# ecmwf-ifs/ecwam

Hardware: AMD Instinct MI355X
Metric: grid-point spectral steps/sec (whole node) at O320, 36dir x 36freq (higher is better)
Workload: dtype f32; 1 GPU; O320 all-ocean octahedral grid, 421080 sea points, 36 dir x 36 freq (NFRE_RED=36), full WAMINTGR step = PROPAGS2 advection + NEWWIND + IMPLSCH as one kernel (PROPAGS2 inside IMPLSCH's tile load), IDELT=IDELPRO=450 s, flag set A (IPHYS=1, ISNONLIN=0, LLGCBZ0=F, LLNORMAGAM=F); points_per_gpu=421080, halo_points=0, parallelism=sea-point block x1, ranks=1

## Files before the change

ecwam_amd/api.py:

```python
from __future__ import annotations

import ctypes as C

import numpy as np
import torch

from . import lib as _lib
from .tables import Tables

NFF, NINTF, NWPR = 16, 16, 5
OUTBS_SEP_FIELDS = ("mp1", "mp2", "wdw", "shww", "shts", "mdww", "mdts", "mpww", "mpts",
                    "p1sea", "p1swell", "p2sea", "p2swell", "sprdsea", "sprdswell")
OUTBS_PART_FIELDS = OUTBS_SEP_FIELDS + ("swh1", "mwd1", "mwp1", "swh2", "mwd2", "mwp2", "swh3", "mwd3", "mwp3")
OUTBS_EXT_FIELDS = ("c4", "bfi", "qp", "hmax", "tmax", "c3", "eta_m", "r", "xnslc", "cmax_f", "hmax_n", "cmax_st", "hmax_st")
OUTBS_ABS_FIELDS = ("swh", "mwd", "mwp", "em", "pp1d", "mp1", "mp2", "wdw")


class EcwamHipError(RuntimeError):
    pass


def _stream_ptr() -> int:
    return torch.cuda.current_stream().cuda_stream

# ... 146 lines not shown
            self._real(g["wlat"], (n, 2), "WLAT"), self._real(g["cosphm1_ext"], (nrow,), "COSPHM1_EXT"),
            self._real(depth_ext, (nrow,), "DEPTH_EXT"), self._real(u_ext, (nrow,), "U_EXT"), self._real(v_ext, (nrow,), "V_EXT"),
            self._real(refr, (n, 2 * self.NANG + 5), "REFR"), _stream_ptr()))

    def ctuw_refra(self, grid_dev: dict, cgroup_ext, omosnh2kd_ext, wavnum_ext, refr, cflfail, delpro: float, mstart=1, mend=None,
                   llcflcuroff=True, frange=0):
        mend = self.NR if mend is None else mend
        g = grid_dev
        n, nland, ngy = g["n"], g["nland"], g["ngy"]
        nrow = cgroup_ext.shape[0]
        if nland >= nrow:
            raise ValueError("CTUW: CGROUP_EXT must include the land row")
        ext = [self._real(a, (nrow, self.NFRE), nm) for a, nm in ((cgroup_ext, "CGROUP_EXT"), (omosnh2kd_ext, "OMOSNH2KD_EXT"),
                                                                 (wavnum_ext, "WAVNUM_EXT"))]
        self._chk(self.lib.ecwam_hip_ctuw_refra(self._h, n, nland, ngy, float(delpro), mstart, mend, *self._geom(g, n, ngy), *ext,
                                                self._real(g["cosphm1_ext"], (nrow,), "COSPHM1_EXT"),
                                                self._real(refr, (n, 2 * self.NANG + 5), "REFR"), int(llcflcuroff), int(frange),
                                                self._int(cflfail, (n,), "CFLFAIL"), _stream_ptr()))

    def propags2_refra(self, f1, f3, grid_dev: dict, cgroup_ext, omosnh2kd_ext, wavnum_ext, refr, delpro: float, kijs, kijl, nd3s=1,
                       nd3e=None, copy_rest=True, frange=0):
        nd3e = self.NR if nd3e is None else nd3e
        g = grid_dev
        n, nland, ngy = g["n"], g["nland"], g["ngy"]
        nrow = f1.shape[0]
        if not (0 <= kijs <= kijl <= n) or nland >= nrow or cgroup_ext.shape[0] != nrow:
            raise ValueError("PROPAGS2: KIJS/KIJL outside the neighbour tables, or F1 / CGROUP_EXT without the land row")
        ext = [self._real(a, (nrow, self.NFRE), nm) for a, nm in ((cgroup_ext, "CGROUP_EXT"), (omosnh2kd_ext, "OMOSNH2KD_EXT"),
                                                                 (wavnum_ext, "WAVNUM_EXT"))]
        self._chk(self.lib.ecwam_hip_propags2_refra(
            self._h, self._real(f1, (nrow, self.NANG, self.NFRE), "F1"), self._real(f3, (nrow, self.NANG, self.NFRE), "F3"), n, ngy,
            float(delpro), *self._geom(g, n, ngy), *ext, self._real(g["cosphm1_ext"], (nrow,), "COSPHM1_EXT"),
            self._real(refr, (n, 2 * self.NANG + 5), "REFR"), int(frange), kijs, kijl, nd3s, nd3e, int(copy_rest), _stream_ptr()))

    def implsch(self, kijs, kijl, fl1, wvprpt, ff, intf, mij, xllws, dbg=None, wam2nemo=None):
        nrow = fl1.shape[0]
        if not (0 <= kijs <= kijl <= min(nrow, wvprpt.shape[0], ff.shape[0], intf.shape[0], mij.shape[0], xllws.shape[0])):
            raise ValueError("IMPLSCH: KIJS/KIJL outside the operands")
        a = [self._real(fl1, (nrow, self.NANG, self.NFRE), "FL1"), self._real(wvprpt, (wvprpt.shape[0], NWPR, self.NFRE), "WVPRPT"),
             self._real(ff, (ff.shape[0], NFF), "FF"), self._real(intf, (intf.shape[0], NINTF), "INTF"),
             self._int(mij, (mij.shape[0],), "MIJ"), self._real(xllws, (xllws.shape[0], self.NANG, self.NFRE), "XLLWS")]
        pd = None if dbg is None else self._real(dbg, (nrow, 32), "DBG")
        pw = None
        if wam2nemo is not None:
            if not (wam2nemo.is_cuda and wam2nemo.dtype == torch.float64 and wam2nemo.is_contiguous() and wam2nemo.dim() == 2
                    and wam2nemo.shape[1] == 13 and wam2nemo.shape[0] >= kijl):
                raise ValueError("WAM2NEMO: expected contiguous float64 cuda tensor [npts >= KIJL][13]")
            pw = wam2nemo.data_ptr()
        self._chk(self.lib.ecwam_hip_implsch(self._h, kijs, kijl, *a, pw, pd, _stream_ptr()))

    def fused_supported(self, fast_waves: bool = False, obstructions: bool = False) -> bool:
        mask = int(self.lib.ecwam_hip_propags2_implsch_supported(self._h))
        need = 1 | (2 if fast_waves else 0) | (4 if obstructions else 0)
        return (mask & need) == need

    def propags2_implsch(self, f1, f3, grid_dev: dict, cgroup_ext, delpro: float, kijs, kijl, wvprpt, ff, intf, mij, xllws, nd3s=1, nd3e=None,
                         wam2nemo=None, flags: int = 0, ifrelfmax: int = 0, delpro_lf: float | None = None, gin=None):
        nd3e = self.NR if nd3e is None else nd3e
        g = grid_dev
        n, nland, ngy = g["n"], g["nland"], g["ngy"]
        nrow = f1.shape[0]
        if not (0 <= kijs <= kijl <= n) or nland >= nrow or cgroup_ext.shape[0] != nrow or f3.shape[0] < kijl:
            raise ValueError("PROPAGS2 + IMPLSCH: KIJS/KIJL outside the neighbour tables, or F1 / CGROUP_EXT without the land row")
        if not (kijl <= min(wvprpt.shape[0], ff.shape[0], intf.shape[0], mij.shape[0], xllws.shape[0])):
            raise ValueError("PROPAGS2 + IMPLSCH: KIJL outside the operands")
        pw = None
        if wam2nemo is not None:
            if not (wam2nemo.is_cuda and wam2nemo.dtype == torch.float64 and wam2nemo.is_contiguous() and wam2nemo.dim() == 2
                    and wam2nemo.shape[1] == 13 and wam2nemo.shape[0] >= kijl):
                raise ValueError("WAM2NEMO: expected contiguous float64 cuda tensor [npts >= KIJL][13]")
            pw = wam2nemo.data_ptr()
        args = [self._real(f1, (nrow, self.NANG, self.NFRE), "F1"), self._real(f3, (f3.shape[0], self.NANG, self.NFRE), "F3"), n, ngy, float(delpro),
                self._int(g["kxlt"], (n,), "KXLT"), self._real(g["zdello"], (ngy,), "ZDELLO"), float(g["xdella"]),
                self._real(g["cosph"], (ngy,), "COSPH"), self._real(g["sinph"], (ngy,), "SINPH"),
                self._int(g["klon"], (n, 2), "KLON"), self._int(g["klat"], (n, 2, 2), "KLAT"), self._int(g["kcor"], (n, 4, 2), "KCOR"),
                self._real(g["wlat"], (n, 2), "WLAT"), self._real(g["wcor"], (n, 4), "WCOR"),
                self._real(cgroup_ext, (nrow, self.NFRE), "CGROUP_EXT"), self._real(g["cosphm1_ext"], (nrow,), "COSPHM1_EXT"), kijs, kijl, nd3s, nd3e,
                self._real(wvprpt, (wvprpt.shape[0], NWPR, self.NFRE), "WVPRPT"), self._real(ff, (ff.shape[0], NFF), "FF"),
                self._real(intf, (intf.shape[0], NINTF), "INTF"), self._int(mij, (mij.shape[0],), "MIJ"),
                self._real(xllws, (xllws.shape[0], self.NANG, self.NFRE), "XLLWS"), pw,
                float(delpro if delpro_lf is None else delpro_lf), int(ifrelfmax),
                None if gin is None else self._real(gin, (gin.shape[0], self.NANG, gin.shape[2]), "GIN"), 0 if gin is None else int(gin.shape[2]),
                int(flags), _stream_ptr()]
        self._chk(self.lib.ecwam_hip_propags2_implsch(self._h, *args))

    def implsch_reserve(self, npts: int) -> None:
        self._chk(self.lib.ecwam_hip_implsch_reserve(self._h, int(npts)))

    def implsch_generation_used(self) -> int:
        return int(self.lib.ecwam_hip_implsch_generation_used(self._h))

    def device_tables(self) -> int:
        return int(self.lib.ecwam_hip_device_tables(self._h) or 0)

    def outbs(self, kijs, kijl, fl1, out, zmiss: float = -999.0):
        nrow = fl1.shape[0]
        if not (0 <= kijs <= kijl <= min(nrow, out.shape[0])):
            raise ValueError("OUTBS: KIJS/KIJL outside the operands")
        self._chk(self.lib.ecwam_hip_outbs(self._h, kijs, kijl, self._real(fl1, (nrow, self.NANG, self.NFRE), "FL1"), float(zmiss),
                                           self._real(out, (out.shape[0], 5), "OUT"), _stream_ptr()))

    def outbs_sepwisw(self, kijs, kijl, fl1, xllws, wvprpt, ff, out, zmiss: float = -999.0, small_domain: bool = False):
        nrow = fl1.shape[0]
        if not (0 <= kijs <= kijl <= min(nrow, xllws.shape[0], wvprpt.shape[0], ff.shape[0], out.shape[0])):
            raise ValueError("OUTBS_SEPWISW: KIJS/KIJL outside the operands")
        a = [self._real(fl1, (nrow, self.NANG, self.NFRE), "FL1"), self._real(xllws, (xllws.shape[0], self.NANG, self.NFRE), "XLLWS"),
             self._real(wvprpt, (wvprpt.shape[0], NWPR, self.NFRE), "WVPRPT"), self._real(ff, (ff.shape[0], NFF), "FF")]
        self._chk(self.lib.ecwam_hip_outbs_sepwisw(self._h, kijs, kijl, *a, 1 if small_domain else 0, float(zmiss),
                                                   self._real(out, (out.shape[0], len(OUTBS_SEP_FIELDS)), "OUT"), _stream_ptr()))

    def outbs_partition(self, kijs, kijl, fl1, xllws, mij, wvprpt, ff, out, zmiss: float = -999.0, flags: int = 0):
        nrow = fl1.shape[0]
        if not (0 <= kijs <= kijl <= min(nrow, xllws.shape[0], mij.shape[0], wvprpt.shape[0], ff.shape[0], out.shape[0])):
            raise ValueError("OUTBS_PARTITION: KIJS/KIJL outside the operands")
        a = [self._real(fl1, (nrow, self.NANG, self.NFRE), "FL1"), self._real(xllws, (xllws.shape[0], self.NANG, self.NFRE), "XLLWS"),
             self._int(mij, (mij.shape[0],), "MIJ"), self._real(wvprpt, (wvprpt.shape[0], NWPR, self.NFRE), "WVPRPT"),
             self._real(ff, (ff.shape[0], NFF), "FF")]
        self._chk(self.lib.ecwam_hip_outbs_partition(self._h, kijs, kijl, *a, int(flags), float(zmiss),
                                                     self._real(out, (out.shape[0], len(OUTBS_PART_FIELDS)), "OUT"), _stream_ptr()))

    def outbs_extremes(self, kijs, kijl, fl1, wvprpt, ff, out, kurtosis_only: bool = False):
        nrow = fl1.shape[0]
        if not (0 <= kijs <= kijl <= min(nrow, wvprpt.shape[0], ff.shape[0], out.shape[0])):
            raise ValueError("OUTBS_EXTREMES: KIJS/KIJL outside the operands")
        a = [self._real(fl1, (nrow, self.NANG, self.NFRE), "FL1"), self._real(wvprpt, (wvprpt.shape[0], NWPR, self.NFRE), "WVPRPT"),
             self._real(ff, (ff.shape[0], NFF), "FF")]
        self._chk(self.lib.ecwam_hip_outbs_extremes(self._h, kijs, kijl, *a, 1 if kurtosis_only else 0,
                                                    self._real(out, (out.shape[0], len(OUTBS_EXT_FIELDS)), "OUT"), _stream_ptr()))

    def outbs_absolute(self, kijs, kijl, fl1, wvprpt, ucur, vcur, ff, out, fl2nd=None, zmiss: float = -999.0, flags: int = 0):
        nrow = fl1.shape[0]
        rows = [nrow, out.shape[0]] + [a.shape[0] for a in (wvprpt, ucur, vcur, ff, fl2nd) if a is not None]
        if not (0 <= kijs <= kijl <= min(rows)):
            raise ValueError("OUTBS_ABSOLUTE: KIJS/KIJL outside the operands")
        opt = lambda a, shape, name: None if a is None else self._real(a, shape, name)
        a = [self._real(fl1, (nrow, self.NANG, self.NFRE), "FL1"),
             opt(wvprpt, (0 if wvprpt is None else wvprpt.shape[0], NWPR, self.NFRE), "WVPRPT"),
             opt(ucur, (0 if ucur is None else ucur.shape[0],), "UCUR"), opt(vcur, (0 if vcur is None else vcur.shape[0],), "VCUR"),
             opt(ff, (0 if ff is None else ff.shape[0], NFF), "FF")]
        self._chk(self.lib.ecwam_hip_outbs_absolute(self._h, kijs, kijl, *a, int(flags), float(zmiss),
                                                    self._real(out, (out.shape[0], len(OUTBS_ABS_FIELDS)), "OUT"),
                                                    opt(fl2nd, (0 if fl2nd is None else fl2nd.shape[0], self.NANG, self.NFRE), "FL2ND"), _stream_ptr()))

    @property
    def has_second_order(self) -> bool:
        return getattr(self, "_second_order", False)

    def set_second_order(self, so, coefficients=None) -> None:
        self._second_order = False
        if so is None:
            self._chk(self.lib.ecwam_hip_set_second_order(self._h, 0, 1.0, 1.1, 0, None, None, None, None, None, None, None))
            return
        dt = self.t.dtype
        if so.dtype != dt or so.NANGH * 2 != self.NANG or so.NFREH * 2 != self.NFRE:
            raise ValueError("second-order tables of another grid or precision")
        tabs = [getattr(so, c) for c in so.COEFFICIENTS] if coefficients is None else list(coefficients)
        shape = (so.NDEPTH, so.NANGH, so.NFREH, so.NFREH)
        host = [np.ascontiguousarray(np.asarray(a, dt).reshape(shape).transpose(3, 2, 1, 0)) for a in tabs]
        imp = np.ascontiguousarray(so.IM_P.T.astype(np.int32))
        imm = np.ascontiguousarray(so.IM_M.T.astype(np.int32))
        self._chk(self.lib.ecwam_hip_set_second_order(self._h, so.NDEPTH, float(so.DEPTHA), float(so.DEPTHD), so.NMAX, imp.ctypes.data, imm.ctypes.data,
                                                      *[a.ctypes.data for a in host]))
        self._second_order = True

    def outbs_second_order(self, kijs, kijl, fl1, wvprpt, depth, ucur, vcur, ff, out, fl2nd=None, sig: float = 1.0, zmiss: float = -999.0):
        nrow = fl1.shape[0]
        rows = [nrow, out.shape[0], wvprpt.shape[0], depth.shape[0]] + [a.shape[0] for a in (ucur, vcur, ff, fl2nd) if a is not None]
# ... 146 lines not shown
```

ecwam_amd/csrc/capi.hip:

```cpp
#include <cmath>
#include <cstdio>
#include <cstdlib>
#include <cstring>
#include <string>
#include <vector>

#include <dlfcn.h>
#include <rccl/rccl.h>

#include "dev.h"
#include "implsch_adv_args.h"

static thread_local std::string g_err;
static int fail(const std::string& m) {
  g_err = m;
  return 1;
}
#define HIPCHK(x)                                                                        \
  do {                                                                                   \
    hipError_t e_ = (x);                                                                 \
    if (e_ != hipSuccess) return fail(std::string(#x) + ": " + hipGetErrorString(e_));   \
  } while (0)

struct ecwam_hip_ctx {
  int real_bytes;
  int device;
  int NANG, NFRE, NFRE_RED;
  void* dtab = nullptr;
  double* norm_scratch = nullptr;
  void* itab = nullptr;
  int v4_ok = 0, v4_r1 = 0, v4_r2 = 0, v4_nh = 0, v4_shelter = 0;
  int implsch_last = 0;
  void* fin = nullptr;
  size_t fin_bytes = 0;
  void* wi = nullptr;
  size_t wi_bytes = 0;
  int rank = 0, nranks = 1;
  std::vector<int> peer, send_cnt, send_off, recv_dst0, recv_cnt;
  int n_send = 0, n_recv = 0;
  int* d_send_idx = nullptr;
  struct HaloSlot {
    int rowlen = 0;
    void* buf = nullptr;
    size_t bytes = 0;
    hipEvent_t ev_packed = nullptr, ev_done = nullptr;
    bool used = false;
    bool pending = false;
    unsigned long long age = 0;
  };
  static constexpr int NSLOT = 4;
  HaloSlot slot[NSLOT];
  unsigned long long slot_clock = 0;
  ncclComm_t comm = nullptr;
  hipStream_t comm_stream = nullptr;
  ecwam_hip_params p;
  void* fast_g = nullptr;
  int fast_gk = 0;
  std::string implsch_why;
  void* adv_pt = nullptr;
  size_t adv_pt_bytes = 0;
  void* adv_dir = nullptr;
  void* so_tab = nullptr;
  void* so_coef = nullptr;
  void* so_work = nullptr;
  size_t so_work_bytes = 0;
  int so_nmax = 0;
  std::vector<unsigned char> fr_host;
  const void* obs = nullptr;
  int n_obs = 0;
};

template <typename T> void launch_propags2(const void*, const void*, void*, const int*, const int*, const int*, const void*, int, int, int, int, int, int, hipStream_t);
template <typename T> void launch_ctuw(const void*, int, int, int, double, int, int, const int*, const void*, double, const void*, const void*, const int*, const int*, const int*, void*, void*, const void*, const void*, void*, int*, int, const void*, hipStream_t);
template <typename T> void launch_ctuwini_only(int, int, const int*, const int*, void*, void*, hipStream_t);
template <typename T> void launch_propdot(const void*, int, int, int, const int*, const void*, double, const void*, const int*, const int*, const void*, const void*, const void*, const void*, const void*, void*, hipStream_t);
template <typename T> void launch_curmask(int, int, int, const int*, void*, hipStream_t);
template <typename T> void launch_propags2_gen(const void*, int, const void*, void*, int, double, const int*, const void*, double, const void*, const void*, const int*, const int*, const int*, const void*, const void*, const void*, const void*, const void*, const void*, const void*, int*, int, int, int, int, int, int, int, const void*, hipStream_t);
template <typename T> void launch_propags2_otf(const void*, const void*, void*, int, int, double, const int*, const void*, double, const void*, const void*, const int*, const int*, const int*, const void*, const void*, const void*, const void*, const int*, int, int, int, int, int, int, const void*, int, double, int, void*, int, const void*, int, int, hipStream_t);
template <typename T> void launch_copy_freq_range(const void*, void*, int, int, int, int, int, int, hipStream_t);
template <typename T> int launch_outbs(const void*, int, int, const void*, double, void*, int, int, hipStream_t);
template <typename T> int launch_outbs_sepwisw(const void*, int, int, const void*, const void*, const void*, const void*, int, double, void*, int, int,
                                               hipStream_t);
template <typename T> int launch_outbs_partition(const void*, int, int, const void*, const void*, const int*, const void*, const void*, double, void*, int,
                                                  int, hipStream_t);
template <typename T> int launch_outbs_extremes(const void*, int, int, const void*, const void*, const void*, int, void*, int, int, hipStream_t);
template <typename T> int launch_outbs_absolute(const void*, const void*, int, int, int, const void*, const void*, const void*, const void*, const void*,
                                                 double, void*, void*, int, int, hipStream_t);
template <typename T> int launch_outbs_second_order(const void*, const void*, const void*, const void*, void*, int, int, int, int, const void*, const void*,
                                                     const void*, const void*, const void*, const void*, double, double, void*, void*, int, int, hipStream_t);
const char* so_tab_build(const ecwam_hip_params*, const void*, int, int, double, double, int, const int*, const int*, std::vector<unsigned char>&);
void so_coef_layout(int, int, int, int, const void* const[5], std::vector<unsigned char>&);
size_t so_work_bytes(int, int, int, int, int);
size_t intpol_tab_build(const ecwam_hip_params*, const ecwam_hip_tables*, int, std::vector<unsigned char>&);
template <typename T> void launch_norm(const void*, int, int, double, double*, int, hipStream_t);
template <typename T> void launch_newwind(const void*, int, void*, const void*, int, hipStream_t);
template <typename T> void launch_nosource(const void*, int, int, int, void*, void*, int*, hipStream_t);
template <typename T> void launch_c2p(const void*, void*, int, int, int, int, int, hipStream_t);
template <typename T> void launch_p2c(const void*, void*, int, int, int, int, int, hipStream_t);
template <typename T> void launch_pack(const void*, const int*, int, int, void*, hipStream_t);
template <typename T> void launch_proenv_pack(int, int, const void*, const void*, const void*, const void*, const void*, void*, hipStream_t);
template <typename T> void launch_proenv_unpack(int, int, const void*, const void*, void*, void*, void*, void*, void*, void*, hipStream_t);
template <typename T> int launch_implsch4(const void*, int, int, void*, const void*, void*, void*, int*, void*, void*, double*, void*, int, void*, int, int, int, int, int, int, hipStream_t);
template <typename T> int launch_implsch4x(const void*, int, int, void*, const void*, void*, void*, int*, void*, void*, double*, void*, int, void*, int, int, int, int, int, int, hipStream_t);
template <typename T> int launch_implsch4r(const void*, int, int, void*, const void*, void*, void*, int*, void*, void*, double*, void*, int, void*, int, int, int, int, int, int, hipStream_t);
template <typename T> void launch_ctu_prep(const void*, int, int, int, double, double, const int*, const void*, double, const void*, const void*, const void*, const void*, const void*, void*, void*, int*, hipStream_t);
template <typename T> int launch_implsch4_adv(const void*, int, int, void*, const void*, void*, void*, int*, void*, void*, double*, const Implsch4AdvArgs*, int, int, int, int, int, int, hipStream_t);
int implsch4_adv_forms(int, int);
int implsch4_fin_row();

template <typename T>
static void v4_probe(const DevTab<T>& h, ecwam_hip_ctx* c) {
  c->v4_ok = 0;
  const int NANG = h.NANG;
  if (!h.DIA_PULL || !h.V4_ROWS || (NANG & 1) || h.NFRE != 36) return;
  const int r1 = (NANG - h.K1W[0][0]) % NANG, r2 = h.K2W[0][0];
  if (h.D11[0] != -1 || h.D21[0] != 1 || h.D11[1] != 1 || h.D21[1] != -1) return;
  if (h.K1W[1][0] != r1 % NANG || h.K2W[1][0] != (NANG - r2) % NANG) return;
  T wmax = T(0);
  for (int t = 0; t < h.NTAP; t++) wmax = wmax > h.SATWEIGHTS[t][NANG / 2] ? wmax : h.SATWEIGHTS[t][NANG / 2];
  const T eps = sizeof(T) == 4 ? T(1.2e-7) : T(2.3e-16);
  for (int t = 0; t < h.NTAP; t++)
    for (int k = 0; k < NANG; k++) {
      const T d = h.SATWEIGHTS[t][k] - h.SATWEIGHTS[t][NANG / 2];
      if ((d < 0 ? -d : d) > T(16) * eps * wmax) return;
      const T e = h.SATWEIGHTS[t][NANG / 2] - h.SATWEIGHTS[h.NTAP - 1 - t][NANG / 2];
      if ((e < 0 ? -e : e) > T(16) * eps * wmax) return;
      if (h.INDICESSAT[t][k] != ((k - h.NSDSNTH + t) % NANG + NANG) % NANG) return;
    }
  c->v4_r1 = r1; c->v4_r2 = r2; c->v4_nh = h.NSDSNTH; c->v4_shelter = (h.TAUWSHELTER != T(0)); c->v4_ok = 1;
}

template <typename T>
static void cpv(T* dst, const void* src, int n) {
  if (src) for (int i = 0; i < n; i++) dst[i] = ((const T*)src)[i];
}

template <typename T>
static int build_tab(const ecwam_hip_params* p, const ecwam_hip_tables* t, DevTab<T>* d) {
  memset(d, 0, sizeof(*d));
  const int NANG = p->nang, NFRE = p->nfre, ML = p->mlsthg;
  d->NANG = NANG; d->NFRE = NFRE; d->NFRE_RED = p->nfre_red; d->NFRE_ODD = p->nfre_odd; d->IDELT = p->idelt;
  d->LLGCBZ0 = p->llgcbz0; d->LLNORMAGAM = p->llnormagam; d->LLCAPCHNK = p->llcapchnk; d->LBIWBK = p->lbiwbk;
  d->LICERUN = p->licerun; d->LMASKICE = p->lmaskice; d->LWAMRSETCI = p->lwamrsetci; d->LWVFLX_SNL = p->lwvflx_snl;
  d->LWFLUX = p->lwflux; d->LCFLX = (p->lwflux || p->lwfluxout || p->lwnemocou); d->LWNEMOCOU = p->lwnemocou; d->LWCOU = p->lwcou;
  d->LWCOUAST = p->lwcouast; d->LWNEMOCOUWRS = p->lwnemocouwrs;
  d->LWNEMOTAUOC = p->lwnemotauoc; d->LWNEMOCOUSEND = p->lwnemocousend; d->LWNEMOCOUSTK = p->lwnemocoustk;
  d->ICODE = p->icode; d->ISNONLIN = p->isnonlin; d->IPHYS = p->iphys; d->IDAMPING = p->idamping;
  d->LCISCAL = p->lciscal; d->LCIWA2 = p->lciwa2; d->LCIWA3 = p->lciwa3;
  d->LCIWA1 = p->lciwa1; d->LWNEMOCOUIBR = p->lwnemocouibr; d->LWNEMOCOUSTRN = p->lwnemocoustrn; d->NICT = p->nict; d->NICH = p->nich;
  for (int i = 0; i < 36 * 16; i++) d->CIDEAC[i] = T(0);
  if (p->lciwa1 && t->cideac) cpv(d->CIDEAC, t->cideac, p->nict * p->nich);
  d->DBG_SKIP = 0;
#ifdef ECWAM_HIP_DIAGNOSTICS
  { const char* e_ = getenv("ECWAM_HIP_DEBUG_SKIP"); d->DBG_SKIP = e_ ? atoi(e_) : 0; }
#endif
  d->NSDSNTH = p->nsdsnth; d->NTAP = 2 * p->nsdsnth + 1; d->MFRSTLW = p->mfrstlw; d->MLSTHG = ML; d->KFRH = p->kfrh; d->NWAV_GC = p->nwav_gc;
#define S_(dst, src) d->dst = (T)p->src
  S_(ZIBRW_THRSH, zibrw_thrsh); S_(TICMIN, ticmin); S_(DTIC, dtic); S_(DHIC, dhic); S_(HICMIN, hicmin);
  S_(XIMP, ximp); S_(G, g); S_(GM1, gm1); S_(PI, pi); S_(ZPI, zpi); S_(ZPI4GM1, zpi4gm1); S_(ZPI4GM2, zpi4gm2); S_(EPSMIN, epsmin);
  S_(ROWATER, rowater); S_(ROWATERM1, rowaterm1); S_(EPSUS, epsus); S_(EPSU10, epsu10); S_(ACD, acd); S_(BCD, bcd);
  S_(ACDLIN, acdlin); S_(BCDLIN, bcdlin); S_(CDMAX, cdmax); S_(TAUOCMIN, tauocmin); S_(TAUOCMAX, tauocmax);
  S_(PHIEPSMIN, phiepsmin); S_(PHIEPSMAX, phiepsmax); S_(WSEMEAN_MIN, wsemean_min); S_(CIRC, circ); S_(R, r_earth);
  S_(FRATIO, fratio); S_(WETAIL, wetail); S_(FRTAIL, frtail); S_(WP1TAIL, wp1tail); S_(FRIC, fric); S_(DELTH, delth);
  S_(FLOGSPRDM1, flogsprdm1); S_(XKAPPA, xkappa); S_(XNLEV, xnlev); S_(RNU, rnu); S_(RNUM, rnum);
  S_(BETAMAXOXKAPPA2, betamaxoxkappa2); S_(BMAXOKAP, bmaxokap); S_(GAMNCONST, gamnconst); S_(ZALP, zalp); S_(ALPHA, alpha);
  S_(ALPHAMIN, alphamin); S_(ALPHAMAX, alphamax); S_(CHNKMIN_U, chnkmin_u); S_(TAUWSHELTER, tauwshelter); S_(DTHRN_A, dthrn_a);
  S_(DTHRN_U, dthrn_u); S_(TAILFACTOR, tailfactor); S_(TAILFACTOR_PM, tailfactor_pm); S_(ANG_GC_A, ang_gc_a);
  S_(ANG_GC_B, ang_gc_b); S_(ANG_GC_C, ang_gc_c); S_(RN1_RN, rn1_rn); S_(ALPHAPMAX, alphapmax); S_(CDIS, cdis); S_(DELTA_SDIS, delta_sdis); S_(CDISVIS, cdisvis); S_(CDICWA, cdicwa); S_(ZALPFACB, zalpfacb); S_(ZALPFACX, zalpfacx); S_(SWELLF, swellf); S_(SWELLF2, swellf2);
  S_(SWELLF3, swellf3); S_(SWELLF4, swellf4); S_(SWELLF5, swellf5); S_(SWELLF6, swellf6); S_(SWELLF7, swellf7);
  S_(SWELLF7M1, swellf7m1); S_(Z0RAT, z0rat); S_(Z0TUBMAX, z0tubmax); S_(ABMIN, abmin); S_(ABMAX, abmax); S_(SDSBR, sdsbr);
  S_(SSDSC2, ssdsc2); S_(SSDSC3, ssdsc3); S_(SSDSC4, ssdsc4); S_(SSDSC5, ssdsc5); S_(SSDSC6, ssdsc6); S_(MICHE, miche);
  S_(EGRCRV, egrcrv); S_(AFCRV, afcrv); S_(BFCRV, bfcrv); S_(X0TAUHF, x0tauhf); S_(EPS1, eps1); S_(FLMIN, flmin);
  S_(CITHRSH, cithrsh); S_(CIBLOCK, ciblock); S_(CITHRSH_TAIL, cithrsh_tail); S_(ZALPWRS, zalpwrs); S_(BATHYMAX, bathymax);
  S_(WSPMIN, wspmin); S_(WSPMIN_RESET_TAUW, wspmin_reset_tauw); S_(DAL1, dal1); S_(DAL2, dal2);
  S_(XLOGKRATIOM1_GC, xlogkratiom1_gc); S_(SQRTGOSURFT, sqrtgosurft);
#undef S_
  cpv(d->FR, t->fr, NFRE); cpv(d->DFIM, t->dfim, NFRE); cpv(d->DFIMOFR, t->dfimofr, NFRE); cpv(d->DFIMFR, t->dfimfr, NFRE);
  cpv(d->DFIM_SIM, t->dfim_sim, NFRE); cpv(d->RHOWG_DFIM, t->rhowg_dfim, NFRE); cpv(d->ZPIFR, t->zpifr, NFRE);
  cpv(d->FR5, t->fr5, NFRE); cpv(d->COFRM4, t->cofrm4, NFRE); cpv(d->FLMAX, t->flmax, NFRE);
  cpv(d->TH, t->th, NANG); cpv(d->COSTH, t->costh, NANG); cpv(d->SINTH, t->sinth, NANG);
  cpv(d->WTAUHF, t->wtauhf, JTOT);
  cpv(d->SWELLFT + 1, t->swellft, ECWAM_HIP_IAB);
  for (int i = 0; i < ML; i++) { d->IKP[i] = t->ikp[i]; d->IKP1[i] = t->ikp1[i]; d->IKM[i] = t->ikm[i]; d->IKM1[i] = t->ikm1[i]; }
  cpv(d->AF11, t->af11, ML);
  for (int k = 0; k < NANG; k++)
    for (int kh = 0; kh < 2; kh++) {
      d->K1W[kh][k] = t->k1w[k * 2 + kh] - 1; d->K2W[kh][k] = t->k2w[k * 2 + kh] - 1;
      d->K11W[kh][k] = t->k11w[k * 2 + kh] - 1; d->K21W[kh][k] = t->k21w[k * 2 + kh] - 1;
// ... 237 lines not shown
  HIPCHK(hipGetLastError());
  HIPCHK(hipMemcpy(h, d, 2 * sizeof(int), hipMemcpyDeviceToHost));
  (void)hipFree(d);
  if (h[0] || h[1]) return fail("ecwam_hip_selftest: a wavefront primitive returned a wrong value");
  return 0;
}

int ecwam_hip_create(const ecwam_hip_params* p, const ecwam_hip_tables* t, int real_bytes, int device, ecwam_hip_ctx** out) {
  if (!p || !t || !out) return fail("ecwam_hip_create: null argument");
  if (real_bytes != 4 && real_bytes != 8) return fail("ecwam_hip_create: real_bytes must be 4 or 8");
  if (p->nang < 4 || p->nang > MAXA || p->nfre < 8 || p->nfre > MAXF || p->nfre_red < 1 || p->nfre_red > p->nfre)
    return fail("ecwam_hip_create: NANG/NFRE/NFRE_RED out of the supported range");
  if (p->mlsthg > MAXMC || 2 * p->nsdsnth + 1 > MAXTAP || p->nwav_gc + 1 > MAXGC) return fail("ecwam_hip_create: table size exceeds library limits");
  if ((p->iphys != 0 && p->iphys != 1) || (p->isnonlin < 0 || p->isnonlin > 2) || p->irefra < 0 || p->irefra > 3 || p->icode < 1 || p->icode > 3)
    return fail("ecwam_hip_create: only IPHYS=0/1, ISNONLIN=0/1/2, IREFRA=0..3, ICODE=1..3 are on the hot path (SURVEY.md 8a)");
  if (p->lciwa1 && (!t->cideac || p->nict < 2 || p->nich < 2 || p->nict * p->nich > 36 * 16))
    return fail("ecwam_hip_create: LCIWA1 (SDICE1) needs the CIDEAC table (tables.cideac, NICT*NICH <= 576)");
  {
    const void* need[] = {t->fr, t->dfim, t->dfimofr, t->dfimfr, t->dfim_sim, t->rhowg_dfim, t->zpifr, t->fr5, t->cofrm4, t->flmax, t->th, t->costh,
                          t->sinth, t->wtauhf, t->swellft, t->ikp, t->ikp1, t->ikm, t->ikm1, t->af11, t->k1w, t->k2w, t->k11w, t->k21w, t->inlcoef,
                          t->rnlcoef, t->indicessat, t->satweights, t->kpm, t->jxo, t->jyo, t->kcr};
    for (const void* q : need) if (!q) return fail("ecwam_hip_create: a required table pointer is NULL");
    if (p->nwav_gc > 0 && (!t->xk_gc || !t->xkm_gc || !t->omega_gc || !t->omxkm3_gc || !t->cm_gc || !t->c2osqrtvg_gc || !t->xkmsqrtvgoc2_gc ||
                           !t->om3gmkm_gc || !t->delkcc_gc_ns || !t->delkcc_omxkm3_gc)) return fail("ecwam_hip_create: a gravity-capillary table pointer is NULL");
  }
  HIPCHK(hipSetDevice(device));
  ecwam_hip_ctx* c = new ecwam_hip_ctx();
  c->real_bytes = real_bytes; c->device = device; c->NANG = p->nang; c->NFRE = p->nfre; c->NFRE_RED = p->nfre_red; c->p = *p;
  c->fr_host.assign((const unsigned char*)t->fr, (const unsigned char*)t->fr + (size_t)p->nfre * real_bytes);
#define HIPCHK_CTX(x)                                                                              \
  do {                                                                                             \
    hipError_t e_ = (x);                                                                           \
    if (e_ != hipSuccess) { if (c->dtab) (void)hipFree(c->dtab); if (c->itab) (void)hipFree(c->itab); delete c; return fail(std::string(#x) + ": " + hipGetErrorString(e_)); } \
  } while (0)
  if (real_bytes == 4) {
    std::vector<DevTab<float>> h(1);
    build_tab<float>(p, t, h.data());
    if (!h[0].DIA_PULL) { delete c; return fail("ecwam_hip_create: the interaction tables do not have the rotation structure of INISNONLIN (K1W = K -+ r1, K2W = K +- r2, INLCOEF = MC, MC+2, MC+3, MC-4, MC-3; KFRH = 8, MFRSTLW = -3): not supported"); }
    v4_probe<float>(h[0], c);
    HIPCHK_CTX(hipMalloc(&c->dtab, sizeof(DevTab<float>)));
    HIPCHK_CTX(hipMemcpy(c->dtab, h.data(), sizeof(DevTab<float>), hipMemcpyHostToDevice));
  } else {
    std::vector<DevTab<double>> h(1);
    build_tab<double>(p, t, h.data());
    if (!h[0].DIA_PULL) { delete c; return fail("ecwam_hip_create: the interaction tables do not have the rotation structure of INISNONLIN (K1W = K -+ r1, K2W = K +- r2, INLCOEF = MC, MC+2, MC+3, MC-4, MC-3; KFRH = 8, MFRSTLW = -3): not supported"); }
    v4_probe<double>(h[0], c);
    HIPCHK_CTX(hipMalloc(&c->dtab, sizeof(DevTab<double>)));
    HIPCHK_CTX(hipMemcpy(c->dtab, h.data(), sizeof(DevTab<double>), hipMemcpyHostToDevice));
  }
  if (p->irefra >= 2) {
    std::vector<unsigned char> h;
    const size_t nb = intpol_tab_build(p, t, real_bytes, h);
    if (nb) {
      HIPCHK_CTX(hipMalloc(&c->itab, nb));
      HIPCHK_CTX(hipMemcpy(c->itab, h.data(), nb, hipMemcpyHostToDevice));
    }
  }
#undef HIPCHK_CTX
  {
    const char* why = nullptr;
    const bool inst = (c->NANG == 48 && c->v4_r1 == 1 && c->v4_r2 == 4 && c->v4_nh == 11) || (c->NANG == 36 && c->v4_r1 == 1 && c->v4_r2 == 3 && c->v4_nh == 8) ||
                      (c->NANG == 24 && c->v4_r1 == 0 && c->v4_r2 == 2 && c->v4_nh == 5) || (c->NANG == 12 && c->v4_r1 == 0 && c->v4_r2 == 1 && c->v4_nh == 3);
    if (p->nfre != 36) why = "NFRE must be 36 (the frequency grid of every configuration of the reference)";
    else if (!c->v4_ok) why = "the saturation weights / indices do not have the structure of INIT_SDISS_ARDH (COS**2 taps, symmetric, the same for every direction) or the DIA mirror images differ";
    else if (!inst) why = "NANG must be 48, 36, 24 or 12 with the interaction rotations and the saturation half-width of INISNONLIN / INIT_SDISS_ARDH on that grid";
    else if (p->iphys == 1 && p->llnormagam && c->v4_shelter) why = "LLNORMAGAM needs TAUWSHELTER = 0 (setwavphys.F90:150-190: the normalised growth rate replaces the sheltering)";
    else if (p->iphys == 1 && !p->llnormagam && !c->v4_shelter) why = "IPHYS = 1 without LLNORMAGAM needs TAUWSHELTER /= 0 (setwavphys.F90:150-190)";
    if (why) c->implsch_why = std::string("configuration not covered by the IMPLSCH kernel: ") + why;
  }
  *out = c;
  return 0;
}

int ecwam_hip_destroy(ecwam_hip_ctx* c) {
  if (!c) return 0;
  if (c->dtab) (void)hipFree(c->dtab);
  if (c->norm_scratch) (void)hipFree(c->norm_scratch);
  if (c->itab) (void)hipFree(c->itab);
  if (c->so_tab) (void)hipFree(c->so_tab);
  if (c->so_coef) (void)hipFree(c->so_coef);
  if (c->so_work) (void)hipFree(c->so_work);
  if (c->fin) (void)hipFree(c->fin);
  if (c->wi) (void)hipFree(c->wi);
  if (c->adv_pt) (void)hipFree(c->adv_pt);
  if (c->adv_dir) (void)hipFree(c->adv_dir);
  halo_release(c);
  delete c;
  return 0;
}

#define DISPATCH(call_f, call_d) \
  do {                           \
    if (c->real_bytes == 4) {    \
      call_f;                    \
    } else {                     \
      call_d;                    \
    }                            \
  } while (0)

int ecwam_hip_set_obstructions(ecwam_hip_ctx* c, const void* obs, int n) {
  if (!c) return fail("null context");
  if (n < 0 || (obs && n == 0)) return fail("ecwam_hip_set_obstructions: bad size");
  c->obs = obs; c->n_obs = obs ? n : 0;
  return 0;
}

int ecwam_hip_propags2(ecwam_hip_ctx* c, const void* f1, void* f3, const int* klon, const int* klat, const int* kcor, const void* w,
                       int kijs, int kijl, int nd3s, int nd3e, int copy_rest, void* stream) {
  if (!c) return fail("null context");
  if (kijl < kijs || nd3s < 1 || nd3e > c->NFRE_RED || nd3e < nd3s - 1) return fail("ecwam_hip_propags2: bad range");
  if (kijl > kijs && (!f1 || !f3 || !klon || !klat || !kcor || !w)) return fail("ecwam_hip_propags2: null pointer");
  if (f1 == f3) return fail("ecwam_hip_propags2: F1 and F3 must not alias");
  hipStream_t s = (hipStream_t)stream;
  const int N = (c->NANG << 16) | (c->NFRE << 8) | c->NFRE_RED;
  DISPATCH(launch_propags2<float>(c->dtab, f1, f3, klon, klat, kcor, w, kijs, kijl, nd3s - 1, nd3e, copy_rest, N, s),
           launch_propags2<double>(c->dtab, f1, f3, klon, klat, kcor, w, kijs, kijl, nd3s - 1, nd3e, copy_rest, N, s));
  HIPCHK(hipGetLastError());
  return 0;
}

int ecwam_hip_ctuw(ecwam_hip_ctx* c, int n, int nland, int ngy, double delpro, int mstart, int mend, const int* kxlt, const void* zdello,
                   double xdella, const void* cosph, const void* sinph, const int* klon, const int* klat, const int* kcor, void* wlat,
                   void* wcor, const void* cgroup_ext, const void* cosphm1_ext, void* w, int* cflfail, void* stream) {
  if (!c) return fail("null context");
  if (n < 0 || mstart < 1 || mend > c->NFRE_RED || mend < mstart) return fail("ecwam_hip_ctuw: bad range");
  if (n > 0 && (!kxlt || !zdello || !cosph || !sinph || !klon || !klat || !kcor || !wlat || !wcor || !cgroup_ext || !cosphm1_ext || !cflfail))
    return fail("ecwam_hip_ctuw: null pointer");
  if (c->obs && n > c->n_obs) return fail("ecwam_hip_ctuw: more points than the obstruction table holds");
  hipStream_t s = (hipStream_t)stream;
  DISPATCH(launch_ctuw<float>(c->dtab, n, nland, ngy, delpro, mstart - 1, mend, kxlt, zdello, xdella, cosph, sinph, klon, klat, kcor, wlat, wcor, cgroup_ext, cosphm1_ext, w, cflfail, c->NANG, c->obs, s),
           launch_ctuw<double>(c->dtab, n, nland, ngy, delpro, mstart - 1, mend, kxlt, zdello, xdella, cosph, sinph, klon, klat, kcor, wlat, wcor, cgroup_ext, cosphm1_ext, w, cflfail, c->NANG, c->obs, s));
  HIPCHK(hipGetLastError());
  return 0;
}

int ecwam_hip_propags2_otf_split(ecwam_hip_ctx* c, const void* f1, void* f3, int n, int ngy, double delpro, double delpro_lf, int ifrelfmax,
                                 int in_nfre, void* gout, int gout_nfre, const int* kxlt, const void* zdello, double xdella, const void* cosph, const void* sinph, const int* klon,
                                 const int* klat, const int* kcor, const void* wlat, const void* wcor, const void* cgroup_ext,
                                 const void* cosphm1_ext, const int* order, int kijs, int kijl, int nd3s, int nd3e, int copy_rest,
                                 void* stream) {
  return ecwam_hip_propags2_otf_fast(c, f1, f3, n, ngy, delpro, delpro_lf, ifrelfmax, in_nfre, nullptr, 0, 0, gout, gout_nfre, kxlt, zdello, xdella, cosph,
                                     sinph, klon, klat, kcor, wlat, wcor, cgroup_ext, cosphm1_ext, order, kijs, kijl, nd3s, nd3e, copy_rest, stream);
}

int ecwam_hip_propags2_otf_fast(ecwam_hip_ctx* c, const void* f1, void* f3, int n, int ngy, double delpro, double delpro_lf, int ifrelfmax,
                                int in_nfre, const void* gin, int gin_nfre, int out_nfre, void* gout, int gout_nfre, const int* kxlt,
                                const void* zdello, double xdella, const void* cosph, const void* sinph, const int* klon, const int* klat,
                                const int* kcor, const void* wlat, const void* wcor, const void* cgroup_ext, const void* cosphm1_ext,
                                const int* order, int kijs, int kijl, int nd3s, int nd3e, int copy_rest, void* stream) {
  if (!c) return fail("null context");
  if (out_nfre == 0) out_nfre = c->NFRE;
  if (out_nfre != c->NFRE && (out_nfre < nd3e || out_nfre > c->NFRE || gout))
    return fail("ecwam_hip_propags2_otf_fast: a compact output buffer must hold every advected frequency and excludes a second compact copy");
  if (gin && (in_nfre != 0 && in_nfre != c->NFRE)) return fail("ecwam_hip_propags2_otf_fast: the compact fast-wave input goes with full input rows");
  if (gin && (gin_nfre < 1 || gin_nfre > c->NFRE || gin == f3 || gin == gout)) return fail("ecwam_hip_propags2_otf_fast: bad compact input buffer");
  {
    const int vec = 16 / c->real_bytes;
    if ((gin && (gin_nfre % vec != 0 || ((uintptr_t)gin % 16) != 0)) || (out_nfre != c->NFRE && (out_nfre % vec != 0 || ((uintptr_t)f3 % 16) != 0)) ||
        (in_nfre != 0 && in_nfre != c->NFRE && (in_nfre % vec != 0 || ((uintptr_t)f1 % 16) != 0)))
      return fail("ecwam_hip_propags2_otf_fast: compact rows must be 16-byte aligned and hold a multiple of 16 bytes per direction");
  }
  if (kijl < kijs || kijs < 0 || (!order && kijl > n) || nd3s < 1 || nd3e > c->NFRE_RED || nd3e < nd3s - 1 || ifrelfmax < 0 || ifrelfmax > c->NFRE_RED)
    return fail("ecwam_hip_propags2_otf: bad range");
  if ((copy_rest & 4) && !order) return fail("ecwam_hip_propags2_otf: 2-D tiles need a processing order");
  if (in_nfre == 0) in_nfre = c->NFRE;
  if (gout && (gout_nfre < 1 || gout_nfre > c->NFRE || gout_nfre % (16 / c->real_bytes) != 0 || gout == f1 || ((uintptr_t)gout % 16) != 0))
    return fail("ecwam_hip_propags2_otf: the compact output buffer must be 16-byte aligned, distinct from F1, and hold a multiple of 16 bytes per direction");
  if (in_nfre != c->NFRE && (in_nfre < nd3e || in_nfre > c->NFRE || ((copy_rest & 1) && out_nfre != in_nfre)))
    return fail("ecwam_hip_propags2_otf: a compact input buffer must hold every advected frequency; copy_rest only into a compact output of the same width");
  if (kijl > kijs && (!f1 || !f3 || !kxlt || !zdello || !cosph || !sinph || !klon || !klat || !kcor || !wlat || !wcor || !cgroup_ext || !cosphm1_ext))
    return fail("ecwam_hip_propags2_otf: null pointer");
  if (f1 == f3) return fail("ecwam_hip_propags2_otf: F1 and F3 must not alias");
  if (c->obs && (order ? n : kijl) > c->n_obs) return fail("ecwam_hip_propags2_otf: more points than the obstruction table holds");
  hipStream_t s = (hipStream_t)stream;
  const int N = (c->NANG << 16) | (c->NFRE << 8) | c->NFRE_RED;
  copy_rest = (copy_rest & 1) | (copy_rest & 4);
#ifdef ECWAM_HIP_DIAGNOSTICS
  { const char* e_ = getenv("ECWAM_HIP_OTF_WALK"); if (e_ && atoi(e_) == 0) copy_rest |= 2; }
#endif
  DISPATCH(launch_propags2_otf<float>(c->dtab, f1, f3, n, ngy, delpro, kxlt, zdello, xdella, cosph, sinph, klon, klat, kcor, wlat, wcor, cgroup_ext, cosphm1_ext, order, kijs, kijl, nd3s - 1, nd3e, copy_rest, N, c->obs, ifrelfmax, delpro_lf, in_nfre, gout, gout_nfre, gin, gin_nfre, out_nfre, s),
           launch_propags2_otf<double>(c->dtab, f1, f3, n, ngy, delpro, kxlt, zdello, xdella, cosph, sinph, klon, klat, kcor, wlat, wcor, cgroup_ext, cosphm1_ext, order, kijs, kijl, nd3s - 1, nd3e, copy_rest, N, c->obs, ifrelfmax, delpro_lf, in_nfre, gout, gout_nfre, gin, gin_nfre, out_nfre, s));
  HIPCHK(hipGetLastError());
  return 0;
}

int ecwam_hip_propags2_otf(ecwam_hip_ctx* c, const void* f1, void* f3, int n, int ngy, double delpro, const int* kxlt, const void* zdello,
                           double xdella, const void* cosph, const void* sinph, const int* klon, const int* klat, const int* kcor,
                           const void* wlat, const void* wcor, const void* cgroup_ext, const void* cosphm1_ext, const int* order,
                           int kijs, int kijl, int nd3s, int nd3e, int copy_rest, void* stream) {
  return ecwam_hip_propags2_otf_split(c, f1, f3, n, ngy, delpro, delpro, 0, 0, nullptr, 0, kxlt, zdello, xdella, cosph, sinph, klon, klat, kcor, wlat, wcor,
                                      cgroup_ext, cosphm1_ext, order, kijs, kijl, nd3s, nd3e, copy_rest, stream);
}

int ecwam_hip_copy_freq_range(ecwam_hip_ctx* c, const void* src, void* dst, int n, int m_first, int m_last, int dst_nfre, void* stream) {
  if (!c) return fail("null context");
  if (dst_nfre == 0) dst_nfre = c->NFRE;
  if (n < 0 || m_first < 1 || m_last > c->NFRE || m_last < m_first - 1 || m_last > dst_nfre) return fail("ecwam_hip_copy_freq_range: bad range");
  if (n > 0 && (!src || !dst)) return fail("ecwam_hip_copy_freq_range: null pointer");
  hipStream_t s = (hipStream_t)stream;
  DISPATCH(launch_copy_freq_range<float>(src, dst, n, c->NANG, c->NFRE, m_first - 1, m_last, dst_nfre, s),
           launch_copy_freq_range<double>(src, dst, n, c->NANG, c->NFRE, m_first - 1, m_last, dst_nfre, s));
  HIPCHK(hipGetLastError());
  return 0;
}

int ecwam_hip_propdot(ecwam_hip_ctx* c, int n, int nland, const int* kxlt, const void* zdello, double xdella, const void* cosph,
                      const int* klon, const int* klat, const void* wlat, const void* cosphm1_ext, const void* depth_ext,
                      const void* u_ext, const void* v_ext, void* refr, void* stream) {
  if (!c) return fail("null context");
  if (n < 0) return fail("ecwam_hip_propdot: bad range");
  if (n > 0 && (!kxlt || !zdello || !cosph || !klon || !klat || !wlat || !cosphm1_ext || !depth_ext || !u_ext || !v_ext || !refr))
// ... 6 lines not shown
}

static int propags2_gen_launch(ecwam_hip_ctx* c, const char* who, const void* f1, void* f3, int ngy, double delpro,
                               const int* kxlt, const void* zdello, double xdella, const void* cosph, const void* sinph,
                               const int* klon, const int* klat, const int* kcor, const void* wlat, const void* wcor,
                               const void* cgroup_ext, const void* omosnh2kd_ext, const void* wavnum_ext, const void* cosphm1_ext,
                               const void* refr, int* cflfail, int slot, int kijs, int kijl, int m0, int m1, int copy_rest,
                               hipStream_t s) {
  if (kijl > kijs && (!kxlt || !zdello || !cosph || !sinph || !klon || !klat || !kcor || !wlat || !wcor || !cgroup_ext || !omosnh2kd_ext ||
                      !wavnum_ext || !cosphm1_ext || !refr))
    return fail((std::string(who) + ": null pointer").c_str());
  const int N = (c->NANG << 16) | (c->NFRE << 8) | c->NFRE_RED;
  DISPATCH(launch_propags2_gen<float>(c->dtab, c->p.irefra, f1, f3, ngy, delpro, kxlt, zdello, xdella, cosph, sinph, klon, klat, kcor, wlat, wcor, cgroup_ext, omosnh2kd_ext, wavnum_ext, cosphm1_ext, refr, cflfail, slot, kijs, kijl, m0, m1, copy_rest, N, c->obs, s),
           launch_propags2_gen<double>(c->dtab, c->p.irefra, f1, f3, ngy, delpro, kxlt, zdello, xdella, cosph, sinph, klon, klat, kcor, wlat, wcor, cgroup_ext, omosnh2kd_ext, wavnum_ext, cosphm1_ext, refr, cflfail, slot, kijs, kijl, m0, m1, copy_rest, N, c->obs, s));
  HIPCHK(hipGetLastError());
  return 0;
}

int ecwam_hip_ctuw_refra(ecwam_hip_ctx* c, int n, int nland, int ngy, double delpro, int mstart, int mend, const int* kxlt,
                         const void* zdello, double xdella, const void* cosph, const void* sinph, const int* klon, const int* klat,
                         const int* kcor, void* wlat, void* wcor, const void* cgroup_ext, const void* omosnh2kd_ext,
                         const void* wavnum_ext, const void* cosphm1_ext, void* refr, int llcflcuroff, int range, int* cflfail,
                         void* stream) {
  if (!c) return fail("null context");
  if (n < 0 || mstart < 1 || mend > c->NFRE_RED || mend < mstart || range < 0 || range > 1) return fail("ecwam_hip_ctuw_refra: bad range");
  if (n > 0 && (!wlat || !wcor || !cflfail || !klat || !kcor || !refr)) return fail("ecwam_hip_ctuw_refra: null pointer");
  if (n == 0) return 0;
  hipStream_t s = (hipStream_t)stream;
  DISPATCH(launch_ctuwini_only<float>(n, nland, klat, kcor, wlat, wcor, s), launch_ctuwini_only<double>(n, nland, klat, kcor, wlat, wcor, s));
  const bool cur = c->p.irefra == 2 || c->p.irefra == 3;
  std::vector<int> prev;
  if (range == 1) {
    prev.resize((size_t)n);
    HIPCHK(hipMemcpyAsync(prev.data(), cflfail, sizeof(int) * (size_t)n, hipMemcpyDeviceToHost, s));
    HIPCHK(hipStreamSynchronize(s));
  }
  HIPCHK(hipMemsetAsync(cflfail, 0, sizeof(int) * (size_t)n, s));
  DISPATCH(launch_curmask<float>(n, c->NANG, range, nullptr, refr, s), launch_curmask<double>(n, c->NANG, range, nullptr, refr, s));
  int rc = propags2_gen_launch(c, "ecwam_hip_ctuw_refra", nullptr, nullptr, ngy, delpro, kxlt, zdello, xdella, cosph, sinph, klon, klat, kcor,
                               wlat, wcor, cgroup_ext, omosnh2kd_ext, wavnum_ext, cosphm1_ext, refr, cflfail, range, 0, n, mstart - 1, mend, 0, s);
  if (rc) return rc;
  if (cur && llcflcuroff) {
    std::vector<int> h((size_t)n);
    HIPCHK(hipMemcpyAsync(h.data(), cflfail, sizeof(int) * (size_t)n, hipMemcpyDeviceToHost, s));
    HIPCHK(hipStreamSynchronize(s));
    bool any = false;
    for (int i = 0; i < n && !any; i++) any = h[i] != 0;
    if (any) {
      DISPATCH(launch_curmask<float>(n, c->NANG, range, cflfail, refr, s), launch_curmask<double>(n, c->NANG, range, cflfail, refr, s));
      HIPCHK(hipMemsetAsync(cflfail, 0, sizeof(int) * (size_t)n, s));
      rc = propags2_gen_launch(c, "ecwam_hip_ctuw_refra", nullptr, nullptr, ngy, delpro, kxlt, zdello, xdella, cosph, sinph, klon, klat,
                               kcor, wlat, wcor, cgroup_ext, omosnh2kd_ext, wavnum_ext, cosphm1_ext, refr, cflfail, range, 0, n, mstart - 1, mend, 0, s);
      if (rc) return rc;
    }
  }
  if (range == 1) {
    std::vector<int> h((size_t)n);
    HIPCHK(hipMemcpyAsync(h.data(), cflfail, sizeof(int) * (size_t)n, hipMemcpyDeviceToHost, s));
    HIPCHK(hipStreamSynchronize(s));
    for (int i = 0; i < n; i++) h[i] |= prev[i];
    HIPCHK(hipMemcpyAsync(cflfail, h.data(), sizeof(int) * (size_t)n, hipMemcpyHostToDevice, s));
    HIPCHK(hipStreamSynchronize(s));
  }
  return 0;
}

int ecwam_hip_propags2_refra(ecwam_hip_ctx* c, const void* f1, void* f3, int n, int ngy, double delpro, const int* kxlt,
                             const void* zdello, double xdella, const void* cosph, const void* sinph, const int* klon,
                             const int* klat, const int* kcor, const void* wlat, const void* wcor, const void* cgroup_ext,
                             const void* omosnh2kd_ext, const void* wavnum_ext, const void* cosphm1_ext, const void* refr, int range,
                             int kijs, int kijl, int nd3s, int nd3e, int copy_rest, void* stream) {
  if (!c) return fail("null context");
  if (kijl < kijs || kijs < 0 || kijl > n || nd3s < 1 || nd3e > c->NFRE_RED || nd3e < nd3s - 1 || range < 0 || range > 1)
    return fail("ecwam_hip_propags2_refra: bad range");
  if (kijl > kijs && (!f1 || !f3)) return fail("ecwam_hip_propags2_refra: null pointer");
  if (f1 == f3) return fail("ecwam_hip_propags2_refra: F1 and F3 must not alias");
  if (c->obs && kijl > c->n_obs) return fail("ecwam_hip_propags2_refra: more points than the obstruction table holds");
  return propags2_gen_launch(c, "ecwam_hip_propags2_refra", f1, f3, ngy, delpro, kxlt, zdello, xdella, cosph, sinph, klon, klat, kcor, wlat,
                             wcor, cgroup_ext, omosnh2kd_ext, wavnum_ext, cosphm1_ext, refr, nullptr, range, kijs, kijl, nd3s - 1, nd3e,
                             copy_rest ? 1 : 0, (hipStream_t)stream);
}

static bool fused_ok(const ecwam_hip_ctx* c);
static int adv_reserve(ecwam_hip_ctx* c, int npts) {
  if (!fused_ok(c) || !implsch4_adv_forms(c->NANG, c->real_bytes)) return 0;
  const size_t need = (size_t)(npts > 0 ? npts : 0) * 12 * c->real_bytes;
  if (need > c->adv_pt_bytes) {
    if (c->adv_pt) HIPCHK(hipFree(c->adv_pt));
    c->adv_pt = nullptr; c->adv_pt_bytes = 0;
    HIPCHK(hipMalloc(&c->adv_pt, need));
    c->adv_pt_bytes = need;
  }
  if (!c->adv_dir) HIPCHK(hipMalloc(&c->adv_dir, (size_t)(6 * c->NANG + 4) * c->real_bytes + (size_t)4 * c->NANG * sizeof(int)));
  return 0;
}
static bool runs_rare_builds(const ecwam_hip_ctx* c) {
  const int ext = (c->p.llnormagam || c->p.llgcbz0) ? 1 : 0;
  const bool rare4 = c->p.lciwa2 || c->p.lwnemocouwrs || c->p.lwnemocoustrn || c->p.isnonlin > 1 || c->p.icode != 3 || !c->p.lwvflx_snl;
  const int alt = (c->p.iphys == 0 ? 1 : 0) | (c->p.isnonlin == 1 ? 2 : 0);
  return !(!rare4 && (alt == 0 || (!ext && alt != 3)));
}
static int implsch_reserve_on(ecwam_hip_ctx* c, int npts, hipStream_t s, bool sync);
int ecwam_hip_implsch(ecwam_hip_ctx* c, int kijs, int kijl, void* fl1, const void* wvprpt, void* ff, void* intf, int* mij, void* xllws,
                      double* wam2nemo, void* dbg, void* stream) {
  if (!c) return fail("null context");
  if (kijl < kijs || kijs < 0) return fail("ecwam_hip_implsch: bad range");
  HIPCHK(hipSetDevice(c->device));
  if (kijl > kijs && (!fl1 || !wvprpt || !ff || !intf || !mij || !xllws)) return fail("ecwam_hip_implsch: null pointer");
  if (kijl > kijs && c->p.lwnemocou && !wam2nemo) return fail("ecwam_hip_implsch: LWNEMOCOU needs the WAVE2OCEAN buffer");
  if (!c->p.lwnemocou) wam2nemo = nullptr;
  hipStream_t s = (hipStream_t)stream;
  int rc = -1;
  if (!c->implsch_why.empty()) return fail("ecwam_hip_implsch: " + c->implsch_why);
  if (dbg) return fail("ecwam_hip_implsch: the per-point debug rows were an output of the retired one-point-per-wavefront kernel: pass NULL");
  const int ext = (c->p.llnormagam || c->p.llgcbz0) ? 1 : 0;
  const bool rare4 = c->p.lciwa2 || c->p.lwnemocouwrs || c->p.lwnemocoustrn || c->p.isnonlin > 1 || c->p.icode != 3 || !c->p.lwvflx_snl;
  const int alt = (c->p.iphys == 0 ? 1 : 0) | (c->p.isnonlin == 1 ? 2 : 0);
  const bool common_ok = !rare4 && (alt == 0 || (!ext && alt != 3));
  {
    if (int rc2 = implsch_reserve_on(c, kijl, s, false)) return rc2;
    if (!common_ok)
      DISPATCH(rc = launch_implsch4r<float>(c->dtab, kijs, kijl, fl1, wvprpt, ff, intf, mij, xllws, c->fin, wam2nemo, c->fast_g, c->fast_gk, c->wi, c->NANG, c->NFRE, c->v4_r1, c->v4_r2, c->v4_nh, c->p.iphys == 0 ? 1 : 0, s),
               rc = launch_implsch4r<double>(c->dtab, kijs, kijl, fl1, wvprpt, ff, intf, mij, xllws, c->fin, wam2nemo, c->fast_g, c->fast_gk, c->wi, c->NANG, c->NFRE, c->v4_r1, c->v4_r2, c->v4_nh, c->p.iphys == 0 ? 1 : 0, s));
    else if (alt)
      DISPATCH(rc = launch_implsch4x<float>(c->dtab, kijs, kijl, fl1, wvprpt, ff, intf, mij, xllws, c->fin, wam2nemo, c->fast_g, c->fast_gk, c->wi, c->NANG, c->NFRE, c->v4_r1, c->v4_r2, c->v4_nh, alt, s),
               rc = launch_implsch4x<double>(c->dtab, kijs, kijl, fl1, wvprpt, ff, intf, mij, xllws, c->fin, wam2nemo, c->fast_g, c->fast_gk, c->wi, c->NANG, c->NFRE, c->v4_r1, c->v4_r2, c->v4_nh, alt, s));
    else
      DISPATCH(rc = launch_implsch4<float>(c->dtab, kijs, kijl, fl1, wvprpt, ff, intf, mij, xllws, c->fin, wam2nemo, c->fast_g, c->fast_gk, c->wi, c->NANG, c->NFRE, c->v4_r1, c->v4_r2, c->v4_nh, ext, s),
               rc = launch_implsch4<double>(c->dtab, kijs, kijl, fl1, wvprpt, ff, intf, mij, xllws, c->fin, wam2nemo, c->fast_g, c->fast_gk, c->wi, c->NANG, c->NFRE, c->v4_r1, c->v4_r2, c->v4_nh, ext, s));
    if (rc == 0) { HIPCHK(hipGetLastError()); c->implsch_last = 4; return 0; }
  }
  return fail("ecwam_hip_implsch: no build of k_implsch4 covers the configuration (ecwam_hip_create should have refused it)");
}

static bool fused_ok(const ecwam_hip_ctx* c) {
  if (!c->implsch_why.empty()) return false;
  const bool rare4 = c->p.lciwa2 || c->p.lwnemocouwrs || c->p.lwnemocoustrn || c->p.isnonlin > 1 || c->p.icode != 3 || !c->p.lwvflx_snl;
  return !rare4 && c->p.iphys == 1 && c->p.isnonlin == 0 && c->NFRE == 36;
}
int ecwam_hip_propags2_implsch_supported(ecwam_hip_ctx* c) { return c && fused_ok(c) ? implsch4_adv_forms(c->NANG, c->real_bytes) : 0; }

int ecwam_hip_propags2_implsch(ecwam_hip_ctx* c, const void* f1, void* f3, int n, int ngy, double delpro, const int* kxlt, const void* zdello,
                               double xdella, const void* cosph, const void* sinph, const int* klon, const int* klat, const int* kcor,
                               const void* wlat, const void* wcor, const void* cgroup_ext, const void* cosphm1_ext, int kijs, int kijl, int nd3s,
                               int nd3e, const void* wvprpt, void* ff, void* intf, int* mij, void* xllws, double* wam2nemo, double delpro_lf,
                               int ifrelfmax, const void* gin, int gin_nfre, int flags, void* stream) {
  if (!c) return fail("null context");
  if (flags) return fail("ecwam_hip_propags2_implsch: unknown flags");
  if (!fused_ok(c) || !implsch4_adv_forms(c->NANG, c->real_bytes)) return fail("ecwam_hip_propags2_implsch: no one-kernel build covers the configuration (ecwam_hip_propags2_implsch_supported): call ecwam_hip_propags2_otf and ecwam_hip_implsch");
  if (kijl < kijs || kijs < 0 || kijl > n || nd3s < 1 || nd3e > c->NFRE_RED || nd3e < nd3s - 1) return fail("ecwam_hip_propags2_implsch: bad range");
  if (kijl > kijs && (!f1 || !f3 || !kxlt || !zdello || !cosph || !sinph || !klon || !klat || !kcor || !wlat || !wcor || !cgroup_ext || !cosphm1_ext ||
                      !wvprpt || !ff || !intf || !mij || !xllws))
    return fail("ecwam_hip_propags2_implsch: null pointer");
  if (f1 == f3) return fail("ecwam_hip_propags2_implsch: F1 and F3 must not alias (the neighbours of a point are read while other points are stored)");
  if (((uintptr_t)f1 % 16) != 0 || ((uintptr_t)f3 % 16) != 0) return fail("ecwam_hip_propags2_implsch: the spectra must be 16-byte aligned");
  if (ifrelfmax < 0 || ifrelfmax > c->NFRE_RED || (ifrelfmax > 0) != (gin != nullptr))
    return fail("ecwam_hip_propags2_implsch: fast waves (ifrelfmax > 0) come with their compact input rows (gin), and only then");
  if (gin && (nd3s != 1 || gin_nfre < ifrelfmax || gin_nfre > c->NFRE || gin_nfre % (16 / c->real_bytes) != 0 || ((uintptr_t)gin % 16) != 0 || gin == c->fast_g ||
              !(delpro_lf > 0.0)))
    return fail("ecwam_hip_propags2_implsch: the compact fast-wave rows must be 16-byte aligned, hold the fast waves in a multiple of 16 bytes per direction, and differ from the rows of ecwam_hip_set_fastwave_copy");
  if (c->p.lwnemocou && kijl > kijs && !wam2nemo) return fail("ecwam_hip_propags2_implsch: LWNEMOCOU needs the WAVE2OCEAN buffer");
  if (c->obs && kijl > c->n_obs) return fail("ecwam_hip_propags2_implsch: more points than the obstruction table holds");
  if (!c->p.lwnemocou) wam2nemo = nullptr;
  HIPCHK(hipSetDevice(c->device));
  hipStream_t s = (hipStream_t)stream;
  if (kijl == kijs) return 0;
  if (int rc2 = implsch_reserve_on(c, kijl, s, false)) return rc2;
  const size_t dir_reals = (size_t)(6 * c->NANG + 4);
  int* dirI = reinterpret_cast<int*>(reinterpret_cast<char*>(c->adv_dir) + dir_reals * c->real_bytes);
  const double dlf = gin ? delpro_lf : 0.0;
  DISPATCH(launch_ctu_prep<float>(c->dtab, kijs, kijl, ngy, delpro, dlf, kxlt, zdello, xdella, cosph, sinph, wlat, wcor, cosphm1_ext, c->adv_pt, c->adv_dir, dirI, s),
           launch_ctu_prep<double>(c->dtab, kijs, kijl, ngy, delpro, dlf, kxlt, zdello, xdella, cosph, sinph, wlat, wcor, cosphm1_ext, c->adv_pt, c->adv_dir, dirI, s));
  Implsch4AdvArgs a;
  a.f_in = f1; a.klon = klon; a.klat = klat; a.kcor = kcor; a.cg = cgroup_ext; a.pt = c->adv_pt; a.dirT = c->adv_dir; a.dirI = dirI;
  a.xdella = xdella; a.delpro = delpro; a.m0 = nd3s - 1; a.m1 = nd3e;
  a.gin = gin; a.delpro_lf = dlf; a.gin_k = gin ? gin_nfre : 0; a.mlf = gin ? ifrelfmax : 0;
  a.obs = c->obs;
  a.gfast = c->fast_g; a.gfast_k = c->fast_g ? c->fast_gk : 0;
  const int ext = (c->p.llnormagam || c->p.llgcbz0) ? 1 : 0;
  int rc = -1;
  DISPATCH(rc = launch_implsch4_adv<float>(c->dtab, kijs, kijl, f3, wvprpt, ff, intf, mij, xllws, c->fin, wam2nemo, &a, c->NANG, c->NFRE, c->v4_r1, c->v4_r2, c->v4_nh, ext, s),
           rc = launch_implsch4_adv<double>(c->dtab, kijs, kijl, f3, wvprpt, ff, intf, mij, xllws, c->fin, wam2nemo, &a, c->NANG, c->NFRE, c->v4_r1, c->v4_r2, c->v4_nh, ext, s));
  if (rc != 0) return fail("ecwam_hip_propags2_implsch: no one-kernel build covers the configuration (the strict build of the weights has neither the fast-wave nor the obstruction form)");
  HIPCHK(hipGetLastError());
  c->implsch_last = 4;
  return 0;
}

int ecwam_hip_set_fastwave_copy(ecwam_hip_ctx* c, void* g, int g_nfre) {
  if (!c) return fail("null context");
  if (g && (g_nfre < 1 || g_nfre > c->NFRE || g_nfre % (16 / c->real_bytes) != 0 || ((uintptr_t)g % 16) != 0))
    return fail("ecwam_hip_set_fastwave_copy: the compact rows must be 16-byte aligned and hold a multiple of 16 bytes per direction");
  c->fast_g = g; c->fast_gk = g ? g_nfre : 0;
  return 0;
}

static int implsch_reserve_on(ecwam_hip_ctx* c, int npts, hipStream_t s, bool sync) {
  HIPCHK(hipSetDevice(c->device));
  const size_t need = (size_t)(npts > 0 ? npts : 0) * implsch4_fin_row() * c->real_bytes;
  if (need > c->fin_bytes) {
    if (c->fin) HIPCHK(hipFree(c->fin));
    c->fin = nullptr; c->fin_bytes = 0;
    HIPCHK(hipMalloc(&c->fin, need));
    HIPCHK(hipMemsetAsync(c->fin, 0, need, s));
    HIPCHK(hipStreamSynchronize(s));
    (void)sync;
    c->fin_bytes = need;
  }
  const bool split = c->real_bytes == 8 && runs_rare_builds(c);
  const size_t need_wi = split ? (size_t)(npts > 0 ? npts : 0) * c->NANG * c->NFRE * c->real_bytes : 0;
  if (need_wi > c->wi_bytes) {
    if (c->wi) HIPCHK(hipFree(c->wi));
    c->wi = nullptr; c->wi_bytes = 0;
    HIPCHK(hipMalloc(&c->wi, need_wi));
    c->wi_bytes = need_wi;
  }
  return adv_reserve(c, npts);
}

int ecwam_hip_implsch_reserve(ecwam_hip_ctx* c, int npts) {
  if (!c) return fail("ecwam_hip_implsch_reserve: null context");
  return implsch_reserve_on(c, npts, nullptr, true);
}

int ecwam_hip_implsch_generation_used(ecwam_hip_ctx* c) { return c ? c->implsch_last : 0; }

const void* ecwam_hip_device_tables(ecwam_hip_ctx* c) { return c ? c->dtab : nullptr; }

int ecwam_hip_outbs(ecwam_hip_ctx* c, int kijs, int kijl, const void* fl1, double zmiss, void* out, void* stream) {
  if (!c) return fail("null context");
  if (kijl < kijs || kijs < 0) return fail("ecwam_hip_outbs: bad range");
  if (kijl > kijs && (!fl1 || !out)) return fail("ecwam_hip_outbs: null pointer");
  hipStream_t s = (hipStream_t)stream;
  int rc;
  DISPATCH(rc = launch_outbs<float>(c->dtab, kijs, kijl, fl1, zmiss, out, c->NANG, c->NFRE, s),
           rc = launch_outbs<double>(c->dtab, kijs, kijl, fl1, zmiss, out, c->NANG, c->NFRE, s));
  if (rc) return fail("ecwam_hip_outbs: unsupported spectral size");
  HIPCHK(hipGetLastError());
  return 0;
}

int ecwam_hip_outbs_sepwisw(ecwam_hip_ctx* c, int kijs, int kijl, const void* fl1, const void* xllws, const void* wvprpt, const void* ff, int flags,
                            double zmiss, void* out, void* stream) {
  if (!c) return fail("null context");
  if (kijl < kijs || kijs < 0) return fail("ecwam_hip_outbs_sepwisw: bad range");
  if (kijl > kijs && (!fl1 || !xllws || !wvprpt || !ff || !out)) return fail("ecwam_hip_outbs_sepwisw: null pointer");
  if (flags & ~1) return fail("ecwam_hip_outbs_sepwisw: unknown flags");
  hipStream_t s = (hipStream_t)stream;
  int rc;
  DISPATCH(rc = launch_outbs_sepwisw<float>(c->dtab, kijs, kijl, fl1, xllws, wvprpt, ff, flags, zmiss, out, c->NANG, c->NFRE, s),
           rc = launch_outbs_sepwisw<double>(c->dtab, kijs, kijl, fl1, xllws, wvprpt, ff, flags, zmiss, out, c->NANG, c->NFRE, s));
  if (rc) return fail("ecwam_hip_outbs_sepwisw: unsupported spectral size");
  HIPCHK(hipGetLastError());
  return 0;
}

int ecwam_hip_outbs_partition(ecwam_hip_ctx* c, int kijs, int kijl, const void* fl1, const void* xllws, const int* mij, const void* wvprpt,
                              const void* ff, int flags, double zmiss, void* out, void* stream) {
  if (!c) return fail("null context");
  if (kijl < kijs || kijs < 0) return fail("ecwam_hip_outbs_partition: bad range");
  if (kijl > kijs && (!fl1 || !xllws || !mij || !wvprpt || !ff || !out)) return fail("ecwam_hip_outbs_partition: null pointer");
  if (flags & 1)
    return fail("ecwam_hip_outbs_partition: CLDOMAIN = 's' (flags bit 0) is not supported: SEP3TR would read an FSEA that SEPWISW has not computed");
  if (flags) return fail("ecwam_hip_outbs_partition: unknown flags");
  hipStream_t s = (hipStream_t)stream;
  int rc;
  DISPATCH(rc = launch_outbs_partition<float>(c->dtab, kijs, kijl, fl1, xllws, mij, wvprpt, ff, zmiss, out, c->NANG, c->NFRE, s),
           rc = launch_outbs_partition<double>(c->dtab, kijs, kijl, fl1, xllws, mij, wvprpt, ff, zmiss, out, c->NANG, c->NFRE, s));
  if (rc) return fail("ecwam_hip_outbs_partition: unsupported spectral size");
  HIPCHK(hipGetLastError());
  return 0;
}

int ecwam_hip_outbs_extremes(ecwam_hip_ctx* c, int kijs, int kijl, const void* fl1, const void* wvprpt, const void* ff, int flags, void* out,
                             void* stream) {
  if (!c) return fail("null context");
  if (kijl < kijs || kijs < 0) return fail("ecwam_hip_outbs_extremes: bad range");
  if (kijl > kijs && (!fl1 || !wvprpt || !ff || !out)) return fail("ecwam_hip_outbs_extremes: null pointer");
  if (flags & ~1) return fail("ecwam_hip_outbs_extremes: unknown flags");
  hipStream_t s = (hipStream_t)stream;
  int rc;
  DISPATCH(rc = launch_outbs_extremes<float>(c->dtab, kijs, kijl, fl1, wvprpt, ff, flags, out, c->NANG, c->NFRE, s),
           rc = launch_outbs_extremes<double>(c->dtab, kijs, kijl, fl1, wvprpt, ff, flags, out, c->NANG, c->NFRE, s));
  if (rc) return fail("ecwam_hip_outbs_extremes: unsupported spectral size");
  HIPCHK(hipGetLastError());
  return 0;
}

int ecwam_hip_outbs_absolute(ecwam_hip_ctx* c, int kijs, int kijl, const void* fl1, const void* wvprpt, const void* ucur, const void* vcur,
                             const void* ff, int flags, double zmiss, void* out, void* fl2nd, void* stream) {
  if (!c) return fail("null context");
  if (kijl < kijs || kijs < 0) return fail("ecwam_hip_outbs_absolute: bad range");
  if (flags) return fail("ecwam_hip_outbs_absolute: unknown flags");
  const bool intpol = c->p.irefra >= 2, ice = c->p.licerun && !c->p.lmaskice;
  if (kijl > kijs && (!fl1 || !out)) return fail("ecwam_hip_outbs_absolute: null pointer");
  if (kijl > kijs && intpol && (!wvprpt || !ucur || !vcur)) return fail("ecwam_hip_outbs_absolute: IREFRA = 2 / 3 needs wvprpt, ucur and vcur");
  if (kijl > kijs && ice && !ff) return fail("ecwam_hip_outbs_absolute: LICERUN without LMASKICE needs ff (CICOVER, WSWAVE)");
  if (fl2nd && fl2nd == fl1) return fail("ecwam_hip_outbs_absolute: FL1 and FL2ND must not alias");
  if (intpol && !c->itab) return fail("ecwam_hip_outbs_absolute: NFRE_MAX of INTPOL exceeds the library's table");
  hipStream_t s = (hipStream_t)stream;
  const int mode = (intpol ? 1 : 0) | (ice ? 2 : 0);
  int rc;
  DISPATCH(rc = launch_outbs_absolute<float>(c->dtab, c->itab, kijs, kijl, mode, fl1, wvprpt, ucur, vcur, ff, zmiss, out, fl2nd, c->NANG, c->NFRE, s),
           rc = launch_outbs_absolute<double>(c->dtab, c->itab, kijs, kijl, mode, fl1, wvprpt, ucur, vcur, ff, zmiss, out, fl2nd, c->NANG, c->NFRE, s));
  if (rc) return fail("ecwam_hip_outbs_absolute: unsupported spectral size");
// ... 116 lines not shown
  if (!c) return fail("null context");
  if (nproma < 1 || nchnk < 0 || npts > nproma * nchnk || n2 < 1 || n3 < 1) return fail("ecwam_hip_chunks_to_points: bad shape");
  hipStream_t s = (hipStream_t)stream;
  DISPATCH(launch_c2p<float>(chunked, points, nproma, nchnk, npts, n2, n3, s), launch_c2p<double>(chunked, points, nproma, nchnk, npts, n2, n3, s));
  HIPCHK(hipGetLastError());
  return 0;
}

int ecwam_hip_points_to_chunks(ecwam_hip_ctx* c, const void* points, void* chunked, int nproma, int nchnk, int npts, int n2, int n3, void* stream) {
  if (!c) return fail("null context");
  if (nproma < 1 || nchnk < 0 || npts > nproma * nchnk || npts <= nproma * (nchnk - 1) || n2 < 1 || n3 < 1) return fail("ecwam_hip_points_to_chunks: bad shape");
  hipStream_t s = (hipStream_t)stream;
  DISPATCH(launch_p2c<float>(points, chunked, nproma, nchnk, npts, n2, n3, s), launch_p2c<double>(points, chunked, nproma, nchnk, npts, n2, n3, s));
  HIPCHK(hipGetLastError());
  return 0;
}

static int member_args(const char* who, int nproma, int nchnk, int npts, int nm, long long row_stride, long long row_off, int elem_bytes,
                       const void* a, const void* b) {
  if (nproma < 1 || nchnk < 0 || npts < 0 || npts > nproma * nchnk || (npts > 0 && npts <= nproma * (nchnk - 1)) || nm < 1 || row_off < 0 ||
      row_off + nm > row_stride || (elem_bytes != 4 && elem_bytes != 8))
    return fail(std::string(who) + ": bad shape");
  if (npts > 0 && (!a || !b)) return fail(std::string(who) + ": null pointer");
  return 0;
}

int ecwam_hip_member_scatter(ecwam_hip_ctx* c, const void* chunked, void* rows, int nproma, int nchnk, int npts, int nm, long long row_stride,
                             long long row_off, int elem_bytes, void* stream) {
  if (!c) return fail("null context");
  if (member_args("ecwam_hip_member_scatter", nproma, nchnk, npts, nm, row_stride, row_off, elem_bytes, chunked, rows)) return 1;
  if (npts == 0) return 0;
  hipStream_t s = (hipStream_t)stream;
  const long long total = (long long)npts * nm;
  const int nb = (int)((total + 255) / 256 > 65535 ? 65535 : (total + 255) / 256);
  if (elem_bytes == 4)
    hipLaunchKernelGGL(k_member_scatter<unsigned int>, dim3(nb), dim3(256), 0, s, (const unsigned int*)chunked, (unsigned int*)rows, nproma, npts, nm, row_stride, row_off);
  else
    hipLaunchKernelGGL(k_member_scatter<unsigned long long>, dim3(nb), dim3(256), 0, s, (const unsigned long long*)chunked, (unsigned long long*)rows, nproma, npts, nm, row_stride, row_off);
  HIPCHK(hipGetLastError());
  return 0;
}

int ecwam_hip_member_gather(ecwam_hip_ctx* c, const void* rows, void* chunked, int nproma, int nchnk, int npts, int nm, long long row_stride,
                            long long row_off, int elem_bytes, void* stream) {
  if (!c) return fail("null context");
  if (member_args("ecwam_hip_member_gather", nproma, nchnk, npts, nm, row_stride, row_off, elem_bytes, rows, chunked)) return 1;
  if (npts == 0) return 0;
  hipStream_t s = (hipStream_t)stream;
  const long long total = (long long)nchnk * nproma * nm;
  const int nb = (int)((total + 255) / 256 > 65535 ? 65535 : (total + 255) / 256);
  if (elem_bytes == 4)
    hipLaunchKernelGGL(k_member_gather<unsigned int>, dim3(nb), dim3(256), 0, s, (const unsigned int*)rows, (unsigned int*)chunked, nproma, nchnk, npts, nm, row_stride, row_off);
  else
    hipLaunchKernelGGL(k_member_gather<unsigned long long>, dim3(nb), dim3(256), 0, s, (const unsigned long long*)rows, (unsigned long long*)chunked, nproma, nchnk, npts, nm, row_stride, row_off);
  HIPCHK(hipGetLastError());
  return 0;
}

int ecwam_hip_pack_rows(ecwam_hip_ctx* c, const void* fl, const int* idx, int n, void* buf, void* stream) {
  if (!c) return fail("null context");
  if (n > 0 && (!fl || !idx || !buf)) return fail("ecwam_hip_pack_rows: null pointer");
  hipStream_t s = (hipStream_t)stream;
  const int rowlen = c->NANG * c->NFRE;
  DISPATCH(launch_pack<float>(fl, idx, n, rowlen, buf, s), launch_pack<double>(fl, idx, n, rowlen, buf, s));
  HIPCHK(hipGetLastError());
  return 0;
}

int ecwam_hip_unpack_rows(ecwam_hip_ctx* c, const void* buf, int n, void* fl, int dst0, void* stream) {
  if (!c) return fail("null context");
  if (n > 0 && (!fl || !buf)) return fail("ecwam_hip_unpack_rows: null pointer");
  if (n <= 0) return 0;
  const size_t row = (size_t)c->NANG * c->NFRE * c->real_bytes;
  HIPCHK(hipMemcpyAsync((char*)fl + (size_t)dst0 * row, buf, (size_t)n * row, hipMemcpyDeviceToDevice, (hipStream_t)stream));
  return 0;
}

int ecwam_hip_halo_setup(ecwam_hip_ctx* c, int rank, int nranks, int npeers, const int* peer, const int* send_count, const int* send_idx,
                         const int* recv_dst0, const int* recv_count) {
  if (!c) return fail("null context");
  if (nranks < 1 || rank < 0 || rank >= nranks || npeers < 0 || (npeers > 0 && (!peer || !send_count || !recv_dst0 || !recv_count)))
    return fail("ecwam_hip_halo_setup: bad arguments");
  HIPCHK(hipSetDevice(c->device));
  if (c->d_send_idx) { (void)hipFree(c->d_send_idx); c->d_send_idx = nullptr; }
  c->rank = rank; c->nranks = nranks;
  c->peer.assign(peer, peer + npeers); c->send_cnt.assign(send_count, send_count + npeers);
  c->recv_dst0.assign(recv_dst0, recv_dst0 + npeers); c->recv_cnt.assign(recv_count, recv_count + npeers);
  c->send_off.resize(npeers);
  c->n_send = 0; c->n_recv = 0;
  for (int i = 0; i < npeers; i++) {
    if (peer[i] < 0 || peer[i] >= nranks || send_count[i] < 0 || recv_count[i] < 0 || recv_dst0[i] < 0)
      return fail("ecwam_hip_halo_setup: bad peer entry");
    c->send_off[i] = c->n_send; c->n_send += send_count[i]; c->n_recv += recv_count[i];
  }
  if (c->n_send > 0) {
    if (!send_idx) return fail("ecwam_hip_halo_setup: send_idx missing");
    HIPCHK(hipMalloc(&c->d_send_idx, (size_t)c->n_send * sizeof(int)));
    HIPCHK(hipMemcpy(c->d_send_idx, send_idx, (size_t)c->n_send * sizeof(int), hipMemcpyHostToDevice));
  }
  if (!c->comm_stream) HIPCHK(hipStreamCreateWithFlags(&c->comm_stream, hipStreamNonBlocking));
  return 0;
}

int ecwam_hip_proenvhalo_pack(ecwam_hip_ctx* c, int n, const void* wvprpt, const void* omosnh2kd, const void* depth, const void* ucur, const void* vcur,
                              void* buffer_ext, void* stream) {
  if (!c) return fail("null context");
  if (n < 0 || (n > 0 && (!wvprpt || !omosnh2kd || !depth || !ucur || !vcur || !buffer_ext))) return fail("ecwam_hip_proenvhalo_pack: bad arguments");
  DISPATCH(launch_proenv_pack<float>(n, c->NFRE, wvprpt, omosnh2kd, depth, ucur, vcur, buffer_ext, (hipStream_t)stream),
           launch_proenv_pack<double>(n, c->NFRE, wvprpt, omosnh2kd, depth, ucur, vcur, buffer_ext, (hipStream_t)stream));
  HIPCHK(hipGetLastError());
  return 0;
}

int ecwam_hip_proenvhalo_unpack(ecwam_hip_ctx* c, int nrows, const void* buffer_ext, const void* land, void* wavnum_ext, void* cgroup_ext,
                                void* omosnh2kd_ext, void* depth_ext, void* u_ext, void* v_ext, void* stream) {
  if (!c) return fail("null context");
  if (nrows < 0 || !buffer_ext || !land || !wavnum_ext || !cgroup_ext || !omosnh2kd_ext || !depth_ext || !u_ext || !v_ext)
    return fail("ecwam_hip_proenvhalo_unpack: bad arguments");
  DISPATCH(launch_proenv_unpack<float>(nrows, c->NFRE, buffer_ext, land, wavnum_ext, cgroup_ext, omosnh2kd_ext, depth_ext, u_ext, v_ext, (hipStream_t)stream),
           launch_proenv_unpack<double>(nrows, c->NFRE, buffer_ext, land, wavnum_ext, cgroup_ext, omosnh2kd_ext, depth_ext, u_ext, v_ext, (hipStream_t)stream));
  HIPCHK(hipGetLastError());
  return 0;
}

int ecwam_hip_halo_counts(ecwam_hip_ctx* c, int* n_send, int* n_recv) {
  if (!c || !n_send || !n_recv) return fail("ecwam_hip_halo_counts: null argument");
  *n_send = c->n_send; *n_recv = c->n_recv;
  return 0;
}

int ecwam_hip_comm_unique_id(void* id128) {
  if (!id128) return fail("ecwam_hip_comm_unique_id: null argument");
  if (rccl_load()) return 1;
  static_assert(sizeof(ncclUniqueId) == 128, "ncclUniqueId");
  NCCLCHK(g_rccl.GetUniqueId((ncclUniqueId*)id128));
  return 0;
}

int ecwam_hip_comm_init(ecwam_hip_ctx* c, const void* id128) {
  if (!c || !id128) return fail("ecwam_hip_comm_init: null argument");
  if (c->nranks < 2 && c->peer.empty()) return 0;
  if (rccl_load()) return 1;
  HIPCHK(hipSetDevice(c->device));
  if (c->comm) {
    if (c->comm_stream) HIPCHK(hipStreamSynchronize(c->comm_stream));
    (void)g_rccl.CommDestroy(c->comm);
    c->comm = nullptr;
    for (auto& q : c->slot) q.used = q.pending = false;
  }
  ncclUniqueId id;
  memcpy(&id, id128, sizeof(id));
  NCCLCHK(g_rccl.CommInitRank(&c->comm, c->nranks, id, c->rank));
  return 0;
}

int ecwam_hip_comm_count(ecwam_hip_ctx* c, int* nranks) {
  if (!c || !nranks) return fail("ecwam_hip_comm_count: null argument");
  *nranks = 0;
  if (!c->comm) return 0;
  NCCLCHK(g_rccl.CommCount(c->comm, nranks));
  return 0;
}

static ecwam_hip_ctx::HaloSlot* halo_slot(ecwam_hip_ctx* c, int rowlen) {
  ecwam_hip_ctx::HaloSlot* q = nullptr;
  for (auto& x : c->slot) if (x.rowlen == rowlen) { q = &x; break; }
  if (!q) for (auto& x : c->slot) if (x.rowlen == 0) { q = &x; break; }
  if (!q) { q = &c->slot[0]; for (auto& x : c->slot) if (x.age < q->age) q = &x; }
  q->rowlen = rowlen; q->age = ++c->slot_clock;
  return q;
}

static int halo_pack(ecwam_hip_ctx* c, ecwam_hip_ctx::HaloSlot* q, const void* fl, int rowlen, hipStream_t s) {
  const size_t need = (size_t)c->n_send * rowlen * c->real_bytes;
  if (!q->ev_packed) {
    HIPCHK(hipEventCreateWithFlags(&q->ev_packed, hipEventDisableTiming));
    HIPCHK(hipEventCreateWithFlags(&q->ev_done, hipEventDisableTiming));
  }
  if (q->used) HIPCHK(hipStreamWaitEvent(s, q->ev_done, 0));
  if (need > q->bytes) {
    if (q->buf) HIPCHK(hipFree(q->buf));
    q->buf = nullptr; q->bytes = 0;
    HIPCHK(hipMalloc(&q->buf, need));
    q->bytes = need;
  }
  if (c->n_send > 0) {
    DISPATCH(launch_pack<float>(fl, c->d_send_idx, c->n_send, rowlen, q->buf, s),
             launch_pack<double>(fl, c->d_send_idx, c->n_send, rowlen, q->buf, s));
    HIPCHK(hipGetLastError());
  }
  return 0;
}

int ecwam_hip_halo_start(ecwam_hip_ctx* c, void* fl, int rowlen, void* stream) {
  if (!c) return fail("null context");
  if (c->peer.empty()) return 0;
  if (!fl || rowlen < 1) return fail("ecwam_hip_halo_start: bad arguments");
  if (!c->comm) return fail("ecwam_hip_halo_start: no communicator (ecwam_hip_comm_init)");
  hipStream_t s = (hipStream_t)stream;
  HIPCHK(hipSetDevice(c->device));
  ecwam_hip_ctx::HaloSlot* q = halo_slot(c, rowlen);
// ... 114 lines not shown
```

ecwam_amd/csrc/implsch4a.hip:

```cpp
#include "implsch_v4_launch.h"
#include "implsch_adv_args.h"

template <typename T>
int launch_implsch4_adv(const void* tab, int kijs, int kijl, void* fl_out, const void* wvprpt, void* ff, void* intf, int* mij, void* xllws, void* fin,
                        double* w2n, const Implsch4AdvArgs* a, int NANG, int NFRE, int r1, int r2, int nh, int ext, hipStream_t s) {
  if (kijl - kijs <= 0) return 0;
  if (NFRE != V4_NFRE) return -1;
  V4Adv<T> adv;
  adv.f_in = (const T*)a->f_in; adv.klon = a->klon; adv.klat = a->klat; adv.kcor = a->kcor; adv.cg = (const T*)a->cg; adv.pt = (const T*)a->pt;
  adv.dirT = (const T*)a->dirT; adv.dirI = a->dirI; adv.xdella = (T)a->xdella; adv.delpro = (T)a->delpro; adv.m0 = a->m0; adv.m1 = a->m1;
  adv.gin = (const T*)a->gin; adv.delpro_lf = (T)a->delpro_lf; adv.gin_k = a->gin_k; adv.mlf = a->mlf; adv.obs = (const T*)a->obs;
#define V4_ARGS tab, kijs, kijl, fl_out, wvprpt, ff, intf, mij, xllws, fin, w2n, a->gfast, a->gfast_k, adv, s
#define V4_ADV_CASE(NA, PPV, R1V, R2V, NHV, LFOK)                                                                                         \
  if (NANG == NA && r1 == R1V && r2 == R2V && nh == NHV) {                                                                              \
    const int form = (a->gin ? 2 : 0) | (a->obs ? 4 : 0);                                                                               \
    if (!a->gin && a->mlf != 0) return -1;                                                                                              \
    if (form == 0) return ext ? launch4_adv<T, NA, PPV, R1V, R2V, NHV, true, 1>(V4_ARGS) : launch4_adv<T, NA, PPV, R1V, R2V, NHV, false, 1>(V4_ARGS); \
    if constexpr (!ECWAM_HIP_CTU_STRICT) {       \
      if (form == 4) return ext ? launch4_adv<T, NA, PPV, R1V, R2V, NHV, true, 5>(V4_ARGS) : launch4_adv<T, NA, PPV, R1V, R2V, NHV, false, 5>(V4_ARGS); \
      if constexpr (LFOK) {                                                                                                             \
        if (form == 2) return ext ? launch4_adv<T, NA, PPV, R1V, R2V, NHV, true, 3>(V4_ARGS) : launch4_adv<T, NA, PPV, R1V, R2V, NHV, false, 3>(V4_ARGS); \
        if (form == 6) return ext ? launch4_adv<T, NA, PPV, R1V, R2V, NHV, true, 7>(V4_ARGS) : launch4_adv<T, NA, PPV, R1V, R2V, NHV, false, 7>(V4_ARGS); \
      }                                                                                                                                 \
    }                                                                                                                                   \
    return -1;                                                                                                                          \
  }
  constexpr bool SP = sizeof(T) == 4;
  V4_ADV_CASE(36, 3, 1, 3, 8, true)
  if constexpr (SP) {
    V4_ADV_CASE(24, 5, 0, 2, 5, true)
    V4_ADV_CASE(12, 10, 0, 1, 3, true)
    V4_ADV_CASE(48, 2, 1, 4, 11, false)
  }
#undef V4_ADV_CASE
#undef V4_ARGS
  return -1;
}
template int launch_implsch4_adv<float>(const void*, int, int, void*, const void*, void*, void*, int*, void*, void*, double*, const Implsch4AdvArgs*, int, int, int, int, int, int, hipStream_t);
template int launch_implsch4_adv<double>(const void*, int, int, void*, const void*, void*, void*, int*, void*, void*, double*, const Implsch4AdvArgs*, int, int, int, int, int, int, hipStream_t);
int implsch4_adv_forms(int NANG, int real_bytes) {
  if (NANG != 48 && NANG != 36 && NANG != 24 && NANG != 12) return 0;
  if (real_bytes == 8 && NANG != 36) return 0;
  return 1 | (ECWAM_HIP_CTU_STRICT ? 0 : 4) | ((ECWAM_HIP_CTU_STRICT || NANG == 48) ? 0 : 2);
}
```

ecwam_amd/csrc/implsch_adv_args.h:

```cpp
#pragma once
struct Implsch4AdvArgs {
  const void* f_in;
  const int *klon, *klat, *kcor;
  const void* cg;
  const void* pt;
  const void* dirT;
  const int* dirI;
  double xdella, delpro;
  const void* gin;
  double delpro_lf;
  int gin_k, mlf;
  const void* obs;
  void* gfast;
  int gfast_k;
  int m0, m1;
};
```

ecwam_amd/csrc/implsch_v4.h:

```cpp
#pragma once
#include "ctu.h"

#define V4_NFRE 36
#ifdef ECWAM_HIP_DIAGNOSTICS
#define V4_PHASE_EXIT(k) do { if (tb.DBG_SKIP == (k)) return; } while (0)
#else
#define V4_PHASE_EXIT(k) do { } while (0)
#endif
#if defined(V4_CHECK) && V4_CHECK
#include <cassert>
#define V4_CHK(c) assert(c)
#else
#define V4_CHK(c) do { } while (0)
#endif
#define V4_NSTG 4
#define V4_NS(nang) ((V4_NFRE + (nang) / 2 - 1) / ((nang) / 2))
#define V4_PLN(pp, nang) ((pp) * ((nang) > V4_NFRE ? (nang) : V4_NFRE))
#define V4_NFAC 6

#define V4SYNC() WSYNC()
#define V4_WPE_MIN(T) (sizeof(T) == 4 ? 2 : 1)

template <typename T>
using V2 = T __attribute__((ext_vector_type(2)));
// ... 158 lines not shown
    v = v4_allsum1<G, T>(v, r);
  }
  spw[m] = v;
}

template <typename T, int NSH, int r>
__device__ __forceinline__ V2<T> v4_at(const T* row, const int (&sh)[2 * NSH + 1]) {
  if constexpr ((r & 1) == 0) {
    return *reinterpret_cast<const V2<T>*>(row + sh[r / 2 + NSH]);
  } else {
    return V2<T>{row[sh[(r - 1) / 2 + NSH] + 1], row[sh[(r + 1) / 2 + NSH]]};
  }
}

template <bool ON, typename T>
__device__ __forceinline__ T v4_vreg(T x) {
  if constexpr (ON && sizeof(T) == 4) {
    T r;
    asm("v_mov_b32 %0, %1" : "=v"(r) : "s"(x));
    return r;
  } else return x;
}
template <typename T>
__device__ __forceinline__ void v4_pin6(const T (&r)[6]) { asm volatile("" :: "s"(r[0]), "s"(r[1]), "s"(r[2]), "s"(r[3]), "s"(r[4]), "s"(r[5])); }
template <typename T>
__device__ __forceinline__ void v4_pin10(T (&r)[20], int o) {
  asm volatile("" :: "s"(r[o]), "s"(r[o + 1]), "s"(r[o + 2]), "s"(r[o + 3]), "s"(r[o + 4]), "s"(r[o + 5]), "s"(r[o + 6]), "s"(r[o + 7]), "s"(r[o + 8]), "s"(r[o + 9]));
}
template <typename T, int NSH, int ra, int rb>
__device__ __forceinline__ V2<T> v4_win(const T* row, const int (&sh)[2 * NSH + 1], V2<T> own, T ca, T cb) {
  static_assert(ra - rb == 1 || rb - ra == 1, "adjacent rotations");
  constexpr int lo = ra < rb ? ra : rb;
  constexpr int e = (lo >= 0) ? (lo / 2) * 2 : -(((-lo) + 1) / 2) * 2;
  static_assert(e / 2 + NSH >= 0 && e / 2 + 1 + NSH <= 2 * NSH, "shift table");
  const V2<T> a = (e == 0) ? own : *reinterpret_cast<const V2<T>*>(row + sh[e / 2 + NSH]);
  const V2<T> b = (e + 2 == 0) ? own : *reinterpret_cast<const V2<T>*>(row + sh[e / 2 + 1 + NSH]);
  const T el[4] = {a.x, a.y, b.x, b.y};
  return V2<T>{ca * el[ra - e] + cb * el[rb - e], ca * el[ra - e + 1] + cb * el[rb - e + 1]};
}

template <typename T, int NSH, int r>
__device__ __forceinline__ V2<T> v4_pair(const V2<T> (&A)[2 * NSH + 1]) {
  static_assert(r >= -2 * NSH && r <= 2 * NSH, "window");
  if constexpr ((r & 1) == 0) return A[NSH + r / 2];
  else return __builtin_shufflevector(A[NSH + (r - 1) / 2], A[NSH + (r + 1) / 2], 1, 2);
}
template <typename T, int NSH, int NH, int d>
__device__ __forceinline__ void v4_sat_taps(const V2<T> (&A)[2 * NSH + 1], const T (&wt)[NH + 1], V2<T>& acc) {
  if constexpr (d <= NH) {
    acc += wt[NH - d] * (v4_pair<T, NSH, -d>(A) + v4_pair<T, NSH, d>(A));
    v4_sat_taps<T, NSH, NH, d + 1>(A, wt, acc);
  }
}

template <typename T, int PP, bool RARE>
__device__ __forceinline__ void v4_stresso(const DevTab<T>& tb, T* sSC, int lane, bool LLPHIWA) {
  if constexpr (PP <= 3) {
    stresso_stage<T, PP, RARE>(tb, sSC, lane, LLPHIWA);
  } else {
    stresso_stage<T, 3, RARE>(tb, sSC, lane, LLPHIWA);
    WSYNC();
    v4_stresso<T, PP - 3, RARE>(tb, sSC + 3 * NSC, lane, LLPHIWA);
  }
}

template <typename T, int NANG_, int PP_>
struct V4Ctx {
  int lane, p, j;
  T* tile;
  int own;
  T* fac4;
  T* sq;
  T* zcn;
  T* c;
  V4Rot<T> rot;
  V2<T> sinth, costh;
  T rDFIM, rDFIMOFR, rDFIMFR, rZPIFR, rRHOWG, rCOFRM4, rFLMAX;
};
enum { Q4_BSC = 0, Q4_SBO, Q4_CINV, Q4_WAVNUM };

template <typename T>
struct V4Adv {
  const T* f_in;
  const int* klon;
  const int* klat;
  const int* kcor;
  const T* cg;
  const T* pt;
  const T* dirT;
  const int* dirI;
  T xdella, delpro;
  const T* gin;
  T delpro_lf;
  int gin_k, mlf;
  const T* obs;
  int m0, m1;
};
template <typename T, int NANG, int PP, int MODE, int NSCR>
__device__ __forceinline__ void v4_advect_tile(const V4Adv<T>& A, int ij0, int n, int lane, T* __restrict__ sT, T* __restrict__ sScr) {
  constexpr int NFRE = V4_NFRE, N = NANG * NFRE, RS = PP * NANG, VEC = 16 / (int)sizeof(T), NC = NFRE / VEC, NVL = N / VEC;
  constexpr int NFULL = NVL / 64, NREM = NVL - 64 * NFULL, NTS = (PP * NREM + 63) / 64, NCH = NFULL * PP + NTS, NRND = NFULL + NTS, D = 3;
  constexpr int PTW = 20;
  typedef T VT __attribute__((ext_vector_type(VEC)));
  typedef int I4 __attribute__((ext_vector_type(4)));
  T* sB = sScr;
  T* sPt = sB + PP * 5 * NFRE;
  T* sK = sPt + PP * PTW;
  constexpr bool LF = (MODE & 3) == 3;
  constexpr bool OBS = (MODE & 4) != 0;
  constexpr int NB = OBS ? 11 : 8;
  static_assert(MODE & 1, "modes: 1 plain, 3 fast waves, + 4 obstructions");
  constexpr int NKW = NANG * 4 + 4 + (LF ? NANG * 2 : 0);
  int* sI = reinterpret_cast<int*>(sK + NKW);
  int* sD = sI + PP * 16;
  static_assert((PP * 5 * NFRE + PP * PTW + NKW) * sizeof(T) + (PP * 16 + NANG * 4) * sizeof(int) <= NSCR * sizeof(T), "LDS scratch of the advecting load");
  for (int i = lane; i < PP * PTW; i += 64) {
    const int q = i / PTW, e = i - q * PTW;
    const T* g = A.pt + (size_t)(ij0 + (q < n ? q : n - 1)) * 12;
    T v = T(0);
    if (e < 12) v = g[e];
    else if (e < 18) v = T(1) - g[e - 6];
    else if (e == 18) v = g[0] * g[2];
    else v = A.xdella * g[2];
    if (e == 1) v = m_abs(v);
    sPt[i] = v;
  }
  for (int i = lane; i < PP * 16; i += 64) {
    const int q = i >> 4, e = i & 15;
    const int ijq = ij0 + (q < n ? q : n - 1);
    int v = ijq;
    if (e >= 1 && e <= 2) v = A.klon[(size_t)ijq * 2 + (e - 1)];
    if (e >= 3 && e <= 6) v = A.klat[(size_t)ijq * 4 + (e - 3)];
    if (e >= 7 && e <= 14) v = A.kcor[(size_t)ijq * 8 + (e - 7)];
    sI[i] = v;
  }
  for (int i = lane; i < NKW; i += 64) {
    const T v = A.dirT[i];
    const int e = i & 3;
    sK[i] = i >= NANG * 4 + 4 ? T(2) * v : (i >= NANG * 4 ? v : (e < 2 ? T(2) * v : m_abs(v)));
  }
  for (int i = lane; i < NANG * 4; i += 64) sD[i] = A.dirI[i];
  WSYNC();
  VT buf[D][NB];
  struct Rnd {
    int q;
    int k, m;
    int jx0, jy0, kc;
    unsigned off0, off6, off7;
    const char* src;
    const char* srcl;
    unsigned rnb;
  };
  Rnd R[NRND];
  auto round_of = [&](int c) { return c < NFULL * PP ? c / PP : NFULL + (c - NFULL * PP); };
  auto make_round = [&](int r) {
    Rnd o;
    int w;
    o.q = 0;
    if (r < NFULL) {
      w = lane + 64 * r;
    } else {
      int t = lane + 64 * (r - NFULL);
      t = t < PP * NREM ? t : PP * NREM - 1;
      o.q = t / (NREM > 0 ? NREM : 1);
      w = 64 * NFULL + (t - o.q * NREM);
    }
    o.k = w / NC;
    o.m = (w - o.k * NC) * VEC;
    const I4 dk = *reinterpret_cast<const I4*>(sD + 4 * o.k);
    o.jx0 = dk.x & 1; o.jy0 = (dk.x >> 1) & 1; o.kc = (dk.x >> 2) & 3;
    const bool fromg = LF && o.m < A.gin_k;
    const int rk = fromg ? A.gin_k : NFRE;
    o.src = reinterpret_cast<const char*>(fromg ? A.gin : A.f_in);
    o.rnb = (unsigned)(NANG * rk * (int)sizeof(T));
    o.off0 = (unsigned)((o.k * rk + o.m) * (int)sizeof(T));
    o.off6 = (unsigned)((dk.y * rk + o.m) * (int)sizeof(T));
    o.off7 = (unsigned)((dk.z * rk + o.m) * (int)sizeof(T));
    o.srcl = o.src + o.off0;
    return o;
  };
  auto ld = [](const char* p) { return *reinterpret_cast<const VT*>(p); };
  auto issue = [&](int c, VT (&b)[NB]) {
    const bool full = c < NFULL * PP;
    const int r = round_of(c);
    if (!full || c % PP == 0) R[r] = make_round(r);
    const Rnd& o = R[r];
    const int q = full ? c % PP : o.q;
    const int* iq = sI + q * 16;
    const int row0 = full ? ij0 + (q < n ? q : n - 1) : iq[0];
    const char* own = o.src + (size_t)(unsigned)row0 * o.rnb;
    b[0] = ld(own + o.off0);
    b[1] = ld(o.srcl + (size_t)(unsigned)iq[1 + o.jx0] * o.rnb);
    b[2] = ld(o.srcl + (size_t)(unsigned)iq[3 + 2 * o.jy0] * o.rnb);
    b[3] = ld(o.srcl + (size_t)(unsigned)iq[4 + 2 * o.jy0] * o.rnb);
    b[4] = ld(o.srcl + (size_t)(unsigned)iq[7 + 2 * o.kc] * o.rnb);
    b[5] = ld(o.srcl + (size_t)(unsigned)iq[8 + 2 * o.kc] * o.rnb);
    b[6] = ld(own + o.off6);
    b[7] = ld(own + o.off7);
    if constexpr (OBS) {
      const T* ob = A.obs + (size_t)row0 * 8 * NFRE + o.m;
      b[8] = *reinterpret_cast<const VT*>(ob + (2 + o.jx0) * NFRE);
      b[9] = *reinterpret_cast<const VT*>(ob + o.jy0 * NFRE);
      b[10] = *reinterpret_cast<const VT*>(ob + (4 + o.kc) * NFRE);
    }
  };
  const bool carry = A.m0 > 0 || A.m1 < NFRE;
  const T cmtodeg = sK[NANG * 4];
  auto finish = [&](int c, const VT (&b)[NB]) {
    const Rnd& o = R[round_of(c)];
    const int q = c < NFULL * PP ? c % PP : o.q, k = o.k, m = o.m;
    T r[VEC];
    const int jx0 = o.jx0, jy0 = o.jy0, kc = o.kc;
    const T* pq = sPt + q * PTW;
    const T zd = pq[0], acpm1 = pq[1], ga = pq[2], tanph = pq[3], wl = pq[6 + jy0], omwl = pq[12 + jy0], wc = pq[8 + kc], omwc = pq[14 + kc];
    const VT kk = *reinterpret_cast<const VT*>(sK + 4 * k);
    const T kk2 = sizeof(T) == 4 ? kk[2 % VEC] : sK[4 * k + 2], kk3 = sizeof(T) == 4 ? kk[3 % VEC] : sK[4 * k + 3];
#if ECWAM_HIP_CTU_STRICT
    T a2, b2, p2, m2;
    {
#pragma clang fp contract(off)
      const T tsp2 = tanph * kk[0], tsm2 = tanph * kk[1];
      a2 = m_max(tsp2, T(0)); p2 = m_max(-tsp2, T(0)); b2 = m_max(-tsm2, T(0)); m2 = m_max(tsm2, T(0));
    }
#else
    T ab2, p2, m2;
    ctu_fast_dir<T>(tanph, kk[0], kk[1], ab2, p2, m2);
    T ab2_lf = ab2, p2_lf = p2, m2_lf = m2;
    if constexpr (LF) ctu_fast_dir<T>(tanph, sK[NANG * 4 + 4 + 2 * k], sK[NANG * 4 + 4 + 2 * k + 1], ab2_lf, p2_lf, m2_lf);
#endif
    const T* bb = sB + q * 5 * NFRE + m;
    const VT bha = *reinterpret_cast<const VT*>(bb + jx0 * NFRE), bhb = *reinterpret_cast<const VT*>(bb + (1 - jx0) * NFRE),
             bya = *reinterpret_cast<const VT*>(bb + (2 + jy0) * NFRE), byb = *reinterpret_cast<const VT*>(bb + (3 - jy0) * NFRE),
             bc0 = *reinterpret_cast<const VT*>(bb + 4 * NFRE);
#if ECWAM_HIP_CTU_STRICT
    static_assert(!LF && !OBS, "the strict build of the weights has the plain form only");
#pragma unroll
    for (int i = 0; i < VEC; i += 2) {
#define P2(a) V2<T>{a[i], a[i + 1]}
      const V2<T> rr = ctu_w8_stencil_abs<T>(P2(bha), P2(bhb), P2(bya), P2(byb), P2(bc0), kk2, kk3, acpm1, zd, A.xdella, ga, A.delpro, cmtodeg, wl, omwl,
                                             wc, omwc, a2, b2, p2, m2, P2(b[0]), P2(b[1]), P2(b[2]), P2(b[3]), P2(b[4]), P2(b[5]), P2(b[6]), P2(b[7]));
#undef P2
      r[i] = rr.x; r[i + 1] = rr.y;
    }
#else
    const T zdg = pq[18], xdg = pq[19];
#pragma unroll
    for (int i = 0; i < VEC; i += 2) {
#define P2(a) V2<T>{a[i], a[i + 1]}
      const bool lf0 = LF && (m + i) < A.mlf, lf1 = LF && (m + i + 1) < A.mlf;
      CtuFastW8<T> w = ctu_fast_w8<T>(P2(bha), P2(bhb), P2(bya), P2(byb), P2(bc0), kk2, kk3, zd, A.xdella, ga, zdg, xdg, wl, omwl, wc, omwc,
                                      V2<T>{lf0 ? ab2_lf : ab2, lf1 ? ab2_lf : ab2}, V2<T>{lf0 ? p2_lf : p2, lf1 ? p2_lf : p2},
                                      V2<T>{lf0 ? m2_lf : m2, lf1 ? m2_lf : m2});
      if constexpr (OBS) {
        w.wlon = w.wlon * P2(b[8]); w.wlat1 = w.wlat1 * P2(b[9]); w.wlat2 = w.wlat2 * P2(b[9]); w.wcor1 = w.wcor1 * P2(b[10]); w.wcor2 = w.wcor2 * P2(b[10]);
      }
      const V2<T> rr = ctu_fast_apply<T>(w, P2(b[0]), P2(b[1]), P2(b[2]), P2(b[3]), P2(b[4]), P2(b[5]), P2(b[6]), P2(b[7]));
#undef P2
      r[i] = rr.x; r[i + 1] = rr.y;
    }
#endif
    if (carry) {
#pragma unroll
      for (int i = 0; i < VEC; i++)
        if (m + i < A.m0 || m + i >= A.m1) r[i] = b[0][i];
    }
    T* d = sT + m * RS + q * NANG + k;
#pragma unroll
    for (int i = 0; i < VEC; i++) d[i * RS] = r[i];
  };
#pragma unroll
  for (int c = 0; c < D - 1 && c < NCH; c++) issue(c, buf[c % D]);
  __builtin_amdgcn_sched_barrier(0);
  for (int i = lane; i < PP * NFRE; i += 64) {
    const int q = i / NFRE, m = i - q * NFRE;
    const int* iq = sI + q * 16;
    const T* pq = sPt + q * PTW;
    T cgl[2], cgy0[2], cgy1[2];
#pragma unroll
    for (int ic = 0; ic < 2; ic++) {
      cgl[ic] = A.cg[(size_t)iq[1 + ic] * NFRE + m];
      cgy0[ic] = A.cg[(size_t)iq[3 + 2 * ic] * NFRE + m];
      cgy1[ic] = A.cg[(size_t)iq[4 + 2 * ic] * NFRE + m];
    }
    const T wl[2] = {pq[6], pq[7]}, dp[2] = {pq[4], pq[5]};
    const CtuBase<T> b = ctu_base(A.cg[(size_t)iq[0] * NFRE + m], cgl, cgy0, cgy1, wl, dp);
    T* o = sB + q * 5 * NFRE + m;
#if ECWAM_HIP_CTU_STRICT
    o[0] = m_abs(b.h[0]); o[NFRE] = m_abs(b.h[1]); o[2 * NFRE] = m_abs(b.hy[0]); o[3 * NFRE] = m_abs(b.hy[1]); o[4 * NFRE] = b.cg0;
#else
    ctu_fast_planes<T>(b, pq[1], ((LF && m < A.mlf) ? A.delpro_lf : A.delpro) * sK[NANG * 4], o, o + NFRE, o + 2 * NFRE, o + 3 * NFRE);
    o[4 * NFRE] = b.cg0;
#endif
  }
  WSYNC();
#pragma unroll
  for (int c = 0; c < NCH; c++) {
    if (c + D - 1 < NCH) issue(c + D - 1, buf[(c + D - 1) % D]);
    __builtin_amdgcn_sched_barrier(0);
    finish(c, buf[c % D]);
    __builtin_amdgcn_sched_barrier(0);
  }
  WSYNC();
}

template <typename T>
__device__ T stress_gc_row(const DevTab<T>& tb, int l16, bool run, T ANG_GC, T USTAR, T Z0, T Z0MIN, T HALP, T RNFAC) {
  const T XLAMA = T(0.25), XLAMB = T(4.0);
  const int NS = ns_gc_d(tb, USTAR);
  const T t = USTAR * (Z0MIN / Z0);
  const T TAUWCG_MIN = t * t;
  const T XLAMBDA = T(1) + XLAMA * m_tanh(XLAMB * m_pow4(USTAR));
  const T LOGXL = m_log(XLAMBDA);
  const T hc = HALP * tb.C2OSQRTVG_GC[NS];
  const T ZABHRC = ANG_GC * tb.BETAMAXOXKAPPA2 * hc;
  const T CONST = tb.LLNORMAGAM ? RNFAC * tb.BMAXOKAP * hc / m_max(USTAR, tb.EPSUS) : T(0);
  T acc = T(0);
  for (int I = NS + l16;; I += 16) {
    const bool act = run && I <= tb.NWAV_GC;
    if (__builtin_amdgcn_ballot_w64(act) == 0ull) break;
    if (act) {
      const T X = USTAR * tb.CM_GC[I];
      const T XLOG = m_log(tb.XK_GC[I] * Z0) + tb.XKAPPA / (X + tb.ZALP);
      const T ZLOG = m_min(XLOG - LOGXL, T(0));
      const T ZLOG2X = ZLOG * ZLOG * X;
      const T GAM_W = ZLOG2X * ZLOG2X * m_exp(XLOG) * tb.OM3GMKM_GC[I];
      const T ZN = CONST * tb.XKMSQRTVGOC2_GC[I] * GAM_W;
      const T GAMNORMA = (T(1) + tb.RN1_RN * ZN) / (T(1) + ZN);
      const T wt = (I == NS) ? tb.DELKCC_GC_NS[NS] * tb.OMXKM3_GC[NS] : tb.DELKCC_OMXKM3_GC[I];
      acc = acc + (GAM_W * wt) * GAMNORMA;
    }
  }
  const T TAUWCG = v4_rowsum<T>(V2<T>{acc, T(0)}).x;
  return m_max(ZABHRC * TAUWCG, TAUWCG_MIN);
}
template <typename T>
__device__ void taut_z0_b_rows(const DevTab<T>& tb, int l16, int IUSFG, T HALP, T UTOP, T COSDIFF, T TAUW, T RNFAC, T& USTAR, T& Z0, T& Z0B,
                               T& CHRNCK) {
  const int NITER = 18;
  const T PMAX = T(0.99), Z0MIN = T(0.000001);
  const T US2TOTAUW = T(1) + tb.EPS1;
  const T RNUKAPPAM1 = (T(0.04) * tb.RNU) / tb.XKAPPA;
  const T PCE_GC = T(0.001) * IUSFG + (1 - IUSFG) * T(0.005);
  const T TAUWACT = m_max(TAUW * COSDIFF, tb.EPSMIN);
  const bool LLCOSDIFF = (COSDIFF > T(0.9));
  T ALPHAOG = T(0);
  if (tb.LLCAPCHNK) ALPHAOG = chnkmin(tb, UTOP) * tb.GM1;
  const T USMAX = m_max(-T(0.21339) + T(0.093698) * UTOP - T(0.0020944) * UTOP * UTOP + T(5.5091E-5) * UTOP * UTOP * UTOP, T(0.03));
  const T TAUWEFF = m_min(TAUWACT * US2TOTAUW, USMAX * USMAX);
  T X, CDFG;
  if (IUSFG == 0) {
    const T ALPHAGM1 = tb.ALPHA * tb.GM1;
    if (UTOP < T(1)) CDFG = T(0.002);
    else if (LLCOSDIFF) {
      const T um = m_max(USTAR, tb.EPSUS);
      X = m_min(TAUWACT / (um * um), PMAX);
      T ZCHAR = m_min(ALPHAGM1 * USTAR * USTAR / m_sqrt(T(1) - X), T(0.05) * m_exp(-T(0.05) * (UTOP - T(35.))));
      ZCHAR = m_min(ZCHAR, tb.ALPHAMAX);
      CDFG = tb.ACDLIN + tb.BCDLIN * m_sqrt(ZCHAR) * UTOP;
    } else CDFG = cdm_d(UTOP);
    USTAR = UTOP * m_sqrt(CDFG);
  }
  const T W1 = T(0.85) - T(0.05) * (m_tanh(T(10) * (UTOP - T(5))) + T(1));
  const T XKUTOP = tb.XKAPPA * UTOP;
  T USTOLD = USTAR;
  T TAUOLD = USTOLD * USTOLD;
  T TAUUNR = T(0);
  bool run = true;
  for (int ITER = 1; ITER <= NITER; ITER++) {
    if (__builtin_amdgcn_ballot_w64(run) == 0ull) break;
    const T Z0n = m_max(tb.XNLEV / (m_exp(m_min(XKUTOP / USTOLD, T(50))) - T(1)), Z0MIN);
    const T TAUV = RNUKAPPAM1 * USTOLD / Z0n;
    const T ANG_GC = tb.ANG_GC_A + tb.ANG_GC_B * m_tanh(tb.ANG_GC_C * TAUOLD);
    const T TAUUNRn = stress_gc_row(tb, l16, run, ANG_GC, USTAR, Z0n, Z0MIN, HALP, RNFAC);
    const T TAUNEW = TAUWEFF + TAUV + TAUUNRn;
    const T USTNEW = m_sqrt(TAUNEW);
    const T USTARn = W1 * USTOLD + (T(1) - W1) * USTNEW;
    if (run) {
// ... 1702 lines not shown
```

ecwam_amd/csrc/propag.hip:

```cpp
#include "dev.h"

#include "ctu.h"

template <typename T>
__global__ void __launch_bounds__(256) k_propags2(const DevTab<T>* __restrict__ tab, const T* __restrict__ f1, T* __restrict__ f3,
                                                  const int* __restrict__ klon, const int* __restrict__ klat,
                                                  const int* __restrict__ kcor, const T* __restrict__ w, int kijs, int kijl,
                                                  int m0, int m1, int copy_rest) {
  const int NANG = tab->NANG, NFRE = tab->NFRE, NR = tab->NFRE_RED;
  const int N = NANG * NFRE;
  const long long total = (long long)(kijl - kijs) * N;
  for (long long g = (long long)blockIdx.x * blockDim.x + threadIdx.x; g < total; g += (long long)gridDim.x * blockDim.x) {
    const int ij = kijs + (int)(g / N);
    const int e = (int)(g - (long long)(ij - kijs) * N);
    const int k = e / NFRE, m = e - k * NFRE;
    const size_t own = (size_t)ij * N;
    if (m < m0 || m >= m1) {
      if (copy_rest) f3[own + e] = f1[own + e];
      continue;
    }
    const int jx = tab->JXO[k][0], jy = tab->JYO[k][0], kc = tab->KCR[k][0];
    const int km = tab->KPM[k][0], kp = tab->KPM[k][2];
    const int ilon = klon[ij * 2 + jx];
    const int ilat1 = klat[(ij * 2 + jy) * 2 + 0], ilat2 = klat[(ij * 2 + jy) * 2 + 1];
// ... 1141 lines not shown
      (const T*)sinph, klon, klat, kcor, (const T*)wlat, (const T*)wcor, (const T*)cg, (const T*)cosphm1, order, kijs, kijl, m0, \
      m1, copy_rest, ntiles, (const T*)obs, mlf, (T)delpro_lf, in_k, (T*)gout, gout_k, (const T*)gin, gin_k, out_k
  int vw = W;
#ifdef ECWAM_HIP_DIAGNOSTICS
  { const char* e_ = getenv("ECWAM_HIP_OTF_VW"); if (e_) vw = atoi(e_); }
#endif
  if (gout && (gout_k % W != 0 || (uintptr_t)gout % 16 != 0)) gout = nullptr;
  if (out_k <= 0) out_k = NFRE;
  const bool vec = vw >= W && aligned && NFRE % W == 0 && in_k % W == 0 && out_k % W == 0 && (!gin || (gin_k % W == 0 && (uintptr_t)gin % 16 == 0));
  if (obs) {
    if (vec) { allow_lds(k_propags2_otf<T, W, true>, shmem); hipLaunchKernelGGL((k_propags2_otf<T, W, true>), dim3(grid), dim3(256), shmem, s, OTF_ARGS); }
    else { allow_lds(k_propags2_otf<T, 1, true>, shmem); hipLaunchKernelGGL((k_propags2_otf<T, 1, true>), dim3(grid), dim3(256), shmem, s, OTF_ARGS); }
  } else if (vec)
    { allow_lds(k_propags2_otf<T, W, false>, shmem); hipLaunchKernelGGL((k_propags2_otf<T, W, false>), dim3(grid), dim3(256), shmem, s, OTF_ARGS); }
  else if (vw >= 2 && aligned && NFRE % 2 == 0 && in_k % 2 == 0 && out_k % 2 == 0 && (!gin || gin_k % 2 == 0))
    { allow_lds(k_propags2_otf<T, 2, false>, shmem); hipLaunchKernelGGL((k_propags2_otf<T, 2, false>), dim3(grid), dim3(256), shmem, s, OTF_ARGS); }
  else
    { allow_lds(k_propags2_otf<T, 1, false>, shmem); hipLaunchKernelGGL((k_propags2_otf<T, 1, false>), dim3(grid), dim3(256), shmem, s, OTF_ARGS); }
#undef OTF_ARGS
}
template <typename T>
void launch_ctuwini_only(int n, int nland, const int* klat, const int* kcor, void* wlat, void* wcor, hipStream_t s) {
  if (n <= 0) return;
  hipLaunchKernelGGL(k_ctuwini<T>, dim3((n + 255) / 256), dim3(256), 0, s, n, nland, klat, kcor, (T*)wlat, (T*)wcor);
}
template <typename T>
void launch_propdot(const void* tab, int n, int nland, int irefra, const int* kxlt, const void* zdello, double xdella, const void* cosph,
                    const int* klon, const int* klat, const void* wlat, const void* cosphm1, const void* depth, const void* ue,
                    const void* ve, void* refr, hipStream_t s) {
  if (n <= 0) return;
  hipLaunchKernelGGL(k_propdot<T>, dim3((n + 127) / 128), dim3(128), 0, s, (const DevTab<T>*)tab, n, nland, irefra, kxlt,
                     (const T*)zdello, (T)xdella, (const T*)cosph, klon, klat, (const T*)wlat, (const T*)cosphm1, (const T*)depth,
                     (const T*)ue, (const T*)ve, (T*)refr);
}
template <typename T>
void launch_curmask(int n, int NANG, int slot, const int* cflfail, void* refr, hipStream_t s) {
  if (n <= 0) return;
  hipLaunchKernelGGL(k_curmask<T>, dim3((n + 255) / 256), dim3(256), 0, s, n, NANG, slot, cflfail, (T*)refr);
}
template <typename T>
void launch_propags2_gen(const void* tab, int irefra, const void* f1, void* f3, int ngy, double delpro, const int* kxlt,
                         const void* zdello, double xdella, const void* cosph, const void* sinph, const int* klon, const int* klat,
                         const int* kcor, const void* wlat, const void* wcor, const void* cg, const void* om, const void* wn,
                         const void* cosphm1, const void* refr, int* cflfail, int slot, int kijs, int kijl, int m0, int m1,
                         int copy_rest, int dims, const void* obs, hipStream_t s) {
  const int NANG = dims >> 16, NFRE = (dims >> 8) & 0xFF, NR = dims & 0xFF;
  const int n = kijl - kijs;
  if (n <= 0) return;
  const int ntiles = (n + GEN_TP - 1) / GEN_TP;
  const size_t shmem = GEN_TP * (sizeof(CtuPoint<T>) + 16 * sizeof(int)) +
                       ((size_t)GEN_TP * (obs && f1 ? 19 : 11) * NFRE + (size_t)GEN_TP * (REFR_W(NANG) + 12) + 4 * NANG + 2 * NFRE) * sizeof(T) + 12 * NANG * sizeof(int) + 16;
  const int grid = ntiles < 256 * 16 ? ntiles : 256 * 16;
  constexpr int W = VecOf<T>::W;
  const bool aligned = ((uintptr_t)f1 % 16 == 0) && ((uintptr_t)f3 % 16 == 0);
#define GEN_ARGS                                                                                                               \
  (const DevTab<T>*)tab, irefra, (const T*)f1, (T*)f3, ngy, (T)delpro, kxlt, (const T*)zdello, (T)xdella, (const T*)cosph,       \
      (const T*)sinph, klon, klat, kcor, (const T*)wlat, (const T*)wcor, (const T*)cg, (const T*)om, (const T*)wn,             \
      (const T*)cosphm1, (const T*)refr, cflfail, slot, kijs, kijl, m0, m1, copy_rest, ntiles, (const T*)obs
  int vw = 2;
#ifdef ECWAM_HIP_DIAGNOSTICS
  { const char* e_ = getenv("ECWAM_HIP_GEN_VW"); if (e_) vw = atoi(e_); }
#endif
  const bool v4 = vw >= W && aligned && NFRE % W == 0 && NR % W == 0 && m0 % W == 0 && m1 % W == 0;
  const bool v2 = vw >= 2 && aligned && NFRE % 2 == 0 && NR % 2 == 0 && m0 % 2 == 0 && m1 % 2 == 0;
  if (!f1)
    { allow_lds(k_propags2_gen<T, 1, true, false>, shmem); hipLaunchKernelGGL((k_propags2_gen<T, 1, true, false>), dim3(grid), dim3(256), shmem, s, GEN_ARGS); }
  else if (obs) {
    if (v2) { allow_lds(k_propags2_gen<T, 2, false, true>, shmem); hipLaunchKernelGGL((k_propags2_gen<T, 2, false, true>), dim3(grid), dim3(256), shmem, s, GEN_ARGS); }
    else { allow_lds(k_propags2_gen<T, 1, false, true>, shmem); hipLaunchKernelGGL((k_propags2_gen<T, 1, false, true>), dim3(grid), dim3(256), shmem, s, GEN_ARGS); }
  } else if (v4)
    { allow_lds(k_propags2_gen<T, W, false, false>, shmem); hipLaunchKernelGGL((k_propags2_gen<T, W, false, false>), dim3(grid), dim3(256), shmem, s, GEN_ARGS); }
  else if (v2)
    { allow_lds(k_propags2_gen<T, 2, false, false>, shmem); hipLaunchKernelGGL((k_propags2_gen<T, 2, false, false>), dim3(grid), dim3(256), shmem, s, GEN_ARGS); }
  else
    { allow_lds(k_propags2_gen<T, 1, false, false>, shmem); hipLaunchKernelGGL((k_propags2_gen<T, 1, false, false>), dim3(grid), dim3(256), shmem, s, GEN_ARGS); }
#undef GEN_ARGS
}
template <typename T>
void launch_newwind(const void* tab, int n, void* ff, const void* ffn, int icode_wnd, hipStream_t s) {
  if (n <= 0) return;
  hipLaunchKernelGGL(k_newwind<T>, dim3((n + 255) / 256), dim3(256), 0, s, (const DevTab<T>*)tab, n, (T*)ff, (const T*)ffn, icode_wnd);
}
template <typename T>
__global__ void k_ctu_prep(const DevTab<T>* __restrict__ tab, int kijs, int kijl, int ngy, T delpro, T delpro_lf, const int* __restrict__ kxlt,
                           const T* __restrict__ zdello, T xdella, const T* __restrict__ cosph, const T* __restrict__ sinph,
                           const T* __restrict__ wlat, const T* __restrict__ wcor, const T* __restrict__ cosphm1, T* __restrict__ pt,
                           T* __restrict__ dirT, int* __restrict__ dirI) {
  const int NANG = tab->NANG;
  if (blockIdx.x == 0) {
    const T DELTH0 = T(0.25) * delpro / tab->DELTH;
    for (int k = threadIdx.x; k < NANG; k += blockDim.x) {
      T a, b;
      ctu_dirfac(tab, k, DELTH0, T(1), a, b);
      dirT[4 * k] = a; dirT[4 * k + 1] = b; dirT[4 * k + 2] = tab->SINTH[k]; dirT[4 * k + 3] = tab->COSTH[k];
      dirI[4 * k] = tab->JXO[k][0] | (tab->JYO[k][0] << 1) | (tab->KCR[k][0] << 2);
      dirI[4 * k + 1] = tab->KPM[k][0]; dirI[4 * k + 2] = tab->KPM[k][2]; dirI[4 * k + 3] = 0;
      if (delpro_lf > T(0)) {
        ctu_dirfac(tab, k, T(0.25) * delpro_lf / tab->DELTH, T(1), a, b);
        dirT[4 * NANG + 4 + 2 * k] = a; dirT[4 * NANG + 4 + 2 * k + 1] = b;
      }
    }
    if (threadIdx.x == 0) {
      dirT[4 * NANG] = T(360.0) / tab->CIRC;
      dirT[4 * NANG + 1] = dirT[4 * NANG + 2] = dirT[4 * NANG + 3] = T(0);
    }
  }
  for (int ij = kijs + blockIdx.x * blockDim.x + threadIdx.x; ij < kijl; ij += gridDim.x * blockDim.x) {
    const CtuPoint<T> p = ctu_point(ij, ngy, kxlt, zdello, xdella, cosph, sinph, wlat, wcor, cosphm1);
    T* o = pt + (size_t)ij * 12;
    o[0] = p.zd; o[1] = p.cpm1; o[2] = p.ga; o[3] = p.tanph; o[4] = p.dp[0]; o[5] = p.dp[1]; o[6] = p.wl[0]; o[7] = p.wl[1];
    o[8] = p.wc[0]; o[9] = p.wc[1]; o[10] = p.wc[2]; o[11] = p.wc[3];
  }
}
template <typename T>
void launch_ctu_prep(const void* tab, int kijs, int kijl, int ngy, double delpro, double delpro_lf, const int* kxlt, const void* zdello, double xdella,
                     const void* cosph, const void* sinph, const void* wlat, const void* wcor, const void* cosphm1, void* pt, void* dirT, int* dirI,
                     hipStream_t s) {
  const int n = kijl - kijs;
  hipLaunchKernelGGL(k_ctu_prep<T>, dim3(n > 0 ? grid_for(n) : 1), dim3(256), 0, s, (const DevTab<T>*)tab, kijs, kijl, ngy, (T)delpro, (T)delpro_lf, kxlt,
                     (const T*)zdello, (T)xdella, (const T*)cosph, (const T*)sinph, (const T*)wlat, (const T*)wcor, (const T*)cosphm1, (T*)pt,
                     (T*)dirT, dirI);
}
template <typename T>
__global__ void k_nosource(const DevTab<T>* __restrict__ tab, long long e0, long long e1, T* __restrict__ fl1, T* __restrict__ xllws, int kijs,
                           int kijl, int* __restrict__ mij) {
  const T eps = tab->EPSMIN;
  for (long long g = e0 + (long long)blockIdx.x * blockDim.x + threadIdx.x; g < e1; g += (long long)gridDim.x * blockDim.x) {
    if (fl1) fl1[g] = m_max(fl1[g], eps);
    xllws[g] = T(0);
  }
  for (int ij = kijs + blockIdx.x * blockDim.x + threadIdx.x; ij < kijl; ij += gridDim.x * blockDim.x) mij[ij] = tab->NFRE;
}
template <typename T>
void launch_nosource(const void* tab, int kijs, int kijl, int rowlen, void* fl1, void* xllws, int* mij, hipStream_t s) {
  if (kijl <= kijs) return;
  const long long e0 = (long long)kijs * rowlen, e1 = (long long)kijl * rowlen;
  hipLaunchKernelGGL(k_nosource<T>, dim3(grid_for(e1 - e0)), dim3(256), 0, s, (const DevTab<T>*)tab, e0, e1, (T*)fl1, (T*)xllws, kijs, kijl, mij);
}
template <typename T>
void launch_c2p(const void* ch, void* pt, int nproma, int nchnk, int npts, int n2, int n3, hipStream_t s) {
  long long total = (long long)npts * n2 * n3;
  if (total <= 0) return;
  hipLaunchKernelGGL(k_chunks_to_points<T>, dim3(grid_for(total)), dim3(256), 0, s, (const T*)ch, (T*)pt, nproma, nchnk, npts, n2, n3);
}
template <typename T>
void launch_p2c(const void* pt, void* ch, int nproma, int nchnk, int npts, int n2, int n3, hipStream_t s) {
  long long total = (long long)nchnk * nproma * n2 * n3;
  if (total <= 0) return;
  hipLaunchKernelGGL(k_points_to_chunks<T>, dim3(grid_for(total)), dim3(256), 0, s, (const T*)pt, (T*)ch, nproma, nchnk, npts, n2, n3);
}
template <typename T>
void launch_copy_freq_range(const void* src, void* dst, int n, int NANG, int NFRE, int m0, int m1, int dst_nfre, hipStream_t s) {
  long long total = (long long)n * NANG * (m1 - m0);
  if (total <= 0) return;
  hipLaunchKernelGGL(k_copy_freq_range<T>, dim3(grid_for(total)), dim3(256), 0, s, (const T*)src, (T*)dst, n, NANG, NFRE, m0, m1,
                     dst_nfre);
}
template <typename T>
void launch_pack(const void* fl, const int* idx, int n, int rowlen, void* buf, hipStream_t s) {
  long long total = (long long)n * rowlen;
  if (total <= 0) return;
  hipLaunchKernelGGL(k_pack_rows<T>, dim3(grid_for(total)), dim3(256), 0, s, (const T*)fl, idx, n, rowlen, (T*)buf);
}

template <typename T>
void launch_proenv_pack(int n, int NFRE, const void* wvprpt, const void* om, const void* depth, const void* u, const void* v, void* buf, hipStream_t s) {
  const long long total = (long long)n * (3 * NFRE + 3);
  if (total <= 0) return;
  hipLaunchKernelGGL(k_proenv_pack<T>, dim3(grid_for(total)), dim3(256), 0, s, n, NFRE, (const T*)wvprpt, (const T*)om, (const T*)depth, (const T*)u,
                     (const T*)v, (T*)buf);
}
template <typename T>
void launch_proenv_unpack(int nrows, int NFRE, const void* buf, const void* land, void* wn, void* cg, void* om, void* dep, void* u, void* v, hipStream_t s) {
  const long long total = (long long)(nrows + 1) * (3 * NFRE + 3);
  hipLaunchKernelGGL(k_proenv_unpack<T>, dim3(grid_for(total)), dim3(256), 0, s, nrows, NFRE, (const T*)buf, (const T*)land, (T*)wn, (T*)cg, (T*)om,
                     (T*)dep, (T*)u, (T*)v);
}

#define INST(T)                                                                                                                   \
  template void launch_proenv_pack<T>(int, int, const void*, const void*, const void*, const void*, const void*, void*, hipStream_t); \
  template void launch_proenv_unpack<T>(int, int, const void*, const void*, void*, void*, void*, void*, void*, void*, hipStream_t); \
  template void launch_propags2<T>(const void*, const void*, void*, const int*, const int*, const int*, const void*, int, int,   \
                                   int, int, int, int, hipStream_t);                                                              \
  template void launch_ctuw<T>(const void*, int, int, int, double, int, int, const int*, const void*, double, const void*,       \
                               const void*, const int*, const int*, const int*, void*, void*, const void*, const void*, void*,   \
                               int*, int, const void*, hipStream_t);                                                              \
  template void launch_newwind<T>(const void*, int, void*, const void*, int, hipStream_t);                                        \
  template void launch_ctu_prep<T>(const void*, int, int, int, double, double, const int*, const void*, double, const void*, const void*, const void*, const void*, const void*, void*, void*, int*, hipStream_t);\
  template void launch_nosource<T>(const void*, int, int, int, void*, void*, int*, hipStream_t);                                  \
  template void launch_propdot<T>(const void*, int, int, int, const int*, const void*, double, const void*, const int*,         \
                                  const int*, const void*, const void*, const void*, const void*, const void*, void*, hipStream_t); \
  template void launch_ctuwini_only<T>(int, int, const int*, const int*, void*, void*, hipStream_t);                               \
  template void launch_curmask<T>(int, int, int, const int*, void*, hipStream_t);                                                      \
  template void launch_propags2_gen<T>(const void*, int, const void*, void*, int, double, const int*, const void*, double,        \
                                       const void*, const void*, const int*, const int*, const int*, const void*, const void*,   \
                                       const void*, const void*, const void*, const void*, const void*, int*, int, int, int, int, \
                                       int, int, int, const void*, hipStream_t);                                                                    \
  template void launch_propags2_otf<T>(const void*, const void*, void*, int, int, double, const int*, const void*, double,        \
                                       const void*, const void*, const int*, const int*, const int*, const void*, const void*,   \
                                       const void*, const void*, const int*, int, int, int, int, int, int, const void*, int, double,   \
                                       int, void*, int, const void*, int, int, hipStream_t);                                                                              \
  template void launch_c2p<T>(const void*, void*, int, int, int, int, int, hipStream_t);                                          \
  template void launch_p2c<T>(const void*, void*, int, int, int, int, int, hipStream_t);                                          \
  template void launch_copy_freq_range<T>(const void*, void*, int, int, int, int, int, int, hipStream_t);                             \
  template void launch_pack<T>(const void*, const int*, int, int, void*, hipStream_t);
INST(float)
INST(double)
```

ecwam_amd/lib.py:

```python
from __future__ import annotations

import ctypes as C
import os

import numpy as np

from .tables import JTOT_TAUHF, Tables

HERE = os.path.dirname(os.path.abspath(__file__))
LIBPATH = os.environ.get("ECWAM_HIP_LIB") or os.path.join(HERE, "lib", "libecwam_hip.so")

_INT_FIELDS_1 = ["nang", "nfre", "nfre_red", "nfre_odd", "idelt"]
_PARAM_LAYOUT = (
    [(n, C.c_int) for n in _INT_FIELDS_1]
    + [("ximp", C.c_double)]
    + [(n, C.c_int) for n in ["iphys", "isnonlin", "irefra", "icode", "llgcbz0", "llnormagam", "llcapchnk", "lbiwbk", "licerun",
                               "lmaskice", "lwamrsetci", "lciwa1", "lciwa2", "lciwa3", "lciscal", "lwvflx_snl", "lwflux",
                               "lwfluxout", "lwnemocou", "lwcou", "lwcouast", "lwnemocouwrs", "lwnemotauoc", "lwnemocousend",
                               "lwnemocoustk", "lwnemocoustrn"]]
    + [(n, C.c_double) for n in ["g", "gm1", "pi", "zpi", "zpi4gm1", "zpi4gm2", "epsmin", "rowater", "rowaterm1", "epsus",
                                  "epsu10", "acd", "bcd", "acdlin", "bcdlin", "cdmax", "tauocmin", "tauocmax", "phiepsmin",
                                  "phiepsmax", "wsemean_min", "circ", "r_earth", "fratio", "wetail", "frtail", "wp1tail", "fric",
                                  "delth", "flogsprdm1", "xkappa", "xnlev", "rnu", "rnum", "betamaxoxkappa2", "bmaxokap",
                                  "gamnconst", "zalp", "alpha", "alphamin", "alphamax", "chnkmin_u", "alphapmax", "tauwshelter", "dthrn_a",
                                  "dthrn_u", "tailfactor", "tailfactor_pm", "ang_gc_a", "ang_gc_b", "ang_gc_c", "rn1_rn", "swellf",
                                  "swellf2", "swellf3", "swellf4", "swellf5", "swellf6", "swellf7", "swellf7m1", "z0rat",
                                  "z0tubmax", "abmin", "abmax", "sdsbr", "ssdsc2", "ssdsc3", "ssdsc4", "ssdsc5", "ssdsc6", "miche"]]
    + [("nsdsnth", C.c_int), ("ipsat", C.c_int)]
    + [(n, C.c_double) for n in ["egrcrv", "afcrv", "bfcrv", "x0tauhf", "eps1", "flmin", "cithrsh", "ciblock", "cithrsh_tail",
                                  "zalpwrs", "bathymax", "wspmin", "wspmin_reset_tauw", "cdis", "delta_sdis", "cdisvis"]]
    + [("idamping", C.c_int)]
    + [(n, C.c_double) for n in ["cdicwa", "zalpfacb", "zalpfacx"]]
    + [("lwnemocouibr", C.c_int), ("zibrw_thrsh", C.c_double), ("nict", C.c_int), ("nich", C.c_int)]
    + [(n, C.c_double) for n in ["ticmin", "dtic", "dhic", "hicmin"]]
    + [("mfrstlw", C.c_int), ("mlsthg", C.c_int), ("kfrh", C.c_int), ("dal1", C.c_double), ("dal2", C.c_double),
       ("nwav_gc", C.c_int), ("xlogkratiom1_gc", C.c_double), ("sqrtgosurft", C.c_double)]
)


class Params(C.Structure):
    _fields_ = _PARAM_LAYOUT


_TABLE_NAMES = ["fr", "dfim", "dfimofr", "dfimfr", "dfim_sim", "rhowg_dfim", "zpifr", "fr5", "cofrm4", "flmax", "th", "costh",
                "sinth", "wtauhf", "swellft", "ikp", "ikp1", "ikm", "ikm1", "af11", "k1w", "k2w", "k11w", "k21w", "inlcoef",
                "rnlcoef", "indicessat", "satweights", "kpm", "jxo", "jyo", "kcr", "xk_gc", "xkm_gc", "omega_gc", "omxkm3_gc",
                "cm_gc", "c2osqrtvg_gc", "xkmsqrtvgoc2_gc", "om3gmkm_gc", "delkcc_gc_ns", "delkcc_omxkm3_gc", "cideac"]
_INT_TABLES = {"ikp", "ikp1", "ikm", "ikm1", "k1w", "k2w", "k11w", "k21w", "inlcoef", "indicessat", "kpm", "jxo", "jyo", "kcr"}


class TablePtrs(C.Structure):
    _fields_ = [(n, C.c_void_p) for n in _TABLE_NAMES]


EXPORTS = ["ecwam_hip_last_error", "ecwam_hip_abi_version", "ecwam_hip_selftest", "ecwam_hip_create", "ecwam_hip_destroy", "ecwam_hip_set_obstructions", "ecwam_hip_propags2",
           "ecwam_hip_ctuw", "ecwam_hip_propags2_otf", "ecwam_hip_propags2_otf_split", "ecwam_hip_propags2_otf_fast", "ecwam_hip_set_fastwave_copy", "ecwam_hip_copy_freq_range", "ecwam_hip_propdot", "ecwam_hip_ctuw_refra", "ecwam_hip_propags2_refra", "ecwam_hip_implsch", "ecwam_hip_implsch_generation_used", "ecwam_hip_device_tables", "ecwam_hip_implsch_reserve", "ecwam_hip_propags2_implsch_supported", "ecwam_hip_propags2_implsch", "ecwam_hip_outbs", "ecwam_hip_outbs_sepwisw", "ecwam_hip_outbs_partition", "ecwam_hip_outbs_extremes", "ecwam_hip_outbs_absolute", "ecwam_hip_set_second_order", "ecwam_hip_outbs_second_order", "ecwam_hip_outwnorm", "ecwam_hip_newwind", "ecwam_hip_newwind_icode", "ecwam_hip_nosource", "ecwam_hip_host_register", "ecwam_hip_host_unregister", "ecwam_hip_chunks_to_points",
           "ecwam_hip_points_to_chunks", "ecwam_hip_member_scatter", "ecwam_hip_member_gather", "ecwam_hip_pack_rows", "ecwam_hip_unpack_rows", "ecwam_hip_halo_setup", "ecwam_hip_halo_counts", "ecwam_hip_comm_unique_id",
           "ecwam_hip_comm_init", "ecwam_hip_comm_count", "ecwam_hip_halo_start", "ecwam_hip_halo_finish", "ecwam_hip_halo_pack_host", "ecwam_hip_halo_unpack_host", "ecwam_hip_proenvhalo_pack", "ecwam_hip_proenvhalo_unpack", "ecwam_hip_malloc", "ecwam_hip_free",
           "ecwam_hip_memcpy_h2d", "ecwam_hip_memcpy_d2h", "ecwam_hip_memset", "ecwam_hip_sync", "ecwam_hip_queue_create", "ecwam_hip_queue_destroy",
           "ecwam_hip_queue_wait_for"]

ABI_VERSION = 6
_lib = None


def load() -> C.CDLL:
    global _lib
    if _lib is not None:
        return _lib
    if not os.path.exists(LIBPATH):
        raise RuntimeError(f"{LIBPATH} not found: the HIP extension is not built (run `python -m ecwam_amd.build` or "
                           "__graft_entry__.build()); there is no CPU fallback")
    import torch
    lib = C.CDLL(LIBPATH)
    lib.ecwam_hip_last_error.restype = C.c_char_p
    lib.ecwam_hip_abi_version.restype = C.c_int
    if lib.ecwam_hip_abi_version() != ABI_VERSION:
        raise RuntimeError(f"{LIBPATH}: ABI version {lib.ecwam_hip_abi_version()} but this binding is written for {ABI_VERSION}; rebuild the extension")
    for name in EXPORTS[1:]:
        getattr(lib, name).restype = C.c_int
    vp, ci, cd = C.c_void_p, C.c_int, C.c_double
    lib.ecwam_hip_create.argtypes = [C.POINTER(Params), C.POINTER(TablePtrs), ci, ci, C.POINTER(vp)]
    lib.ecwam_hip_destroy.argtypes = [vp]
    lib.ecwam_hip_selftest.argtypes = [ci]
    lib.ecwam_hip_set_obstructions.argtypes = [vp, vp, ci]
    lib.ecwam_hip_propags2.argtypes = [vp, vp, vp, vp, vp, vp, vp, ci, ci, ci, ci, ci, vp]
    lib.ecwam_hip_ctuw.argtypes = [vp, ci, ci, ci, cd, ci, ci, vp, vp, cd, vp, vp, vp, vp, vp, vp, vp, vp, vp, vp, vp, vp]
    lib.ecwam_hip_propags2_otf.argtypes = [vp, vp, vp, ci, ci, cd, vp, vp, cd, vp, vp, vp, vp, vp, vp, vp, vp, vp, vp, ci, ci, ci, ci, ci, vp]
    lib.ecwam_hip_propags2_otf_split.argtypes = [vp, vp, vp, ci, ci, cd, cd, ci, ci, vp, ci, vp, vp, cd, vp, vp, vp, vp, vp, vp, vp, vp, vp, vp, ci, ci, ci, ci, ci, vp]
    lib.ecwam_hip_propags2_otf_fast.argtypes = [vp, vp, vp, ci, ci, cd, cd, ci, ci, vp, ci, ci, vp, ci, vp, vp, cd, vp, vp, vp, vp, vp, vp, vp, vp, vp, vp, ci, ci, ci, ci, ci, vp]
    lib.ecwam_hip_set_fastwave_copy.argtypes = [vp, vp, ci]
    lib.ecwam_hip_propags2_implsch_supported.argtypes = [vp]
    lib.ecwam_hip_propags2_implsch.argtypes = [vp, vp, vp, ci, ci, cd, vp, vp, cd, vp, vp, vp, vp, vp, vp, vp, vp, vp, ci, ci, ci, ci, vp, vp, vp, vp, vp, vp,
                                               cd, ci, vp, ci, ci, vp]
    lib.ecwam_hip_copy_freq_range.argtypes = [vp, vp, vp, ci, ci, ci, ci, vp]
    lib.ecwam_hip_propdot.argtypes = [vp, ci, ci, vp, vp, cd, vp, vp, vp, vp, vp, vp, vp, vp, vp, vp]
    lib.ecwam_hip_ctuw_refra.argtypes = [vp, ci, ci, ci, cd, ci, ci, vp, vp, cd, vp, vp, vp, vp, vp, vp, vp, vp, vp, vp, vp, vp, ci, ci, vp, vp]
    lib.ecwam_hip_propags2_refra.argtypes = [vp, vp, vp, ci, ci, cd, vp, vp, cd, vp, vp, vp, vp, vp, vp, vp, vp, vp, vp, vp, vp, ci, ci, ci, ci, ci, ci, vp]
    lib.ecwam_hip_implsch.argtypes = [vp, ci, ci, vp, vp, vp, vp, vp, vp, vp, vp, vp]
    lib.ecwam_hip_device_tables.argtypes = [vp]
    lib.ecwam_hip_device_tables.restype = vp
    lib.ecwam_hip_implsch_reserve.argtypes = [vp, ci]
    lib.ecwam_hip_implsch_generation_used.argtypes = [vp]
    lib.ecwam_hip_outbs.argtypes = [vp, ci, ci, vp, cd, vp, vp]
    lib.ecwam_hip_outbs_sepwisw.argtypes = [vp, ci, ci, vp, vp, vp, vp, ci, cd, vp, vp]
    lib.ecwam_hip_outbs_partition.argtypes = [vp, ci, ci, vp, vp, vp, vp, vp, ci, cd, vp, vp]
    lib.ecwam_hip_outbs_extremes.argtypes = [vp, ci, ci, vp, vp, vp, ci, vp, vp]
    lib.ecwam_hip_outbs_absolute.argtypes = [vp, ci, ci, vp, vp, vp, vp, vp, ci, cd, vp, vp, vp]
    lib.ecwam_hip_set_second_order.argtypes = [vp, ci, cd, cd, ci, vp, vp, vp, vp, vp, vp, vp]
    lib.ecwam_hip_outbs_second_order.argtypes = [vp, ci, ci, vp, vp, vp, vp, vp, vp, cd, cd, vp, vp, vp]
    lib.ecwam_hip_outwnorm.argtypes = [vp, vp, ci, ci, cd, C.POINTER(C.c_double), vp]
    lib.ecwam_hip_newwind.argtypes = [vp, ci, vp, vp, vp]
    lib.ecwam_hip_newwind_icode.argtypes = [vp, ci, vp, vp, ci, vp]
    lib.ecwam_hip_nosource.argtypes = [vp, ci, ci, vp, vp, vp, vp]
    lib.ecwam_hip_host_register.argtypes = [vp, vp, C.c_ulonglong]
    lib.ecwam_hip_host_unregister.argtypes = [vp, vp]
    lib.ecwam_hip_chunks_to_points.argtypes = [vp, vp, vp, ci, ci, ci, ci, ci, vp]
    lib.ecwam_hip_points_to_chunks.argtypes = [vp, vp, vp, ci, ci, ci, ci, ci, vp]
    lib.ecwam_hip_member_scatter.argtypes = [vp, vp, vp, ci, ci, ci, ci, C.c_longlong, C.c_longlong, ci, vp]
    lib.ecwam_hip_member_gather.argtypes = [vp, vp, vp, ci, ci, ci, ci, C.c_longlong, C.c_longlong, ci, vp]
    lib.ecwam_hip_pack_rows.argtypes = [vp, vp, vp, ci, vp, vp]
    lib.ecwam_hip_unpack_rows.argtypes = [vp, vp, ci, vp, ci, vp]
    lib.ecwam_hip_halo_setup.argtypes = [vp, ci, ci, ci, vp, vp, vp, vp, vp]
    lib.ecwam_hip_halo_counts.argtypes = [vp, C.POINTER(ci), C.POINTER(ci)]
    lib.ecwam_hip_comm_unique_id.argtypes = [vp]
    lib.ecwam_hip_comm_init.argtypes = [vp, vp]
    lib.ecwam_hip_comm_count.argtypes = [vp, C.POINTER(ci)]
    lib.ecwam_hip_halo_start.argtypes = [vp, vp, ci, vp]
    lib.ecwam_hip_halo_finish.argtypes = [vp, vp]
    lib.ecwam_hip_halo_pack_host.argtypes = [vp, vp, ci, vp, vp]
    lib.ecwam_hip_halo_unpack_host.argtypes = [vp, vp, ci, vp, vp]
    lib.ecwam_hip_proenvhalo_pack.argtypes = [vp, ci, vp, vp, vp, vp, vp, vp, vp]
    lib.ecwam_hip_proenvhalo_unpack.argtypes = [vp, ci, vp, vp, vp, vp, vp, vp, vp, vp, vp]
    _lib = lib
    return lib


def make_params(t: Tables) -> Params:
    c = t.cfg
    p = Params()
    for name, typ in _PARAM_LAYOUT:
        if hasattr(c, name) and name not in ("wspmin", "rnu", "rnum"):
            v = getattr(c, name)
        elif name == "r_earth":
            v = t.R
        else:
            v = getattr(t, name.upper())
        setattr(p, name, int(v) if typ is C.c_int else float(v))
    return p


def make_tables(t: Tables):
    T = t.dtype
    keep = []
    tp = TablePtrs()
    one_based = {"indicessat": 1, "kpm": 1}
    for name in _TABLE_NAMES:
        a = getattr(t, name.upper())
        if name in _INT_TABLES:
            a = np.ascontiguousarray(np.asarray(a) + one_based.get(name, 0), dtype=np.int32)
        else:
            a = np.ascontiguousarray(a, dtype=T)
        keep.append(a)
        setattr(tp, name, a.ctypes.data_as(C.c_void_p))
    assert t.WTAUHF.size == JTOT_TAUHF
    return tp, keep
```

include/ecwam_hip.h:

```cpp
#ifndef ECWAM_HIP_H
#define ECWAM_HIP_H

#ifdef __cplusplus
extern "C" {
#endif

#define ECWAM_HIP_MAXANG 48
#define ECWAM_HIP_ABI_VERSION 6
#define ECWAM_HIP_MAXFRE 48
#define ECWAM_HIP_MAXMC 56
#define ECWAM_HIP_MAXTAP 47
#define ECWAM_HIP_MAXGC 96
#define ECWAM_HIP_IAB 200
#define ECWAM_HIP_JTOT_TAUHF 19
#define ECWAM_HIP_NFF 16
#define ECWAM_HIP_NINTF 16
#define ECWAM_HIP_NWPR 5

typedef struct ecwam_hip_params {
  int nang, nfre, nfre_red, nfre_odd;
  int idelt;
  double ximp;
  int iphys, isnonlin, irefra, icode;
  int llgcbz0, llnormagam, llcapchnk, lbiwbk, licerun, lmaskice, lwamrsetci;
// ... 20 lines not shown
  double dal1, dal2;
  int nwav_gc;
  double xlogkratiom1_gc, sqrtgosurft;
} ecwam_hip_params;

typedef struct ecwam_hip_tables {
  const void *fr, *dfim, *dfimofr, *dfimfr, *dfim_sim, *rhowg_dfim, *zpifr, *fr5, *cofrm4, *flmax;
  const void *th, *costh, *sinth;
  const void *wtauhf;
  const void *swellft;
  const int *ikp, *ikp1, *ikm, *ikm1;
  const void *af11;
  const int *k1w, *k2w, *k11w, *k21w;
  const int *inlcoef;
  const void *rnlcoef;
  const int *indicessat;
  const void *satweights;
  const int *kpm, *jxo, *jyo, *kcr;
  const void *xk_gc, *xkm_gc, *omega_gc, *omxkm3_gc, *cm_gc, *c2osqrtvg_gc, *xkmsqrtvgoc2_gc, *om3gmkm_gc, *delkcc_gc_ns,
      *delkcc_omxkm3_gc;
  const void *cideac;
} ecwam_hip_tables;

typedef struct ecwam_hip_ctx ecwam_hip_ctx;

const char *ecwam_hip_last_error(void);
int ecwam_hip_abi_version(void);
int ecwam_hip_selftest(int device);

int ecwam_hip_create(const ecwam_hip_params *p, const ecwam_hip_tables *t, int real_bytes, int device, ecwam_hip_ctx **out);
int ecwam_hip_destroy(ecwam_hip_ctx *ctx);

int ecwam_hip_set_obstructions(ecwam_hip_ctx *ctx, const void *obs, int n);

int ecwam_hip_propags2(ecwam_hip_ctx *ctx, const void *f1, void *f3, const int *klon, const int *klat, const int *kcor,
                       const void *w, int kijs, int kijl, int nd3s, int nd3e, int copy_rest, void *stream);

int ecwam_hip_ctuw(ecwam_hip_ctx *ctx, int n, int nland, int ngy, double delpro, int mstart, int mend, const int *kxlt,
                   const void *zdello, double xdella, const void *cosph, const void *sinph, const int *klon, const int *klat,
                   const int *kcor, void *wlat, void *wcor, const void *cgroup_ext, const void *cosphm1_ext, void *w,
                   int *cflfail, void *stream);

int ecwam_hip_propags2_otf(ecwam_hip_ctx *ctx, const void *f1, void *f3, int n, int ngy, double delpro, const int *kxlt,
                           const void *zdello, double xdella, const void *cosph, const void *sinph, const int *klon,
                           const int *klat, const int *kcor, const void *wlat, const void *wcor, const void *cgroup_ext,
                           const void *cosphm1_ext, const int *order, int kijs, int kijl, int nd3s, int nd3e, int copy_rest,
                           void *stream);

int ecwam_hip_propags2_otf_split(ecwam_hip_ctx *ctx, const void *f1, void *f3, int n, int ngy, double delpro, double delpro_lf,
                                 int ifrelfmax, int in_nfre, void *gout, int gout_nfre, const int *kxlt, const void *zdello, double xdella, const void *cosph,
                                 const void *sinph, const int *klon, const int *klat, const int *kcor, const void *wlat,
                                 const void *wcor, const void *cgroup_ext, const void *cosphm1_ext, const int *order, int kijs,
                                 int kijl, int nd3s, int nd3e, int copy_rest, void *stream);
int ecwam_hip_propags2_otf_fast(ecwam_hip_ctx *ctx, const void *f1, void *f3, int n, int ngy, double delpro, double delpro_lf,
                                int ifrelfmax, int in_nfre, const void *gin, int gin_nfre, int out_nfre, void *gout, int gout_nfre,
                                const int *kxlt, const void *zdello, double xdella, const void *cosph, const void *sinph,
                                const int *klon, const int *klat, const int *kcor, const void *wlat, const void *wcor,
                                const void *cgroup_ext, const void *cosphm1_ext, const int *order, int kijs, int kijl, int nd3s,
                                int nd3e, int copy_rest, void *stream);
int ecwam_hip_set_fastwave_copy(ecwam_hip_ctx *ctx, void *g, int g_nfre);
int ecwam_hip_copy_freq_range(ecwam_hip_ctx *ctx, const void *src, void *dst, int n, int m_first, int m_last, int dst_nfre,
                              void *stream);

int ecwam_hip_propdot(ecwam_hip_ctx *ctx, int n, int nland, const int *kxlt, const void *zdello, double xdella,
                      const void *cosph, const int *klon, const int *klat, const void *wlat, const void *cosphm1_ext,
                      const void *depth_ext, const void *u_ext, const void *v_ext, void *refr, void *stream);
int ecwam_hip_ctuw_refra(ecwam_hip_ctx *ctx, int n, int nland, int ngy, double delpro, int mstart, int mend, const int *kxlt,
                         const void *zdello, double xdella, const void *cosph, const void *sinph, const int *klon,
                         const int *klat, const int *kcor, void *wlat, void *wcor, const void *cgroup_ext,
                         const void *omosnh2kd_ext, const void *wavnum_ext, const void *cosphm1_ext, void *refr,
                         int llcflcuroff, int range, int *cflfail, void *stream);
int ecwam_hip_propags2_refra(ecwam_hip_ctx *ctx, const void *f1, void *f3, int n, int ngy, double delpro, const int *kxlt,
                             const void *zdello, double xdella, const void *cosph, const void *sinph, const int *klon,
                             const int *klat, const int *kcor, const void *wlat, const void *wcor, const void *cgroup_ext,
                             const void *omosnh2kd_ext, const void *wavnum_ext, const void *cosphm1_ext, const void *refr,
                             int range, int kijs, int kijl, int nd3s, int nd3e, int copy_rest, void *stream);

int ecwam_hip_implsch(ecwam_hip_ctx *ctx, int kijs, int kijl, void *fl1, const void *wvprpt, void *ff, void *intf, int *mij,
                      void *xllws, double *wam2nemo, void *dbg, void *stream);
int ecwam_hip_implsch_generation_used(ecwam_hip_ctx *ctx);
const void *ecwam_hip_device_tables(ecwam_hip_ctx *ctx);
int ecwam_hip_implsch_reserve(ecwam_hip_ctx *ctx, int npts);

int ecwam_hip_propags2_implsch_supported(ecwam_hip_ctx *ctx);
int ecwam_hip_propags2_implsch(ecwam_hip_ctx *ctx, const void *f1, void *f3, int n, int ngy, double delpro, const int *kxlt, const void *zdello,
                               double xdella, const void *cosph, const void *sinph, const int *klon, const int *klat, const int *kcor,
                               const void *wlat, const void *wcor, const void *cgroup_ext, const void *cosphm1_ext, int kijs, int kijl,
                               int nd3s, int nd3e, const void *wvprpt, void *ff, void *intf, int *mij, void *xllws, double *wam2nemo,
                               double delpro_lf, int ifrelfmax, const void *gin, int gin_nfre, int flags, void *stream);

int ecwam_hip_outbs(ecwam_hip_ctx *ctx, int kijs, int kijl, const void *fl1, double zmiss, void *out, void *stream);
int ecwam_hip_outwnorm(ecwam_hip_ctx *ctx, const void *field, int stride, int n, double zmiss, double *result, void *stream);

int ecwam_hip_outbs_sepwisw(ecwam_hip_ctx *ctx, int kijs, int kijl, const void *fl1, const void *xllws, const void *wvprpt, const void *ff,
                            int flags, double zmiss, void *out, void *stream);

int ecwam_hip_outbs_partition(ecwam_hip_ctx *ctx, int kijs, int kijl, const void *fl1, const void *xllws, const int *mij, const void *wvprpt,
                              const void *ff, int flags, double zmiss, void *out, void *stream);

int ecwam_hip_outbs_extremes(ecwam_hip_ctx *ctx, int kijs, int kijl, const void *fl1, const void *wvprpt, const void *ff, int flags,
                             void *out, void *stream);

int ecwam_hip_outbs_absolute(ecwam_hip_ctx *ctx, int kijs, int kijl, const void *fl1, const void *wvprpt, const void *ucur, const void *vcur,
                             const void *ff, int flags, double zmiss, void *out, void *fl2nd, void *stream);

int ecwam_hip_set_second_order(ecwam_hip_ctx *ctx, int ndepth, double deptha, double depthd, int nmax, const int *im_p, const int *im_m,
                               const void *ta, const void *tb, const void *tc_ql, const void *tt_4m, const void *tt_4p);

int ecwam_hip_outbs_second_order(ecwam_hip_ctx *ctx, int kijs, int kijl, const void *fl1, const void *wvprpt, const void *depth,
                                 const void *ucur, const void *vcur, const void *ff, double sig, double zmiss, void *out, void *fl2nd,
                                 void *stream);

int ecwam_hip_newwind(ecwam_hip_ctx *ctx, int n, void *ff, const void *ff_next, void *stream);
int ecwam_hip_newwind_icode(ecwam_hip_ctx *ctx, int n, void *ff, const void *ff_next, int icode_wnd, void *stream);
int ecwam_hip_nosource(ecwam_hip_ctx *ctx, int kijs, int kijl, void *fl1, int *mij, void *xllws, void *stream);

int ecwam_hip_chunks_to_points(ecwam_hip_ctx *ctx, const void *chunked, void *points, int nproma, int nchnk, int npts,
                               int n2, int n3, void *stream);
int ecwam_hip_points_to_chunks(ecwam_hip_ctx *ctx, const void *points, void *chunked, int nproma, int nchnk, int npts,
                               int n2, int n3, void *stream);

int ecwam_hip_member_scatter(ecwam_hip_ctx *ctx, const void *chunked, void *rows, int nproma, int nchnk, int npts, int nm,
                             long long row_stride, long long row_off, int elem_bytes, void *stream);
int ecwam_hip_member_gather(ecwam_hip_ctx *ctx, const void *rows, void *chunked, int nproma, int nchnk, int npts, int nm,
                            long long row_stride, long long row_off, int elem_bytes, void *stream);

int ecwam_hip_pack_rows(ecwam_hip_ctx *ctx, const void *fl, const int *idx, int n, void *buf, void *stream);
int ecwam_hip_unpack_rows(ecwam_hip_ctx *ctx, const void *buf, int n, void *fl, int dst0, void *stream);

int ecwam_hip_halo_setup(ecwam_hip_ctx *ctx, int rank, int nranks, int npeers, const int *peer, const int *send_count,
                         const int *send_idx, const int *recv_dst0, const int *recv_count);
int ecwam_hip_halo_counts(ecwam_hip_ctx *ctx, int *n_send, int *n_recv);
int ecwam_hip_comm_unique_id(void *id128);
int ecwam_hip_comm_init(ecwam_hip_ctx *ctx, const void *id128);
int ecwam_hip_comm_count(ecwam_hip_ctx *ctx, int *nranks);
int ecwam_hip_halo_start(ecwam_hip_ctx *ctx, void *fl, int rowlen, void *stream);
int ecwam_hip_halo_finish(ecwam_hip_ctx *ctx, void *stream);
int ecwam_hip_halo_pack_host(ecwam_hip_ctx *ctx, const void *fl, int rowlen, void *host_send, void *stream);
int ecwam_hip_halo_unpack_host(ecwam_hip_ctx *ctx, void *fl, int rowlen, const void *host_recv, void *stream);

int ecwam_hip_proenvhalo_pack(ecwam_hip_ctx *ctx, int n, const void *wvprpt, const void *omosnh2kd, const void *depth,
                              const void *ucur, const void *vcur, void *buffer_ext, void *stream);
int ecwam_hip_proenvhalo_unpack(ecwam_hip_ctx *ctx, int nrows, const void *buffer_ext, const void *land, void *wavnum_ext,
                                void *cgroup_ext, void *omosnh2kd_ext, void *depth_ext, void *u_ext, void *v_ext, void *stream);

int ecwam_hip_malloc(ecwam_hip_ctx *ctx, unsigned long long bytes, void **dptr);
int ecwam_hip_free(ecwam_hip_ctx *ctx, void *dptr);
int ecwam_hip_memcpy_h2d(ecwam_hip_ctx *ctx, void *dst_dev, const void *src_host, unsigned long long bytes, void *stream);
int ecwam_hip_memcpy_d2h(ecwam_hip_ctx *ctx, void *dst_host, const void *src_dev, unsigned long long bytes, void *stream);
int ecwam_hip_memset(ecwam_hip_ctx *ctx, void *dst_dev, int value, unsigned long long bytes, void *stream);
int ecwam_hip_sync(ecwam_hip_ctx *ctx, void *stream);
int ecwam_hip_queue_create(ecwam_hip_ctx *ctx, void **queue);
int ecwam_hip_queue_destroy(ecwam_hip_ctx *ctx, void *queue);
int ecwam_hip_queue_wait_for(ecwam_hip_ctx *ctx, void *waiter, void *waited);
int ecwam_hip_host_register(ecwam_hip_ctx *ctx, void *host, unsigned long long bytes);
int ecwam_hip_host_unregister(ecwam_hip_ctx *ctx, void *host);

#ifdef __cplusplus
}
#endif
#endif
```

Measured before the change: 60.01 million grid-point spectral steps/s.

## Cache per-point advection tile tables across steps and load them as packed records

Replaces the per-call ctu_prep kernel and the in-kernel computation of CTU weight planes (which gathered neighbour group velocities via klon/klat/kcor) with a precomputed per-point record of planes, geometry terms and neighbour indices. The record is built by a new tile-tables kernel only when the geometry or timestep key changes, with invalidation hooks from the Python side, CTUW, halo setup and proenv unpack. The fused kernel then loads each point's record with 16-byte vector reads into LDS. The intent is to drop the scattered neighbour gathers and the repeated geometry precomputation from every step. In exchange it costs a larger per-point buffer and some risk of stale tables if an input changes in place without invalidation.

```diff
diff --git a/ecwam_amd/api.py b/ecwam_amd/api.py
--- a/ecwam_amd/api.py
+++ b/ecwam_amd/api.py
@@ -252,7 +252,19 @@
                 float(delpro if delpro_lf is None else delpro_lf), int(ifrelfmax),
                 None if gin is None else self._real(gin, (gin.shape[0], self.NANG, gin.shape[2]), "GIN"), 0 if gin is None else int(gin.shape[2]),
                 int(flags), _stream_ptr()]
+        held = [g[k] for k in ("kxlt", "zdello", "cosph", "sinph", "klon", "klat", "kcor", "wlat", "wcor", "cosphm1_ext")] + [cgroup_ext]
+        sig = tuple((id(t), t.data_ptr(), t._version) for t in held)
+        if sig != getattr(self, "_tile_sig", None):
+            self.tile_tables_invalidate()
+            self._tile_sig, self._tile_held = sig, held
         self._chk(self.lib.ecwam_hip_propags2_implsch(self._h, *args))
+
+    def tile_tables_invalidate(self) -> None:
+        self._tile_sig = None
+        self._chk(self.lib.ecwam_hip_tile_tables_invalidate(self._h))
+
+    def tile_tables_fills(self) -> int:
+        return int(self.lib.ecwam_hip_tile_tables_fills(self._h))
 
     def implsch_reserve(self, npts: int) -> None:
         self._chk(self.lib.ecwam_hip_implsch_reserve(self._h, int(npts)))
diff --git a/ecwam_amd/csrc/capi.hip b/ecwam_amd/csrc/capi.hip
--- a/ecwam_amd/csrc/capi.hip
+++ b/ecwam_amd/csrc/capi.hip
@@ -57,9 +57,20 @@
   void* fast_g = nullptr;
   int fast_gk = 0;
   std::string implsch_why;
-  void* adv_pt = nullptr;
-  size_t adv_pt_bytes = 0;
+  void* adv_rec = nullptr;
+  size_t adv_rec_bytes = 0;
   void* adv_dir = nullptr;
+  struct AdvKey {
+    const void* p[12] = {};
+    int n = 0, ngy = 0, mlf = 0;
+    double xdella = 0, delpro = 0, delpro_lf = 0;
+    bool operator==(const AdvKey& o) const {
+      for (int i = 0; i < 12; i++) if (p[i] != o.p[i]) return false;
+      return n == o.n && ngy == o.ngy && mlf == o.mlf && xdella == o.xdella && delpro == o.delpro && delpro_lf == o.delpro_lf;
+    }
+  } adv_key;
+  bool adv_valid = false, adv_filled = false;
+  unsigned long long adv_fills = 0;
   void* so_tab = nullptr;
   void* so_coef = nullptr;
   void* so_work = nullptr;
@@ -103,7 +114,7 @@
 template <typename T> int launch_implsch4(const void*, int, int, void*, const void*, void*, void*, int*, void*, void*, double*, void*, int, void*, int, int, int, int, int, int, hipStream_t);
 template <typename T> int launch_implsch4x(const void*, int, int, void*, const void*, void*, void*, int*, void*, void*, double*, void*, int, void*, int, int, int, int, int, int, hipStream_t);
 template <typename T> int launch_implsch4r(const void*, int, int, void*, const void*, void*, void*, int*, void*, void*, double*, void*, int, void*, int, int, int, int, int, int, hipStream_t);
-template <typename T> void launch_ctu_prep(const void*, int, int, int, double, double, const int*, const void*, double, const void*, const void*, const void*, const void*, const void*, void*, void*, int*, hipStream_t);
+template <typename T> void launch_tile_tables(const void*, int, int, int, double, double, int, const int*, const void*, double, const void*, const void*, const int*, const int*, const int*, const void*, const void*, const void*, const void*, void*, void*, int*, hipStream_t);
 template <typename T> int launch_implsch4_adv(const void*, int, int, void*, const void*, void*, void*, int*, void*, void*, double*, const Implsch4AdvArgs*, int, int, int, int, int, int, hipStream_t);
 int implsch4_adv_forms(int, int);
 int implsch4_fin_row();
@@ -507,7 +518,7 @@
   if (c->so_work) (void)hipFree(c->so_work);
   if (c->fin) (void)hipFree(c->fin);
   if (c->wi) (void)hipFree(c->wi);
-  if (c->adv_pt) (void)hipFree(c->adv_pt);
+  if (c->adv_rec) (void)hipFree(c->adv_rec);
   if (c->adv_dir) (void)hipFree(c->adv_dir);
   halo_release(c);
   delete c;
@@ -552,6 +563,7 @@
   if (n > 0 && (!kxlt || !zdello || !cosph || !sinph || !klon || !klat || !kcor || !wlat || !wcor || !cgroup_ext || !cosphm1_ext || !cflfail))
     return fail("ecwam_hip_ctuw: null pointer");
   if (c->obs && n > c->n_obs) return fail("ecwam_hip_ctuw: more points than the obstruction table holds");
+  c->adv_valid = false;
   hipStream_t s = (hipStream_t)stream;
   DISPATCH(launch_ctuw<float>(c->dtab, n, nland, ngy, delpro, mstart - 1, mend, kxlt, zdello, xdella, cosph, sinph, klon, klat, kcor, wlat, wcor, cgroup_ext, cosphm1_ext, w, cflfail, c->NANG, c->obs, s),
            launch_ctuw<double>(c->dtab, n, nland, ngy, delpro, mstart - 1, mend, kxlt, zdello, xdella, cosph, sinph, klon, klat, kcor, wlat, wcor, cgroup_ext, cosphm1_ext, w, cflfail, c->NANG, c->obs, s));
@@ -724,14 +736,15 @@
 }
 
 static bool fused_ok(const ecwam_hip_ctx* c);
+static size_t adv_rec_row(const ecwam_hip_ctx* c) { return (size_t)(5 * c->NFRE + 20) * c->real_bytes + 16 * sizeof(int); }
 static int adv_reserve(ecwam_hip_ctx* c, int npts) {
   if (!fused_ok(c) || !implsch4_adv_forms(c->NANG, c->real_bytes)) return 0;
-  const size_t need = (size_t)(npts > 0 ? npts : 0) * 12 * c->real_bytes;
-  if (need > c->adv_pt_bytes) {
-    if (c->adv_pt) HIPCHK(hipFree(c->adv_pt));
-    c->adv_pt = nullptr; c->adv_pt_bytes = 0;
-    HIPCHK(hipMalloc(&c->adv_pt, need));
-    c->adv_pt_bytes = need;
+  const size_t need = (size_t)(npts > 0 ? npts : 0) * adv_rec_row(c);
+  if (need > c->adv_rec_bytes) {
+    if (c->adv_rec) HIPCHK(hipFree(c->adv_rec));
+    c->adv_rec = nullptr; c->adv_rec_bytes = 0; c->adv_valid = false;
+    HIPCHK(hipMalloc(&c->adv_rec, need));
+    c->adv_rec_bytes = need;
   }
   if (!c->adv_dir) HIPCHK(hipMalloc(&c->adv_dir, (size_t)(6 * c->NANG + 4) * c->real_bytes + (size_t)4 * c->NANG * sizeof(int)));
   return 0;
@@ -808,15 +821,26 @@
   hipStream_t s = (hipStream_t)stream;
   if (kijl == kijs) return 0;
   if (int rc2 = implsch_reserve_on(c, kijl, s, false)) return rc2;
+  if (int rc2 = adv_reserve(c, n)) return rc2;
   const size_t dir_reals = (size_t)(6 * c->NANG + 4);
   int* dirI = reinterpret_cast<int*>(reinterpret_cast<char*>(c->adv_dir) + dir_reals * c->real_bytes);
   const double dlf = gin ? delpro_lf : 0.0;
-  DISPATCH(launch_ctu_prep<float>(c->dtab, kijs, kijl, ngy, delpro, dlf, kxlt, zdello, xdella, cosph, sinph, wlat, wcor, cosphm1_ext, c->adv_pt, c->adv_dir, dirI, s),
-           launch_ctu_prep<double>(c->dtab, kijs, kijl, ngy, delpro, dlf, kxlt, zdello, xdella, cosph, sinph, wlat, wcor, cosphm1_ext, c->adv_pt, c->adv_dir, dirI, s));
+  ecwam_hip_ctx::AdvKey key;
+  const void* kp[11] = {kxlt, zdello, cosph, sinph, klon, klat, kcor, wlat, wcor, cgroup_ext, cosphm1_ext};
+  for (int i = 0; i < 11; i++) key.p[i] = kp[i];
+  key.n = n; key.ngy = ngy; key.mlf = gin ? ifrelfmax : 0; key.xdella = xdella; key.delpro = delpro; key.delpro_lf = dlf;
+  if (!c->adv_valid || !(key == c->adv_key)) {
+    if (c->adv_filled) HIPCHK(hipDeviceSynchronize());
+    DISPATCH(launch_tile_tables<float>(c->dtab, n, c->NFRE, ngy, delpro, dlf, key.mlf, kxlt, zdello, xdella, cosph, sinph, klon, klat, kcor, wlat, wcor, cgroup_ext, cosphm1_ext, c->adv_rec, c->adv_dir, dirI, s),
+             launch_tile_tables<double>(c->dtab, n, c->NFRE, ngy, delpro, dlf, key.mlf, kxlt, zdello, xdella, cosph, sinph, klon, klat, kcor, wlat, wcor, cgroup_ext, cosphm1_ext, c->adv_rec, c->adv_dir, dirI, s));
+    HIPCHK(hipGetLastError());
+    HIPCHK(hipStreamSynchronize(s));
+    c->adv_key = key; c->adv_valid = true; c->adv_filled = true; c->adv_fills++;
+  }
   Implsch4AdvArgs a;
-  a.f_in = f1; a.klon = klon; a.klat = klat; a.kcor = kcor; a.cg = cgroup_ext; a.pt = c->adv_pt; a.dirT = c->adv_dir; a.dirI = dirI;
+  a.f_in = f1; a.rec = c->adv_rec; a.dirT = c->adv_dir; a.dirI = dirI;
   a.xdella = xdella; a.delpro = delpro; a.m0 = nd3s - 1; a.m1 = nd3e;
-  a.gin = gin; a.delpro_lf = dlf; a.gin_k = gin ? gin_nfre : 0; a.mlf = gin ? ifrelfmax : 0;
+  a.gin = gin; a.gin_k = gin ? gin_nfre : 0; a.mlf = gin ? ifrelfmax : 0;
   a.obs = c->obs;
   a.gfast = c->fast_g; a.gfast_k = c->fast_g ? c->fast_gk : 0;
   const int ext = (c->p.llnormagam || c->p.llgcbz0) ? 1 : 0;
@@ -828,6 +852,13 @@
   c->implsch_last = 4;
   return 0;
 }
+
+int ecwam_hip_tile_tables_invalidate(ecwam_hip_ctx* c) {
+  if (!c) return fail("null context");
+  c->adv_valid = false;
+  return 0;
+}
+long long ecwam_hip_tile_tables_fills(ecwam_hip_ctx* c) { return c ? (long long)c->adv_fills : -1; }
 
 int ecwam_hip_set_fastwave_copy(ecwam_hip_ctx* c, void* g, int g_nfre) {
   if (!c) return fail("null context");
@@ -857,12 +888,13 @@
     HIPCHK(hipMalloc(&c->wi, need_wi));
     c->wi_bytes = need_wi;
   }
-  return adv_reserve(c, npts);
+  return 0;
 }
 
 int ecwam_hip_implsch_reserve(ecwam_hip_ctx* c, int npts) {
   if (!c) return fail("ecwam_hip_implsch_reserve: null context");
-  return implsch_reserve_on(c, npts, nullptr, true);
+  if (int rc = implsch_reserve_on(c, npts, nullptr, true)) return rc;
+  return adv_reserve(c, npts);
 }
 
 int ecwam_hip_implsch_generation_used(ecwam_hip_ctx* c) { return c ? c->implsch_last : 0; }
@@ -1145,6 +1177,7 @@
   if (nranks < 1 || rank < 0 || rank >= nranks || npeers < 0 || (npeers > 0 && (!peer || !send_count || !recv_dst0 || !recv_count)))
     return fail("ecwam_hip_halo_setup: bad arguments");
   HIPCHK(hipSetDevice(c->device));
+  c->adv_valid = false;
   if (c->d_send_idx) { (void)hipFree(c->d_send_idx); c->d_send_idx = nullptr; }
   c->rank = rank; c->nranks = nranks;
   c->peer.assign(peer, peer + npeers); c->send_cnt.assign(send_count, send_count + npeers);
@@ -1180,6 +1213,7 @@
   if (!c) return fail("null context");
   if (nrows < 0 || !buffer_ext || !land || !wavnum_ext || !cgroup_ext || !omosnh2kd_ext || !depth_ext || !u_ext || !v_ext)
     return fail("ecwam_hip_proenvhalo_unpack: bad arguments");
+  c->adv_valid = false;
   DISPATCH(launch_proenv_unpack<float>(nrows, c->NFRE, buffer_ext, land, wavnum_ext, cgroup_ext, omosnh2kd_ext, depth_ext, u_ext, v_ext, (hipStream_t)stream),
            launch_proenv_unpack<double>(nrows, c->NFRE, buffer_ext, land, wavnum_ext, cgroup_ext, omosnh2kd_ext, depth_ext, u_ext, v_ext, (hipStream_t)stream));
   HIPCHK(hipGetLastError());
diff --git a/ecwam_amd/csrc/implsch4a.hip b/ecwam_amd/csrc/implsch4a.hip
--- a/ecwam_amd/csrc/implsch4a.hip
+++ b/ecwam_amd/csrc/implsch4a.hip
@@ -7,9 +7,9 @@
   if (kijl - kijs <= 0) return 0;
   if (NFRE != V4_NFRE) return -1;
   V4Adv<T> adv;
-  adv.f_in = (const T*)a->f_in; adv.klon = a->klon; adv.klat = a->klat; adv.kcor = a->kcor; adv.cg = (const T*)a->cg; adv.pt = (const T*)a->pt;
+  adv.f_in = (const T*)a->f_in; adv.rec = (const char*)a->rec;
   adv.dirT = (const T*)a->dirT; adv.dirI = a->dirI; adv.xdella = (T)a->xdella; adv.delpro = (T)a->delpro; adv.m0 = a->m0; adv.m1 = a->m1;
-  adv.gin = (const T*)a->gin; adv.delpro_lf = (T)a->delpro_lf; adv.gin_k = a->gin_k; adv.mlf = a->mlf; adv.obs = (const T*)a->obs;
+  adv.gin = (const T*)a->gin; adv.gin_k = a->gin_k; adv.mlf = a->mlf; adv.obs = (const T*)a->obs;
 #define V4_ARGS tab, kijs, kijl, fl_out, wvprpt, ff, intf, mij, xllws, fin, w2n, a->gfast, a->gfast_k, adv, s
 #define V4_ADV_CASE(NA, PPV, R1V, R2V, NHV, LFOK)                                                                                         \
   if (NANG == NA && r1 == R1V && r2 == R2V && nh == NHV) {                                                                              \
diff --git a/ecwam_amd/csrc/implsch_adv_args.h b/ecwam_amd/csrc/implsch_adv_args.h
--- a/ecwam_amd/csrc/implsch_adv_args.h
+++ b/ecwam_amd/csrc/implsch_adv_args.h
@@ -1,14 +1,11 @@
 #pragma once
 struct Implsch4AdvArgs {
   const void* f_in;
-  const int *klon, *klat, *kcor;
-  const void* cg;
-  const void* pt;
+  const void* rec;
   const void* dirT;
   const int* dirI;
   double xdella, delpro;
   const void* gin;
-  double delpro_lf;
   int gin_k, mlf;
   const void* obs;
   void* gfast;
diff --git a/ecwam_amd/csrc/implsch_v4.h b/ecwam_amd/csrc/implsch_v4.h
--- a/ecwam_amd/csrc/implsch_v4.h
+++ b/ecwam_amd/csrc/implsch_v4.h
@@ -264,16 +264,11 @@
 template <typename T>
 struct V4Adv {
   const T* f_in;
-  const int* klon;
-  const int* klat;
-  const int* kcor;
-  const T* cg;
-  const T* pt;
+  const char* rec;
   const T* dirT;
   const int* dirI;
   T xdella, delpro;
   const T* gin;
-  T delpro_lf;
   int gin_k, mlf;
   const T* obs;
   int m0, m1;
@@ -296,32 +291,40 @@
   int* sI = reinterpret_cast<int*>(sK + NKW);
   int* sD = sI + PP * 16;
   static_assert((PP * 5 * NFRE + PP * PTW + NKW) * sizeof(T) + (PP * 16 + NANG * 4) * sizeof(int) <= NSCR * sizeof(T), "LDS scratch of the advecting load");
-  for (int i = lane; i < PP * PTW; i += 64) {
-    const int q = i / PTW, e = i - q * PTW;
-    const T* g = A.pt + (size_t)(ij0 + (q < n ? q : n - 1)) * 12;
-    T v = T(0);
-    if (e < 12) v = g[e];
-    else if (e < 18) v = T(1) - g[e - 6];
-    else if (e == 18) v = g[0] * g[2];
-    else v = A.xdella * g[2];
-    if (e == 1) v = m_abs(v);
-    sPt[i] = v;
-  }
-  for (int i = lane; i < PP * 16; i += 64) {
-    const int q = i >> 4, e = i & 15;
-    const int ijq = ij0 + (q < n ? q : n - 1);
-    int v = ijq;
-    if (e >= 1 && e <= 2) v = A.klon[(size_t)ijq * 2 + (e - 1)];
-    if (e >= 3 && e <= 6) v = A.klat[(size_t)ijq * 4 + (e - 3)];
-    if (e >= 7 && e <= 14) v = A.kcor[(size_t)ijq * 8 + (e - 7)];
-    sI[i] = v;
-  }
-  for (int i = lane; i < NKW; i += 64) {
-    const T v = A.dirT[i];
-    const int e = i & 3;
-    sK[i] = i >= NANG * 4 + 4 ? T(2) * v : (i >= NANG * 4 ? v : (e < 2 ? T(2) * v : m_abs(v)));
-  }
-  for (int i = lane; i < NANG * 4; i += 64) sD[i] = A.dirI[i];
+  {
+    constexpr int PLB = 5 * NFRE * (int)sizeof(T), PTB = PTW * (int)sizeof(T), RB = PLB + PTB + 16 * (int)sizeof(int), CPR = RB / 16;
+    constexpr int NIT = (PP * CPR + 63) / 64, NKV = NKW / VEC, NKI = (NKV + 63) / 64, NDI = (NANG + 63) / 64;
+    static_assert(PLB % 16 == 0 && PTB % 16 == 0 && NKW % VEC == 0, "16-byte parts");
+    VT t[NIT], tk[NKI];
+    I4 td[NDI];
+    int dst[NIT];
+#pragma unroll
+    for (int it = 0; it < NIT; it++) {
+      const int c = lane + 64 * it, q = c / CPR, eb = (c - q * CPR) * 16;
+      dst[it] = -1;
+      if (c < PP * CPR) {
+        t[it] = *reinterpret_cast<const VT*>(A.rec + (size_t)(ij0 + (q < n ? q : n - 1)) * RB + eb);
+        dst[it] = eb < PLB ? q * PLB + eb
+                           : (eb < PLB + PTB ? PP * PLB + q * PTB + (eb - PLB)
+                                             : (int)(reinterpret_cast<char*>(sI) - reinterpret_cast<char*>(sB)) + q * 64 + (eb - PLB - PTB));
+      }
+    }
+#pragma unroll
+    for (int it = 0; it < NKI; it++)
+      if (lane + 64 * it < NKV) tk[it] = *reinterpret_cast<const VT*>(A.dirT + (lane + 64 * it) * VEC);
+#pragma unroll
+    for (int it = 0; it < NDI; it++)
+      if (lane + 64 * it < NANG) td[it] = *reinterpret_cast<const I4*>(A.dirI + (lane + 64 * it) * 4);
+#pragma unroll
+    for (int it = 0; it < NIT; it++)
+      if (dst[it] >= 0) *reinterpret_cast<VT*>(reinterpret_cast<char*>(sB) + dst[it]) = t[it];
+#pragma unroll
+    for (int it = 0; it < NKI; it++)
+      if (lane + 64 * it < NKV) *reinterpret_cast<VT*>(sK + (lane + 64 * it) * VEC) = tk[it];
+#pragma unroll
+    for (int it = 0; it < NDI; it++)
+      if (lane + 64 * it < NANG) *reinterpret_cast<I4*>(sD + (lane + 64 * it) * 4) = td[it];
+  }
   WSYNC();
   VT buf[D][NB];
   struct Rnd {
@@ -453,28 +456,6 @@
 #pragma unroll
   for (int c = 0; c < D - 1 && c < NCH; c++) issue(c, buf[c % D]);
   __builtin_amdgcn_sched_barrier(0);
-  for (int i = lane; i < PP * NFRE; i += 64) {
-    const int q = i / NFRE, m = i - q * NFRE;
-    const int* iq = sI + q * 16;
-    const T* pq = sPt + q * PTW;
-    T cgl[2], cgy0[2], cgy1[2];
-#pragma unroll
-    for (int ic = 0; ic < 2; ic++) {
-      cgl[ic] = A.cg[(size_t)iq[1 + ic] * NFRE + m];
-      cgy0[ic] = A.cg[(size_t)iq[3 + 2 * ic] * NFRE + m];
-      cgy1[ic] = A.cg[(size_t)iq[4 + 2 * ic] * NFRE + m];
-    }
-    const T wl[2] = {pq[6], pq[7]}, dp[2] = {pq[4], pq[5]};
-    const CtuBase<T> b = ctu_base(A.cg[(size_t)iq[0] * NFRE + m], cgl, cgy0, cgy1, wl, dp);
-    T* o = sB + q * 5 * NFRE + m;
-#if ECWAM_HIP_CTU_STRICT
-    o[0] = m_abs(b.h[0]); o[NFRE] = m_abs(b.h[1]); o[2 * NFRE] = m_abs(b.hy[0]); o[3 * NFRE] = m_abs(b.hy[1]); o[4 * NFRE] = b.cg0;
-#else
-    ctu_fast_planes<T>(b, pq[1], ((LF && m < A.mlf) ? A.delpro_lf : A.delpro) * sK[NANG * 4], o, o + NFRE, o + 2 * NFRE, o + 3 * NFRE);
-    o[4 * NFRE] = b.cg0;
-#endif
-  }
-  WSYNC();
 #pragma unroll
   for (int c = 0; c < NCH; c++) {
     if (c + D - 1 < NCH) issue(c + D - 1, buf[(c + D - 1) % D]);
diff --git a/ecwam_amd/csrc/propag.hip b/ecwam_amd/csrc/propag.hip
--- a/ecwam_amd/csrc/propag.hip
+++ b/ecwam_amd/csrc/propag.hip
@@ -1247,44 +1247,79 @@
   hipLaunchKernelGGL(k_newwind<T>, dim3((n + 255) / 256), dim3(256), 0, s, (const DevTab<T>*)tab, n, (T*)ff, (const T*)ffn, icode_wnd);
 }
 template <typename T>
-__global__ void k_ctu_prep(const DevTab<T>* __restrict__ tab, int kijs, int kijl, int ngy, T delpro, T delpro_lf, const int* __restrict__ kxlt,
-                           const T* __restrict__ zdello, T xdella, const T* __restrict__ cosph, const T* __restrict__ sinph,
-                           const T* __restrict__ wlat, const T* __restrict__ wcor, const T* __restrict__ cosphm1, T* __restrict__ pt,
-                           T* __restrict__ dirT, int* __restrict__ dirI) {
-  const int NANG = tab->NANG;
+__global__ void k_tile_tables(const DevTab<T>* __restrict__ tab, int n, int ngy, T delpro, T delpro_lf, int mlf, const int* __restrict__ kxlt,
+                              const T* __restrict__ zdello, T xdella, const T* __restrict__ cosph, const T* __restrict__ sinph,
+                              const int* __restrict__ klon, const int* __restrict__ klat, const int* __restrict__ kcor,
+                              const T* __restrict__ wlat, const T* __restrict__ wcor, const T* __restrict__ cg, const T* __restrict__ cosphm1,
+                              char* __restrict__ rec, T* __restrict__ dirT, int* __restrict__ dirI) {
+#pragma clang fp contract(off)
+  const int NANG = tab->NANG, NFRE = tab->NFRE;
+  const T cmtodeg = T(360.0) / tab->CIRC;
   if (blockIdx.x == 0) {
-    const T DELTH0 = T(0.25) * delpro / tab->DELTH;
     for (int k = threadIdx.x; k < NANG; k += blockDim.x) {
       T a, b;
-      ctu_dirfac(tab, k, DELTH0, T(1), a, b);
-      dirT[4 * k] = a; dirT[4 * k + 1] = b; dirT[4 * k + 2] = tab->SINTH[k]; dirT[4 * k + 3] = tab->COSTH[k];
+      ctu_dirfac(tab, k, T(0.25) * delpro / tab->DELTH, T(1), a, b);
+      dirT[4 * k] = T(2) * a; dirT[4 * k + 1] = T(2) * b; dirT[4 * k + 2] = m_abs(tab->SINTH[k]); dirT[4 * k + 3] = m_abs(tab->COSTH[k]);
       dirI[4 * k] = tab->JXO[k][0] | (tab->JYO[k][0] << 1) | (tab->KCR[k][0] << 2);
       dirI[4 * k + 1] = tab->KPM[k][0]; dirI[4 * k + 2] = tab->KPM[k][2]; dirI[4 * k + 3] = 0;
       if (delpro_lf > T(0)) {
         ctu_dirfac(tab, k, T(0.25) * delpro_lf / tab->DELTH, T(1), a, b);
-        dirT[4 * NANG + 4 + 2 * k] = a; dirT[4 * NANG + 4 + 2 * k + 1] = b;
+        dirT[4 * NANG + 4 + 2 * k] = T(2) * a; dirT[4 * NANG + 4 + 2 * k + 1] = T(2) * b;
       }
     }
     if (threadIdx.x == 0) {
-      dirT[4 * NANG] = T(360.0) / tab->CIRC;
+      dirT[4 * NANG] = cmtodeg;
       dirT[4 * NANG + 1] = dirT[4 * NANG + 2] = dirT[4 * NANG + 3] = T(0);
     }
   }
-  for (int ij = kijs + blockIdx.x * blockDim.x + threadIdx.x; ij < kijl; ij += gridDim.x * blockDim.x) {
+  const size_t rb = (size_t)(5 * NFRE + 20) * sizeof(T) + 16 * sizeof(int);
+  const long long total = (long long)n * NFRE;
+  for (long long g = (long long)blockIdx.x * blockDim.x + threadIdx.x; g < total; g += (long long)gridDim.x * blockDim.x) {
+    const int ij = (int)(g / NFRE), m = (int)(g - (long long)ij * NFRE);
     const CtuPoint<T> p = ctu_point(ij, ngy, kxlt, zdello, xdella, cosph, sinph, wlat, wcor, cosphm1);
-    T* o = pt + (size_t)ij * 12;
-    o[0] = p.zd; o[1] = p.cpm1; o[2] = p.ga; o[3] = p.tanph; o[4] = p.dp[0]; o[5] = p.dp[1]; o[6] = p.wl[0]; o[7] = p.wl[1];
-    o[8] = p.wc[0]; o[9] = p.wc[1]; o[10] = p.wc[2]; o[11] = p.wc[3];
-  }
-}
-template <typename T>
-void launch_ctu_prep(const void* tab, int kijs, int kijl, int ngy, double delpro, double delpro_lf, const int* kxlt, const void* zdello, double xdella,
-                     const void* cosph, const void* sinph, const void* wlat, const void* wcor, const void* cosphm1, void* pt, void* dirT, int* dirI,
-                     hipStream_t s) {
-  const int n = kijl - kijs;
-  hipLaunchKernelGGL(k_ctu_prep<T>, dim3(n > 0 ? grid_for(n) : 1), dim3(256), 0, s, (const DevTab<T>*)tab, kijs, kijl, ngy, (T)delpro, (T)delpro_lf, kxlt,
-                     (const T*)zdello, (T)xdella, (const T*)cosph, (const T*)sinph, (const T*)wlat, (const T*)wcor, (const T*)cosphm1, (T*)pt,
-                     (T*)dirT, dirI);
+    T* o = reinterpret_cast<T*>(rec + (size_t)ij * rb);
+    T* opt = o + 5 * NFRE;
+    int* oid = reinterpret_cast<int*>(opt + 20);
+    const T acpm1 = m_abs(p.cpm1);
+    int id[16];
+    id[0] = id[15] = ij;
+    for (int e = 0; e < 2; e++) id[1 + e] = klon[(size_t)ij * 2 + e];
+    for (int e = 0; e < 4; e++) id[3 + e] = klat[(size_t)ij * 4 + e];
+    for (int e = 0; e < 8; e++) id[7 + e] = kcor[(size_t)ij * 8 + e];
+    T cgl[2], cgy0[2], cgy1[2];
+    for (int ic = 0; ic < 2; ic++) {
+      cgl[ic] = cg[(size_t)id[1 + ic] * NFRE + m];
+      cgy0[ic] = cg[(size_t)id[3 + 2 * ic] * NFRE + m];
+      cgy1[ic] = cg[(size_t)id[4 + 2 * ic] * NFRE + m];
+    }
+    const CtuBase<T> b = ctu_base(cg[(size_t)ij * NFRE + m], cgl, cgy0, cgy1, p.wl, p.dp);
+    o += m;
+#if ECWAM_HIP_CTU_STRICT
+    o[0] = m_abs(b.h[0]); o[NFRE] = m_abs(b.h[1]); o[2 * NFRE] = m_abs(b.hy[0]); o[3 * NFRE] = m_abs(b.hy[1]); o[4 * NFRE] = b.cg0;
+#else
+    ctu_fast_planes<T>(b, acpm1, (m < mlf ? delpro_lf : delpro) * cmtodeg, o, o + NFRE, o + 2 * NFRE, o + 3 * NFRE);
+    o[4 * NFRE] = b.cg0;
+#endif
+    for (int e = m; e < 20; e += NFRE) {
+      const T g12[12] = {p.zd, acpm1, p.ga, p.tanph, p.dp[0], p.dp[1], p.wl[0], p.wl[1], p.wc[0], p.wc[1], p.wc[2], p.wc[3]};
+      T v;
+      if (e < 12) v = g12[e];
+      else if (e < 18) v = T(1) - g12[e - 6];
+      else if (e == 18) v = p.zd * p.ga;
+      else v = xdella * p.ga;
+      opt[e] = v;
+    }
+    for (int e = m; e < 16; e += NFRE) oid[e] = id[e];
+  }
+}
+template <typename T>
+void launch_tile_tables(const void* tab, int n, int NFRE, int ngy, double delpro, double delpro_lf, int mlf, const int* kxlt, const void* zdello,
+                        double xdella, const void* cosph, const void* sinph, const int* klon, const int* klat, const int* kcor, const void* wlat,
+                        const void* wcor, const void* cg, const void* cosphm1, void* rec, void* dirT, int* dirI, hipStream_t s) {
+  const long long total = (long long)n * NFRE;
+  hipLaunchKernelGGL(k_tile_tables<T>, dim3(total > 0 ? grid_for(total) : 1), dim3(256), 0, s, (const DevTab<T>*)tab, n, ngy, (T)delpro, (T)delpro_lf,
+                     mlf, kxlt, (const T*)zdello, (T)xdella, (const T*)cosph, (const T*)sinph, klon, klat, kcor, (const T*)wlat, (const T*)wcor,
+                     (const T*)cg, (const T*)cosphm1, (char*)rec, (T*)dirT, dirI);
 }
 template <typename T>
 __global__ void k_nosource(const DevTab<T>* __restrict__ tab, long long e0, long long e1, T* __restrict__ fl1, T* __restrict__ xllws, int kijs,
@@ -1351,7 +1386,7 @@
                                const void*, const int*, const int*, const int*, void*, void*, const void*, const void*, void*,   \
                                int*, int, const void*, hipStream_t);                                                              \
   template void launch_newwind<T>(const void*, int, void*, const void*, int, hipStream_t);                                        \
-  template void launch_ctu_prep<T>(const void*, int, int, int, double, double, const int*, const void*, double, const void*, const void*, const void*, const void*, const void*, void*, void*, int*, hipStream_t);\
+  template void launch_tile_tables<T>(const void*, int, int, int, double, double, int, const int*, const void*, double, const void*, const void*, const int*, const int*, const int*, const void*, const void*, const void*, const void*, void*, void*, int*, hipStream_t);\
   template void launch_nosource<T>(const void*, int, int, int, void*, void*, int*, hipStream_t);                                  \
   template void launch_propdot<T>(const void*, int, int, int, const int*, const void*, double, const void*, const int*,         \
                                   const int*, const void*, const void*, const void*, const void*, const void*, void*, hipStream_t); \
diff --git a/ecwam_amd/lib.py b/ecwam_amd/lib.py
--- a/ecwam_amd/lib.py
+++ b/ecwam_amd/lib.py
@@ -54,7 +54,7 @@
 
 
 EXPORTS = ["ecwam_hip_last_error", "ecwam_hip_abi_version", "ecwam_hip_selftest", "ecwam_hip_create", "ecwam_hip_destroy", "ecwam_hip_set_obstructions", "ecwam_hip_propags2",
-           "ecwam_hip_ctuw", "ecwam_hip_propags2_otf", "ecwam_hip_propags2_otf_split", "ecwam_hip_propags2_otf_fast", "ecwam_hip_set_fastwave_copy", "ecwam_hip_copy_freq_range", "ecwam_hip_propdot", "ecwam_hip_ctuw_refra", "ecwam_hip_propags2_refra", "ecwam_hip_implsch", "ecwam_hip_implsch_generation_used", "ecwam_hip_device_tables", "ecwam_hip_implsch_reserve", "ecwam_hip_propags2_implsch_supported", "ecwam_hip_propags2_implsch", "ecwam_hip_outbs", "ecwam_hip_outbs_sepwisw", "ecwam_hip_outbs_partition", "ecwam_hip_outbs_extremes", "ecwam_hip_outbs_absolute", "ecwam_hip_set_second_order", "ecwam_hip_outbs_second_order", "ecwam_hip_outwnorm", "ecwam_hip_newwind", "ecwam_hip_newwind_icode", "ecwam_hip_nosource", "ecwam_hip_host_register", "ecwam_hip_host_unregister", "ecwam_hip_chunks_to_points",
+           "ecwam_hip_ctuw", "ecwam_hip_propags2_otf", "ecwam_hip_propags2_otf_split", "ecwam_hip_propags2_otf_fast", "ecwam_hip_set_fastwave_copy", "ecwam_hip_tile_tables_invalidate", "ecwam_hip_tile_tables_fills", "ecwam_hip_copy_freq_range", "ecwam_hip_propdot", "ecwam_hip_ctuw_refra", "ecwam_hip_propags2_refra", "ecwam_hip_implsch", "ecwam_hip_implsch_generation_used", "ecwam_hip_device_tables", "ecwam_hip_implsch_reserve", "ecwam_hip_propags2_implsch_supported", "ecwam_hip_propags2_implsch", "ecwam_hip_outbs", "ecwam_hip_outbs_sepwisw", "ecwam_hip_outbs_partition", "ecwam_hip_outbs_extremes", "ecwam_hip_outbs_absolute", "ecwam_hip_set_second_order", "ecwam_hip_outbs_second_order", "ecwam_hip_outwnorm", "ecwam_hip_newwind", "ecwam_hip_newwind_icode", "ecwam_hip_nosource", "ecwam_hip_host_register", "ecwam_hip_host_unregister", "ecwam_hip_chunks_to_points",
            "ecwam_hip_points_to_chunks", "ecwam_hip_member_scatter", "ecwam_hip_member_gather", "ecwam_hip_pack_rows", "ecwam_hip_unpack_rows", "ecwam_hip_halo_setup", "ecwam_hip_halo_counts", "ecwam_hip_comm_unique_id",
            "ecwam_hip_comm_init", "ecwam_hip_comm_count", "ecwam_hip_halo_start", "ecwam_hip_halo_finish", "ecwam_hip_halo_pack_host", "ecwam_hip_halo_unpack_host", "ecwam_hip_proenvhalo_pack", "ecwam_hip_proenvhalo_unpack", "ecwam_hip_malloc", "ecwam_hip_free",
            "ecwam_hip_memcpy_h2d", "ecwam_hip_memcpy_d2h", "ecwam_hip_memset", "ecwam_hip_sync", "ecwam_hip_queue_create", "ecwam_hip_queue_destroy",
@@ -90,6 +90,9 @@
     lib.ecwam_hip_propags2_otf_split.argtypes = [vp, vp, vp, ci, ci, cd, cd, ci, ci, vp, ci, vp, vp, cd, vp, vp, vp, vp, vp, vp, vp, vp, vp, vp, ci, ci, ci, ci, ci, vp]
     lib.ecwam_hip_propags2_otf_fast.argtypes = [vp, vp, vp, ci, ci, cd, cd, ci, ci, vp, ci, ci, vp, ci, vp, vp, cd, vp, vp, vp, vp, vp, vp, vp, vp, vp, vp, ci, ci, ci, ci, ci, vp]
     lib.ecwam_hip_set_fastwave_copy.argtypes = [vp, vp, ci]
+    lib.ecwam_hip_tile_tables_invalidate.argtypes = [vp]
+    lib.ecwam_hip_tile_tables_fills.argtypes = [vp]
+    lib.ecwam_hip_tile_tables_fills.restype = C.c_longlong
     lib.ecwam_hip_propags2_implsch_supported.argtypes = [vp]
     lib.ecwam_hip_propags2_implsch.argtypes = [vp, vp, vp, ci, ci, cd, vp, vp, cd, vp, vp, vp, vp, vp, vp, vp, vp, vp, ci, ci, ci, ci, vp, vp, vp, vp, vp, vp,
                                                cd, ci, vp, ci, ci, vp]
diff --git a/include/ecwam_hip.h b/include/ecwam_hip.h
--- a/include/ecwam_hip.h
+++ b/include/ecwam_hip.h
@@ -126,6 +126,8 @@
 const void *ecwam_hip_device_tables(ecwam_hip_ctx *ctx);
 int ecwam_hip_implsch_reserve(ecwam_hip_ctx *ctx, int npts);
 
+int ecwam_hip_tile_tables_invalidate(ecwam_hip_ctx *ctx);
+long long ecwam_hip_tile_tables_fills(ecwam_hip_ctx *ctx);
 int ecwam_hip_propags2_implsch_supported(ecwam_hip_ctx *ctx);
 int ecwam_hip_propags2_implsch(ecwam_hip_ctx *ctx, const void *f1, void *f3, int n, int ngy, double delpro, const int *kxlt, const void *zdello,
                                double xdella, const void *cosph, const void *sinph, const int *klon, const int *klat, const int *kcor,
```

Measured after the change: 60.40 million grid-point spectral steps/s (median of 6 runs). No clear change (+0.6%).
